# MIT-SPARK/Kimera-Semantics

Hardware: AMD Instinct MI355X
Metric: Mvoxel-updates/s + frames/s, 640×480 @5cm voxels, 1/2/4/8 MI355X (higher is better)
Workload: dtype f32; 1 GPU; bag-replay stand-in: 640x480 depth+label trajectory (room), 'fast' integrator, 5 cm voxels, 5 m rays, trunc 0.2 m, p=0.8; pipeline_frames=12, parallelism=frame-sharded x1, points_per_frame=305657, rays_per_frame=85307, updates_per_frame=502687

## Files before the change

### include/ks_hip.h

```cpp
#ifndef KS_HIP_H_
#define KS_HIP_H_

#include <stddef.h>
#include <stdint.h>

#ifdef __cplusplus
extern "C" {
#endif

#define KS_NUM_LABELS 21

enum {
  KS_OK = 0,
  KS_ERR_INVALID_ARG = -1,
  KS_ERR_LABEL_RANGE = -2,
  KS_ERR_PROBABILITY = -3,
  KS_ERR_HIP = -4,
  KS_ERR_POOL_FULL = -5,
  KS_ERR_INDEX_RANGE = -6,
  KS_ERR_NO_DEVICE = -7,
  KS_ERR_UNSUPPORTED = -8,
  KS_ERR_PEER_FAILED = -9
};

enum { KS_METHOD_FAST = 0, KS_METHOD_MERGED = 1 };
enum { KS_COLOR_MODE_COLOR = 0, KS_COLOR_MODE_SEMANTIC = 1, KS_COLOR_MODE_SEMANTIC_PROBABILITY = 2 };
enum { KS_ORDER_MIXED = 0, KS_ORDER_SORTED = 1, KS_ORDER_MIXED_1024_GROUPS = 2 };
enum { KS_BUNDLE_ORDER_REFERENCE = 0, KS_BUNDLE_ORDER_CANONICAL = 1 };
enum { KS_EARLY_OUT_EXACT = 1 };

typedef struct ks_config {
  float voxel_size;
  int32_t voxels_per_side;
  float truncation_distance;
  float max_weight;
  float min_ray_length_m;
  float max_ray_length_m;
  int32_t voxel_carving_enabled;
  int32_t use_const_weight;
  int32_t allow_clear;
  int32_t use_weight_dropoff;
  int32_t use_sparsity_compensation_factor;
  float sparsity_compensation_factor;
  int32_t enable_anti_grazing;
  float start_voxel_subsampling_factor;
  int32_t max_consecutive_ray_collisions;
  int32_t clear_checks_every_n_frames;
  int32_t integration_order_mode;
  int32_t integrator_threads;
  int32_t method;
  int32_t bundle_order;
  float semantic_measurement_probability;
  int32_t color_mode;
  int32_t n_dynamic_labels;
  uint8_t dynamic_labels[32];
  uint8_t label_rgba[256][4];
  int32_t early_out_phase_growth;
  int32_t device_id;
  uint32_t max_tiles;
  uint32_t max_points;
  int32_t pipeline_frames;
} ks_config;

typedef struct ks_frame_stats {
  uint64_t n_points;
  uint64_t n_valid_points;
  uint64_t n_rays_cast;
  uint64_t n_voxel_updates;
  uint64_t n_blocks_allocated;
} ks_frame_stats;

enum {
  KS_STAGE_POINTS = 0,
  KS_STAGE_SORT_POINTS,
  KS_STAGE_RAYS,
  KS_STAGE_MARCH,
  KS_STAGE_EMIT,
  KS_STAGE_SORT_PAIRS,
  KS_STAGE_APPLY,
  KS_STAGE_APPLY_LONG,
  KS_STAGE_COUNT
};
typedef struct ks_profile {
  double ms[KS_STAGE_COUNT];
  uint64_t launches[KS_STAGE_COUNT];
  uint64_t frames;
  uint64_t updates;
  uint64_t points;
  double apply_kernel_ms;
  uint64_t apply_kernel_launches;
  uint64_t apply_kernel_updates;
  double host_ms;
  double host_wait_ms;
} ks_profile;

typedef struct ks_ctx ks_ctx;

int ks_default_config(ks_config* cfg);
int ks_create(const ks_config* cfg, ks_ctx** out);
void ks_destroy(ks_ctx* ctx);
const char* ks_last_error(ks_ctx* ctx);

int ks_set_color_to_label(ks_ctx* ctx, const uint8_t* rgba_keys, const uint8_t* labels, size_t n);

int ks_integrate_points(ks_ctx* ctx, const float T_G_C[7], const float* xyz, const uint8_t* rgba,
                        const uint8_t* labels, size_t n, int freespace, ks_frame_stats* stats);
int ks_integrate_points_device(ks_ctx* ctx, const float T_G_C[7], const float* d_xyz, const uint8_t* d_rgba,
                               const uint8_t* d_labels, size_t n, int freespace, ks_frame_stats* stats);

int ks_integrate_depth(ks_ctx* ctx, const float T_G_C[7], const void* depth, int depth_fmt, const uint8_t* label_img,
                       const uint8_t* rgba_img, int width, int height, const float K[4], int freespace,
                       ks_frame_stats* stats);
int ks_integrate_depth_device(ks_ctx* ctx, const float T_G_C[7], const void* d_depth, int depth_fmt,
                              const uint8_t* d_label_img, const uint8_t* d_rgba_img, int width, int height,
                              const float K[4], int freespace, ks_frame_stats* stats);

int ks_num_blocks(ks_ctx* ctx, size_t* n);
int ks_get_block_indices(ks_ctx* ctx, int32_t* out_xyz, size_t cap, size_t* n);
int ks_get_updated_block_indices(ks_ctx* ctx, int32_t* out_xyz, size_t cap, size_t* n, int reset);
int ks_download_blocks(ks_ctx* ctx, const int32_t* idx_xyz, size_t n, void* tsdf_out, void* sem_out);
int ks_upload_blocks(ks_ctx* ctx, const int32_t* idx_xyz, size_t n, const void* tsdf_in, const void* sem_in);
#define KS_VOXEL_RECORD_BYTES 120
typedef struct ks_voxel_run {
  int32_t block[3];
  uint32_t first;
  uint32_t count;
} ks_voxel_run;
int ks_count_updated_voxels(ks_ctx* ctx, size_t* n_records, size_t* n_runs );
int ks_download_updated_voxels(ks_ctx* ctx, void* out, size_t cap_records, size_t* n_records, ks_voxel_run* runs,
                               size_t cap_runs, size_t* n_runs);
void* ks_host_alloc(size_t bytes);
void ks_host_free(void* p);

typedef struct ks_mesh_config { float min_weight; int32_t only_stale; } ks_mesh_config;
typedef struct ks_mesh_stats {
  uint64_t blocks_meshed, blocks_total, triangles_total, triangles_changed, degenerate_dropped;
} ks_mesh_stats;
typedef struct ks_mesh_block { int32_t block[3]; uint32_t first_vertex, n_vertices; } ks_mesh_block;
int ks_mesh_default_config(ks_mesh_config* cfg);
int ks_mesh_update(ks_ctx* ctx, const ks_mesh_config* cfg, ks_mesh_stats* stats );
int ks_mesh_size(ks_ctx* ctx, size_t* n_blocks, size_t* n_vertices);
int ks_mesh_download(ks_ctx* ctx, ks_mesh_block* blocks, size_t cap_blocks, float* xyz, float* normals, uint8_t* rgba,
                     uint8_t* labels, size_t cap_vertices);
int ks_mesh_changed_blocks(ks_ctx* ctx, int32_t* out_xyz, size_t cap, size_t* n);

typedef struct ks_esdf_config {
  float min_weight, min_distance_m, max_distance_m;
  int32_t use_region;
  int32_t region_min[3], region_max[3];
  uint64_t max_workspace_bytes;
} ks_esdf_config;
typedef struct ks_esdf_stats { uint64_t voxels_observed, voxels_fixed, voxels_clamped, box_voxels[3], workspace_bytes; } ks_esdf_stats;
#define KS_ESDF_RECORD_BYTES 8
int ks_esdf_default_config(ks_esdf_config* cfg);
int ks_esdf_update(ks_ctx* ctx, const ks_esdf_config* cfg, ks_esdf_stats* stats );
typedef struct ks_esdf_refresh_stats {
  uint64_t tiles_stale, tiles_recomputed, tiles_total;
  uint64_t voxels_observed, voxels_fixed, voxels_clamped;
  uint64_t workspace_bytes;
} ks_esdf_refresh_stats;
int ks_esdf_refresh(ks_ctx* ctx, uint64_t max_workspace_bytes , ks_esdf_refresh_stats* stats );
int ks_esdf_changed_blocks(ks_ctx* ctx, int32_t* out_xyz, size_t cap, size_t* n);
int ks_esdf_download_blocks(ks_ctx* ctx, const int32_t* idx_xyz, size_t n, void* out );
int ks_esdf_query(ks_ctx* ctx, const float* xyz , size_t n, float* distance, uint8_t* flags,
                  uint8_t* label );

typedef struct ks_render_config { float min_weight, min_range_m, max_range_m; } ks_render_config;
typedef struct ks_render_stats { uint64_t pixels_hit, pixels_missed, samples; } ks_render_stats;
int ks_render_default_config(ks_render_config* cfg);
int ks_render_view(ks_ctx* ctx, const float T_G_C[7], const float K[4] , int width, int height,
                   const ks_render_config* cfg, float* depth, uint8_t* labels, uint8_t* rgba ,
                   float* normals , ks_render_stats* stats );
int ks_render_view_device(ks_ctx* ctx, const float T_G_C[7], const float K[4], int width, int height, const ks_render_config* cfg,
                          float* d_depth, uint8_t* d_labels, uint8_t* d_rgba, float* d_normals, ks_render_stats* stats);

#define KS_TILE_BYTES 65536
int ks_get_tile_keys(ks_ctx* ctx, uint64_t* out, size_t cap, size_t* n);
int ks_export_tiles_device(ks_ctx* ctx, const uint32_t* slots, size_t n, void* d_payload);
int ks_merge_tiles_device(ks_ctx* ctx, const uint64_t* keys, size_t n, const void* d_payload);
int ks_clear(ks_ctx* ctx);
int ks_clear_voxels(ks_ctx* ctx);
int ks_reset_tiles(ks_ctx* ctx, const uint32_t* slots, size_t n);
int ks_tile_owner(uint64_t tile_key, int world);
typedef struct ks_reduce_stats {
  uint64_t tiles_sent, tiles_received, tiles_local, bytes_sent;
} ks_reduce_stats;
int ks_reduce(ks_ctx* ctx, void* rccl_comm, int rank, int world, ks_reduce_stats* stats);

typedef struct ks_round_stats {
  uint64_t updates_marched, updates_applied, bytes_sent, origin_voxel_touched, rays_cast;
} ks_round_stats;
int ks_integrate_round_exact(ks_ctx* marcher, ks_ctx* owner, void* rccl_comm, int rank, int world, uint64_t first_frame,
                             const float T_G_C[7], const float* xyz, const uint8_t* rgba, const uint8_t* labels, size_t n,
                             int freespace_points, ks_round_stats* stats);

int ks_debug_radix_sort(ks_ctx* ctx, void* keys, uint32_t* vals, size_t n, int key_bits, unsigned end_bit);

int ks_synchronize(ks_ctx* ctx);
void* ks_stream(ks_ctx* ctx);
int ks_flush(ks_ctx* ctx, ks_frame_stats* stats);
int ks_profile_enable(ks_ctx* ctx, int level);
int ks_early_out_iterations(ks_ctx* ctx, uint64_t* frames, uint64_t* iterations);
int ks_early_out_stats(ks_ctx* ctx, uint64_t out[5]);
int ks_profile_get(ks_ctx* ctx, ks_profile* out, int reset);
int ks_update_stats(ks_ctx* ctx, uint64_t out[4]);
int ks_pipeline_shape(ks_ctx* ctx, int32_t out[4]);
int ks_stream_plan(ks_ctx* ctx, int32_t out[8]);
int ks_seed_launch_shape(int32_t integration_order_mode, int32_t early_out_phase_growth, uint64_t cap_points, uint32_t* out, int32_t max_phases);

#ifdef __cplusplus
}
#endif
#endif
```

### kimera_semantics_amd/binding.py

```python
from __future__ import annotations

import ctypes as C
import os
import subprocess

import numpy as np

_HERE = os.path.dirname(os.path.abspath(__file__))
LIB_PATH = os.environ.get("KS_HIP_LIB") or os.path.join(_HERE, "libks_hip.so")
NUM_LABELS = 21

KS_METHOD_FAST, KS_METHOD_MERGED = 0, 1
KS_COLOR_MODE_COLOR, KS_COLOR_MODE_SEMANTIC, KS_COLOR_MODE_SEMANTIC_PROBABILITY = 0, 1, 2
KS_ORDER_MIXED, KS_ORDER_SORTED, KS_ORDER_MIXED_1024_GROUPS = 0, 1, 2
KS_BUNDLE_ORDER_REFERENCE, KS_BUNDLE_ORDER_CANONICAL = 0, 1
KS_EARLY_OUT_EXACT = 1
KS_ERR_LABEL_RANGE, KS_ERR_PROBABILITY, KS_ERR_POOL_FULL, KS_ERR_NO_DEVICE, KS_ERR_UNSUPPORTED = -2, -3, -5, -7, -8
KS_ERR_INVALID_ARG, KS_ERR_PEER_FAILED = -1, -9

STAGES = ["points", "sort_points", "rays", "march", "emit", "sort_pairs", "apply", "apply_long"]

TSDF_DTYPE = np.dtype([("distance", "<f4"), ("weight", "<f4"), ("color", "u1", (4,))])
SEM_DTYPE = np.dtype([("label", "u1"), ("pad", "u1", (3,)), ("priors", "<f4", (NUM_LABELS,)),
                      ("color", "u1", (4,))])

ABI_SYMBOLS = [
    "ks_default_config", "ks_create", "ks_destroy", "ks_last_error", "ks_set_color_to_label",
    "ks_integrate_points", "ks_integrate_points_device", "ks_integrate_depth", "ks_integrate_depth_device", "ks_num_blocks", "ks_get_block_indices",
    "ks_get_updated_block_indices", "ks_count_updated_voxels", "ks_download_updated_voxels", "ks_download_blocks", "ks_upload_blocks", "ks_host_alloc", "ks_host_free", "ks_get_tile_keys", "ks_export_tiles_device", "ks_merge_tiles_device", "ks_clear", "ks_clear_voxels", "ks_reset_tiles", "ks_tile_owner", "ks_reduce",
    "ks_debug_radix_sort", "ks_synchronize", "ks_flush", "ks_stream",
    "ks_profile_enable", "ks_profile_get", "ks_early_out_iterations", "ks_early_out_stats", "ks_pipeline_shape", "ks_stream_plan", "ks_seed_launch_shape", "ks_update_stats", "ks_integrate_round_exact",
    "ks_mesh_default_config", "ks_mesh_update", "ks_mesh_size", "ks_mesh_download", "ks_mesh_changed_blocks",
    "ks_esdf_default_config", "ks_esdf_update", "ks_esdf_download_blocks", "ks_esdf_query",
    "ks_esdf_refresh", "ks_esdf_changed_blocks",
    "ks_render_default_config", "ks_render_view", "ks_render_view_device",
]


class KsConfig(C.Structure):
    _fields_ = [
        ("voxel_size", C.c_float), ("voxels_per_side", C.c_int32),
        ("truncation_distance", C.c_float), ("max_weight", C.c_float),
        ("min_ray_length_m", C.c_float), ("max_ray_length_m", C.c_float),
        ("voxel_carving_enabled", C.c_int32), ("use_const_weight", C.c_int32),
        ("allow_clear", C.c_int32), ("use_weight_dropoff", C.c_int32),
        ("use_sparsity_compensation_factor", C.c_int32), ("sparsity_compensation_factor", C.c_float),
        ("enable_anti_grazing", C.c_int32), ("start_voxel_subsampling_factor", C.c_float),
        ("max_consecutive_ray_collisions", C.c_int32), ("clear_checks_every_n_frames", C.c_int32),
        ("integration_order_mode", C.c_int32), ("integrator_threads", C.c_int32),
        ("method", C.c_int32), ("bundle_order", C.c_int32),
        ("semantic_measurement_probability", C.c_float), ("color_mode", C.c_int32),
        ("n_dynamic_labels", C.c_int32), ("dynamic_labels", C.c_uint8 * 32),
        ("label_rgba", (C.c_uint8 * 4) * 256),
        ("early_out_phase_growth", C.c_int32),
        ("device_id", C.c_int32), ("max_tiles", C.c_uint32), ("max_points", C.c_uint32), ("pipeline_frames", C.c_int32),
    ]


class KsRoundStats(C.Structure):
    _fields_ = [("updates_marched", C.c_uint64), ("updates_applied", C.c_uint64), ("bytes_sent", C.c_uint64),
                ("origin_voxel_touched", C.c_uint64), ("rays_cast", C.c_uint64)]


class KsFrameStats(C.Structure):
    _fields_ = [("n_points", C.c_uint64), ("n_valid_points", C.c_uint64), ("n_rays_cast", C.c_uint64),
                ("n_voxel_updates", C.c_uint64), ("n_blocks_allocated", C.c_uint64)]


class KsReduceStats(C.Structure):
    _fields_ = [("tiles_sent", C.c_uint64), ("tiles_received", C.c_uint64), ("tiles_local", C.c_uint64),
                ("bytes_sent", C.c_uint64)]


class KsMeshConfig(C.Structure):
    _fields_ = [("min_weight", C.c_float), ("only_stale", C.c_int32)]


class KsMeshStats(C.Structure):
    _fields_ = [("blocks_meshed", C.c_uint64), ("blocks_total", C.c_uint64), ("triangles_total", C.c_uint64),
                ("triangles_changed", C.c_uint64), ("degenerate_dropped", C.c_uint64)]


MESH_BLOCK_DTYPE = np.dtype([("block", "<i4", (3,)), ("first_vertex", "<u4"), ("n_vertices", "<u4")])


class KsEsdfConfig(C.Structure):
    _fields_ = [("min_weight", C.c_float), ("min_distance_m", C.c_float), ("max_distance_m", C.c_float), ("use_region", C.c_int32),
                ("region_min", C.c_int32 * 3), ("region_max", C.c_int32 * 3), ("max_workspace_bytes", C.c_uint64)]


class KsEsdfStats(C.Structure):
    _fields_ = [("voxels_observed", C.c_uint64), ("voxels_fixed", C.c_uint64), ("voxels_clamped", C.c_uint64),
                ("box_voxels", C.c_uint64 * 3), ("workspace_bytes", C.c_uint64)]


class KsEsdfRefreshStats(C.Structure):
    _fields_ = [("tiles_stale", C.c_uint64), ("tiles_recomputed", C.c_uint64), ("tiles_total", C.c_uint64),
                ("voxels_observed", C.c_uint64), ("voxels_fixed", C.c_uint64), ("voxels_clamped", C.c_uint64),
                ("workspace_bytes", C.c_uint64)]


ESDF_DTYPE = np.dtype([("distance", "<f4"), ("flags", "u1"), ("label", "u1"), ("pad", "u1", (2,))])


class KsRenderConfig(C.Structure):
    _fields_ = [("min_weight", C.c_float), ("min_range_m", C.c_float), ("max_range_m", C.c_float)]


class KsRenderStats(C.Structure):
    _fields_ = [("pixels_hit", C.c_uint64), ("pixels_missed", C.c_uint64), ("samples", C.c_uint64)]


class KsProfile(C.Structure):
    _fields_ = [("ms", C.c_double * 8), ("launches", C.c_uint64 * 8), ("frames", C.c_uint64),
                ("updates", C.c_uint64), ("points", C.c_uint64), ("apply_kernel_ms", C.c_double),
                ("apply_kernel_launches", C.c_uint64), ("apply_kernel_updates", C.c_uint64),
                ("host_ms", C.c_double), ("host_wait_ms", C.c_double)]


def build(force: bool = False) -> str:
    src_dir = os.path.join(_HERE, "csrc")
    srcs = [os.path.join(src_dir, f) for f in ("ks_hip.hip", "ks_types.h", "ks_k_rays.h", "ks_k_bundle_order.h", "ks_k_march.h", "ks_k_exact.h", "ks_k_apply.h",
                                                "ks_k_apply_xl.h", "ks_k_shard.h", "ks_k_shard_merged.h", "ks_k_io.h", "ks_k_mesh.h", "ks_k_esdf.h", "ks_k_render.h", "ks_mc_tri_table.inc", "ks_device_math.h", "ks_radix_sort.h", "ks_owned.h")]
    srcs.append(os.path.join(_HERE, "..", "include", "ks_hip.h"))
    stale = (not os.path.exists(LIB_PATH)) or any(
        os.path.exists(s) and os.path.getmtime(s) > os.path.getmtime(LIB_PATH) for s in srcs)
    if force or stale:
        subprocess.check_call(["make", "-C", src_dir])
    return LIB_PATH


_lib = None


def lib():
    global _lib
    if _lib is None:
        if not os.path.exists(LIB_PATH):
            raise RuntimeError(f"{LIB_PATH} is missing: run `python -c 'import __graft_entry__ as g; g.build()'` "
                               "(the HIP path has no CPU fallback)")
        L = C.CDLL(LIB_PATH)
        vp = C.c_void_p
        L.ks_default_config.argtypes = [C.POINTER(KsConfig)]
        L.ks_create.argtypes = [C.POINTER(KsConfig), C.POINTER(vp)]
        L.ks_destroy.argtypes = [vp]
        L.ks_destroy.restype = None
        L.ks_last_error.argtypes = [vp]
        L.ks_last_error.restype = C.c_char_p
        L.ks_set_color_to_label.argtypes = [vp, vp, vp, C.c_size_t]
        L.ks_integrate_points.argtypes = [vp, vp, vp, vp, vp, C.c_size_t, C.c_int, C.POINTER(KsFrameStats)]
        L.ks_integrate_points_device.argtypes = [vp, vp, vp, vp, vp, C.c_size_t, C.c_int, C.POINTER(KsFrameStats)]
        L.ks_integrate_depth.argtypes = [vp, vp, vp, C.c_int, vp, vp, C.c_int, C.c_int, vp, C.c_int, C.POINTER(KsFrameStats)]
        L.ks_integrate_depth_device.argtypes = [vp, vp, vp, C.c_int, vp, vp, C.c_int, C.c_int, vp, C.c_int, C.POINTER(KsFrameStats)]
        L.ks_num_blocks.argtypes = [vp, C.POINTER(C.c_size_t)]
        L.ks_get_block_indices.argtypes = [vp, vp, C.c_size_t, C.POINTER(C.c_size_t)]
        L.ks_get_updated_block_indices.argtypes = [vp, vp, C.c_size_t, C.POINTER(C.c_size_t), C.c_int]
        L.ks_download_blocks.argtypes = [vp, vp, C.c_size_t, vp, vp]
        L.ks_count_updated_voxels.argtypes = [vp, C.POINTER(C.c_size_t), C.POINTER(C.c_size_t)]
        L.ks_download_updated_voxels.argtypes = [vp, vp, C.c_size_t, C.POINTER(C.c_size_t), vp, C.c_size_t, C.POINTER(C.c_size_t)]
        L.ks_upload_blocks.argtypes = [vp, vp, C.c_size_t, vp, vp]
        L.ks_host_alloc.argtypes = [C.c_size_t]
        L.ks_host_alloc.restype = C.c_void_p
        L.ks_host_free.argtypes = [vp]
        L.ks_host_free.restype = None
        L.ks_get_tile_keys.argtypes = [vp, vp, C.c_size_t, C.POINTER(C.c_size_t)]
        L.ks_export_tiles_device.argtypes = [vp, vp, C.c_size_t, vp]
        L.ks_merge_tiles_device.argtypes = [vp, vp, C.c_size_t, vp]
        L.ks_clear.argtypes = [vp]
        L.ks_clear_voxels.argtypes = [vp]
        L.ks_reset_tiles.argtypes = [vp, vp, C.c_size_t]
        L.ks_tile_owner.argtypes = [C.c_uint64, C.c_int]
        L.ks_reduce.argtypes = [vp, vp, C.c_int, C.c_int, C.POINTER(KsReduceStats)]
        L.ks_debug_radix_sort.argtypes = [vp, vp, vp, C.c_size_t, C.c_int, C.c_uint]
        L.ks_synchronize.argtypes = [vp]
        L.ks_flush.argtypes = [vp, C.POINTER(KsFrameStats)]
        L.ks_stream.argtypes = [vp]
        L.ks_stream.restype = vp
        L.ks_profile_enable.argtypes = [vp, C.c_int]
        L.ks_profile_get.argtypes = [vp, C.POINTER(KsProfile), C.c_int]
        L.ks_early_out_iterations.argtypes = [vp, C.POINTER(C.c_uint64), C.POINTER(C.c_uint64)]
        L.ks_early_out_stats.argtypes = [vp, C.POINTER(C.c_uint64)]
        L.ks_pipeline_shape.argtypes = [vp, C.POINTER(C.c_int32)]
        L.ks_stream_plan.argtypes = [vp, C.POINTER(C.c_int32)]
        L.ks_seed_launch_shape.argtypes = [C.c_int32, C.c_int32, C.c_uint64, C.POINTER(C.c_uint32), C.c_int32]
        L.ks_update_stats.argtypes = [vp, C.POINTER(C.c_uint64)]
        L.ks_integrate_round_exact.argtypes = [vp, vp, vp, C.c_int, C.c_int, C.c_uint64, vp, vp, vp, vp, C.c_size_t, C.c_int, C.POINTER(KsRoundStats)]
        L.ks_mesh_default_config.argtypes = [C.POINTER(KsMeshConfig)]
        L.ks_mesh_update.argtypes = [vp, C.POINTER(KsMeshConfig), C.POINTER(KsMeshStats)]
        L.ks_mesh_size.argtypes = [vp, C.POINTER(C.c_size_t), C.POINTER(C.c_size_t)]
        L.ks_mesh_download.argtypes = [vp, vp, C.c_size_t, vp, vp, vp, vp, C.c_size_t]
        L.ks_mesh_changed_blocks.argtypes = [vp, vp, C.c_size_t, C.POINTER(C.c_size_t)]
        L.ks_esdf_default_config.argtypes = [C.POINTER(KsEsdfConfig)]
        L.ks_esdf_update.argtypes = [vp, C.POINTER(KsEsdfConfig), C.POINTER(KsEsdfStats)]
        L.ks_esdf_download_blocks.argtypes = [vp, vp, C.c_size_t, vp]
        L.ks_esdf_query.argtypes = [vp, vp, C.c_size_t, vp, vp, vp]
        L.ks_esdf_refresh.argtypes = [vp, C.c_uint64, C.POINTER(KsEsdfRefreshStats)]
        L.ks_esdf_changed_blocks.argtypes = [vp, vp, C.c_size_t, C.POINTER(C.c_size_t)]
        L.ks_render_default_config.argtypes = [C.POINTER(KsRenderConfig)]
        L.ks_render_view.argtypes = [vp, vp, vp, C.c_int, C.c_int, C.POINTER(KsRenderConfig), vp, vp, vp, vp, C.POINTER(KsRenderStats)]
        L.ks_render_view_device.argtypes = [vp, vp, vp, C.c_int, C.c_int, C.POINTER(KsRenderConfig), vp, vp, vp, vp, C.POINTER(KsRenderStats)]
        _lib = L
    return _lib


def default_config(**overrides) -> KsConfig:
    cfg = KsConfig()
    lib().ks_default_config(C.byref(cfg))
    apply_overrides(cfg, **overrides)
    return cfg


def apply_overrides(cfg, **overrides):
    for k, v in overrides.items():
        if k == "dynamic_labels":
            cfg.n_dynamic_labels = len(v)
            for i, lab in enumerate(v):
                cfg.dynamic_labels[i] = int(lab)
        elif k == "label_rgba":
            arr = np.ascontiguousarray(np.asarray(v, dtype=np.uint8).reshape(256, 4))
            C.memmove(cfg.label_rgba, arr.ctypes.data, 1024)
        else:
            if not hasattr(cfg, k):
                raise AttributeError(k)
            setattr(cfg, k, v)
    return cfg


class KsError(RuntimeError):
    def __init__(self, code, msg):
        super().__init__(f"ks error {code}: {msg}")
        self.code = code


def _ptr(a):
    return None if a is None else a.ctypes.data


class HipIntegrator:

    def __init__(self, cfg: KsConfig):
        self.cfg = cfg
        self.vps = cfg.voxels_per_side
        self._h = C.c_void_p()
        rc = lib().ks_create(C.byref(cfg), C.byref(self._h))
        if rc != 0:
            raise KsError(rc, lib().ks_last_error(None).decode())

    def _chk(self, rc):
        if rc != 0:
            raise KsError(rc, lib().ks_last_error(self._h).decode())

    def close(self):
        if getattr(self, "_h", None):
            lib().ks_destroy(self._h)
            self._h = C.c_void_p()

    def __del__(self):
        try:
            self.close()
        except Exception:
            pass

    def set_color_to_label(self, rgba_keys, labels):
        k = np.ascontiguousarray(rgba_keys, dtype=np.uint8).reshape(-1, 4)
        l = np.ascontiguousarray(labels, dtype=np.uint8)
        self._chk(lib().ks_set_color_to_label(self._h, _ptr(k), _ptr(l), len(l)))

    def integrate(self, T_G_C, xyz, rgba, labels, freespace=False) -> KsFrameStats:
        T = np.ascontiguousarray(T_G_C, dtype=np.float32)
        xyz = np.ascontiguousarray(xyz, dtype=np.float32)
        labels = None if labels is None else np.ascontiguousarray(labels, dtype=np.uint8)
        rgba = None if rgba is None else np.ascontiguousarray(rgba, dtype=np.uint8)
        st = KsFrameStats()
        self._chk(lib().ks_integrate_points(self._h, _ptr(T), _ptr(xyz), _ptr(rgba), _ptr(labels), xyz.shape[0],
                                            int(freespace), C.byref(st)))
        return st

    def integrate_depth(self, T_G_C, depth, K, label_img=None, rgba_img=None, freespace=False) -> KsFrameStats:
        T = np.ascontiguousarray(T_G_C, dtype=np.float32)
        depth = np.ascontiguousarray(depth)
        fmt = 0 if depth.dtype == np.float32 else 1
        assert depth.dtype in (np.float32, np.uint16)
        Kc = np.ascontiguousarray(K, dtype=np.float32)
        lab = None if label_img is None else np.ascontiguousarray(label_img, dtype=np.uint8)
        col = None if rgba_img is None else np.ascontiguousarray(rgba_img, dtype=np.uint8)
        st = KsFrameStats()
        self._chk(lib().ks_integrate_depth(self._h, _ptr(T), _ptr(depth), fmt, _ptr(lab), _ptr(col), depth.shape[1],
                                           depth.shape[0], _ptr(Kc), int(freespace), C.byref(st)))
        return st

    def integrate_depth_device(self, T_G_C, d_depth: int, fmt: int, d_label_img: int, d_rgba_img: int, width: int,
                               height: int, K, freespace=False) -> KsFrameStats:
        T = np.ascontiguousarray(T_G_C, dtype=np.float32)
        Kc = np.ascontiguousarray(K, dtype=np.float32)
        st = KsFrameStats()
        self._chk(lib().ks_integrate_depth_device(self._h, _ptr(T), d_depth or None, fmt, d_label_img or None,
                                                  d_rgba_img or None, width, height, _ptr(Kc), int(freespace), C.byref(st)))
        return st

    def integrate_device(self, T_G_C, d_xyz: int, d_rgba: int, d_labels: int, n: int, freespace=False) -> KsFrameStats:
        T = np.ascontiguousarray(T_G_C, dtype=np.float32)
        st = KsFrameStats()
        self._chk(lib().ks_integrate_points_device(self._h, _ptr(T), d_xyz or None, d_rgba or None, d_labels or None, n,
                                                   int(freespace), C.byref(st)))
        return st

    def block_indices(self) -> np.ndarray:
        n = C.c_size_t()
        self._chk(lib().ks_get_block_indices(self._h, None, 0, C.byref(n)))
        out = np.zeros((n.value, 3), dtype=np.int32)
        if n.value:
            self._chk(lib().ks_get_block_indices(self._h, _ptr(out), n.value, C.byref(n)))
        return out

    def updated_block_indices(self, reset=True) -> np.ndarray:
        n = C.c_size_t()
        self._chk(lib().ks_get_updated_block_indices(self._h, None, 0, C.byref(n), 0))
        out = np.zeros((n.value, 3), dtype=np.int32)
        self._chk(lib().ks_get_updated_block_indices(self._h, _ptr(out), n.value, C.byref(n), int(reset)))
        return out

    def download(self, indices=None):
        if indices is None:
            indices = self.block_indices()
        indices = np.ascontiguousarray(indices, dtype=np.int32).reshape(-1, 3)
        nv = self.vps ** 3
        t = np.zeros((len(indices), nv), dtype=TSDF_DTYPE)
        s = np.zeros((len(indices), nv), dtype=SEM_DTYPE)
        if len(indices):
            self._chk(lib().ks_download_blocks(self._h, _ptr(indices), len(indices), _ptr(t), _ptr(s)))
        return indices, t, s

    def upload(self, indices, tsdf=None, sem=None):
        indices = np.ascontiguousarray(indices, dtype=np.int32).reshape(-1, 3)
        nv = self.vps ** 3
        tp = sp = None
        if tsdf is not None:
            tsdf = np.ascontiguousarray(tsdf, dtype=TSDF_DTYPE).reshape(len(indices), nv)
            tp = _ptr(tsdf)
        if sem is not None:
            sem = np.ascontiguousarray(sem, dtype=SEM_DTYPE).reshape(len(indices), nv)
            sp = _ptr(sem)
        self._chk(lib().ks_upload_blocks(self._h, _ptr(indices), len(indices), tp, sp))

    def mesh(self, only_stale=False, min_weight=1e-4):
        from .mesh import Mesh
        mc, st = KsMeshConfig(float(min_weight), int(bool(only_stale))), KsMeshStats()
        self._chk(lib().ks_mesh_update(self._h, C.byref(mc), C.byref(st)))
        nb, nv = C.c_size_t(), C.c_size_t()
        self._chk(lib().ks_mesh_size(self._h, C.byref(nb), C.byref(nv)))
        blocks = np.zeros(nb.value, dtype=MESH_BLOCK_DTYPE)
        xyz, normals = np.zeros((nv.value, 3), np.float32), np.zeros((nv.value, 3), np.float32)
        rgba, labels = np.zeros((nv.value, 4), np.uint8), np.zeros(nv.value, np.uint8)
        self._chk(lib().ks_mesh_download(self._h, _ptr(blocks), nb.value, _ptr(xyz), _ptr(normals), _ptr(rgba), _ptr(labels), nv.value))
        return Mesh(blocks, xyz, normals, rgba, labels, {k: int(getattr(st, k)) for k, _ in KsMeshStats._fields_})

    def mesh_changed_blocks(self) -> np.ndarray:
        n = C.c_size_t()
        self._chk(lib().ks_mesh_changed_blocks(self._h, None, 0, C.byref(n)))
        out = np.zeros((n.value, 3), dtype=np.int32)
        if n.value:
            self._chk(lib().ks_mesh_changed_blocks(self._h, _ptr(out), n.value, C.byref(n)))
        return out

    def esdf_update(self, region=None, **cfg) -> dict:
        ec, st = KsEsdfConfig(), KsEsdfStats()
        lib().ks_esdf_default_config(C.byref(ec))
        for k, v in cfg.items():
            if k not in ("min_weight", "min_distance_m", "max_distance_m", "max_workspace_bytes"):
                raise AttributeError(k)
            setattr(ec, k, v)
        if region is not None:
            ec.use_region = 1
            for a in range(3):
                ec.region_min[a], ec.region_max[a] = int(region[0][a]), int(region[1][a])
        rc = lib().ks_esdf_update(self._h, C.byref(ec), C.byref(st))
        stats = {k: ([int(v) for v in getattr(st, k)] if k == "box_voxels" else int(getattr(st, k))) for k, _ in KsEsdfStats._fields_}
        if rc != 0:
            err = KsError(rc, lib().ks_last_error(self._h).decode())
            err.stats = stats
            raise err
        return stats

    def esdf(self, region=None, **cfg):
        stats = self.esdf_update(region=region, **cfg)
        idx = self.block_indices()
        return idx, self.esdf_blocks(idx), stats

    def esdf_refresh(self, max_workspace_bytes=0) -> dict:
        st = KsEsdfRefreshStats()
        rc = lib().ks_esdf_refresh(self._h, int(max_workspace_bytes), C.byref(st))
        stats = {k: int(getattr(st, k)) for k, _ in KsEsdfRefreshStats._fields_}
        if rc != 0:
            err = KsError(rc, lib().ks_last_error(self._h).decode())
            err.stats = stats
            raise err
        return stats

    def esdf_changed_blocks(self) -> np.ndarray:
        n = C.c_size_t()
        self._chk(lib().ks_esdf_changed_blocks(self._h, None, 0, C.byref(n)))
        out = np.zeros((n.value, 3), dtype=np.int32)
        if n.value:
            self._chk(lib().ks_esdf_changed_blocks(self._h, _ptr(out), n.value, C.byref(n)))
        return out

    def esdf_blocks(self, indices) -> np.ndarray:
        indices = np.ascontiguousarray(indices, dtype=np.int32).reshape(-1, 3)
        out = np.zeros((len(indices), self.vps ** 3), dtype=ESDF_DTYPE)
        self._chk(lib().ks_esdf_download_blocks(self._h, _ptr(indices), len(indices), _ptr(out)))
        return out

    def esdf_query(self, xyz) -> np.ndarray:
        xyz = np.ascontiguousarray(xyz, dtype=np.float32).reshape(-1, 3)
        n = len(xyz)
        d, f, l = np.zeros(n, np.float32), np.zeros(n, np.uint8), np.zeros(n, np.uint8)
        self._chk(lib().ks_esdf_query(self._h, _ptr(xyz), n, _ptr(d), _ptr(f), _ptr(l)))
        out = np.zeros(n, dtype=ESDF_DTYPE)
        out["distance"], out["flags"], out["label"] = d, f, l
        return out

    def render_config(self, **cfg) -> KsRenderConfig:
        rc = KsRenderConfig()
        lib().ks_render_default_config(C.byref(rc))
        for k, v in cfg.items():
            if k not in ("min_weight", "min_range_m", "max_range_m"):
                raise AttributeError(k)
            if v is not None:
                setattr(rc, k, v)
        return rc

    def render(self, T_G_C, K, width, height, min_weight=None, min_range_m=None, max_range_m=None, normals=True):
        T = np.ascontiguousarray(T_G_C, dtype=np.float32)
        Kc = np.ascontiguousarray(K, dtype=np.float32)
        rc, st = self.render_config(min_weight=min_weight, min_range_m=min_range_m, max_range_m=max_range_m), KsRenderStats()
        w, h = int(width), int(height)
        shape = (max(h, 0), max(w, 0))
        depth, labels, rgba = np.zeros(shape, np.float32), np.zeros(shape, np.uint8), np.zeros(shape + (4,), np.uint8)
        nrm = np.zeros(shape + (3,), np.float32) if normals else None
        self._chk(lib().ks_render_view(self._h, _ptr(T), _ptr(Kc), w, h, C.byref(rc), _ptr(depth), _ptr(labels), _ptr(rgba), _ptr(nrm), C.byref(st)))
        return depth, labels, rgba, nrm, {k: int(getattr(st, k)) for k, _ in KsRenderStats._fields_}

    def render_device(self, T_G_C, K, width, height, d_depth: int, d_labels: int, d_rgba: int, d_normals: int, stats=True, **cfg):
        T = np.ascontiguousarray(T_G_C, dtype=np.float32)
        Kc = np.ascontiguousarray(K, dtype=np.float32)
        rc, st = self.render_config(**cfg), KsRenderStats()
        self._chk(lib().ks_render_view_device(self._h, _ptr(T), _ptr(Kc), int(width), int(height), C.byref(rc), d_depth or None, d_labels or None,
                                              d_rgba or None, d_normals or None, C.byref(st) if stats else None))
        return {k: int(getattr(st, k)) for k, _ in KsRenderStats._fields_} if stats else None

    TILE_BYTES = 65536

    def tile_keys(self) -> np.ndarray:
        n = C.c_size_t()
        self._chk(lib().ks_get_tile_keys(self._h, None, 0, C.byref(n)))
        out = np.zeros(n.value, dtype=np.uint64)
        if n.value:
            self._chk(lib().ks_get_tile_keys(self._h, _ptr(out), n.value, C.byref(n)))
        return out

    def export_tiles(self, slots: np.ndarray, d_payload: int):
        s = np.ascontiguousarray(slots, dtype=np.uint32)
        self._chk(lib().ks_export_tiles_device(self._h, _ptr(s), len(s), d_payload or None))

    def merge_tiles(self, keys: np.ndarray, d_payload: int):
        k = np.ascontiguousarray(keys, dtype=np.uint64)
        self._chk(lib().ks_merge_tiles_device(self._h, _ptr(k), len(k), d_payload or None))

    def download_updated_voxels(self):
        n, nr = C.c_size_t(), C.c_size_t()
        self._chk(lib().ks_count_updated_voxels(self._h, C.byref(n), C.byref(nr)))
        dt = np.dtype([("block", "<i4", (3,)), ("linear", "<u4"), ("tsdf", TSDF_DTYPE), ("sem", SEM_DTYPE)])
        rdt = np.dtype([("block", "<i4", (3,)), ("first", "<u4"), ("count", "<u4")])
        assert dt.itemsize == 120 and rdt.itemsize == 20
        out = np.zeros(n.value, dtype=dt)
        runs = np.zeros(nr.value, dtype=rdt)
        if n.value:
            m, mr = C.c_size_t(), C.c_size_t()
            self._chk(lib().ks_download_updated_voxels(self._h, _ptr(out), n.value, C.byref(m), _ptr(runs), nr.value, C.byref(mr)))
            assert m.value == n.value and mr.value == nr.value
            assert int(runs["count"].sum()) == n.value
            for r in runs[:: max(1, len(runs) // 16)]:
                if r["count"]:
                    assert (out["block"][r["first"]:r["first"] + r["count"]] == r["block"]).all()
        return out

    def clear(self):
        self._chk(lib().ks_clear(self._h))

    def clear_voxels(self):
        self._chk(lib().ks_clear_voxels(self._h))

    def reset_tiles(self, slots: np.ndarray):
        s = np.ascontiguousarray(slots, dtype=np.uint32)
        self._chk(lib().ks_reset_tiles(self._h, _ptr(s), len(s)))

    def reduce(self, rccl_comm, rank: int, world: int) -> dict:
        st = KsReduceStats()
        self._chk(lib().ks_reduce(self._h, C.c_void_p(rccl_comm) if rccl_comm else None, rank, world, C.byref(st)))
        return {"tiles_sent": st.tiles_sent, "tiles_received": st.tiles_received, "tiles_local": st.tiles_local,
                "bytes_sent": st.bytes_sent}

    def debug_radix_sort(self, keys: np.ndarray, vals=None, end_bit=None):
        keys = np.ascontiguousarray(keys).copy()
        bits = keys.dtype.itemsize * 8
        vals = None if vals is None else np.ascontiguousarray(vals, dtype=np.uint32).copy()
        self._chk(lib().ks_debug_radix_sort(self._h, _ptr(keys), _ptr(vals), keys.shape[0], bits,
                                            bits if end_bit is None else end_bit))
        return keys, vals

    def synchronize(self):
        self._chk(lib().ks_synchronize(self._h))

    @property
    def stream(self) -> int:
        return lib().ks_stream(self._h) or 0

    def profile_enable(self, level=1):
        self._chk(lib().ks_profile_enable(self._h, int(level)))

    def early_out_stats(self):
        out = (C.c_uint64 * 5)()
        self._chk(lib().ks_early_out_stats(self._h, out))
        return dict(frames=int(out[0]), rounds=int(out[1]), fallbacks=int(out[2]), event_driven=bool(out[3]), pipelined=bool(out[4]))

    def integrate_round_exact(self, marcher: "HipIntegrator", rccl_comm, rank: int, world: int, first_frame: int, T_G_C, xyz, rgba, labels,
                              freespace=False) -> dict:
        T = np.ascontiguousarray(T_G_C, dtype=np.float32)
        n = 0 if xyz is None else len(xyz)
        x = None if xyz is None else np.ascontiguousarray(xyz, dtype=np.float32)
        c = None if rgba is None else np.ascontiguousarray(rgba, dtype=np.uint8)
        l = None if labels is None else np.ascontiguousarray(labels, dtype=np.uint8)
        st = KsRoundStats()
        self._chk(lib().ks_integrate_round_exact(marcher._h, self._h, rccl_comm, int(rank), int(world), int(first_frame), _ptr(T),
                                                 _ptr(x) if x is not None else None, _ptr(c) if c is not None else None,
                                                 _ptr(l) if l is not None else None, n, int(bool(freespace)), C.byref(st)))
        return dict(updates_marched=int(st.updates_marched), updates_applied=int(st.updates_applied), bytes_sent=int(st.bytes_sent),
                    origin_voxel_touched=bool(st.origin_voxel_touched), rays_cast=int(st.rays_cast))

    def update_stats(self):
        out = (C.c_uint64 * 4)()
        self._chk(lib().ks_update_stats(self._h, out))
        return dict(walked=int(out[0]), serial=int(out[1]), chunks=int(out[2]), replayed=int(out[3]))

    def pipeline_shape(self):
        out = (C.c_int32 * 4)()
        self._chk(lib().ks_pipeline_shape(self._h, out))
        return dict(lag=int(out[0]), slots=int(out[1]), batch=int(out[2]), march_streams=int(out[3]))

    def stream_plan(self):
        out = (C.c_int32 * 8)()
        self._chk(lib().ks_stream_plan(self._h, out))
        side = {1: "own", 0: "tail", -1: "none"}
        return dict(budget=int(out[0]), streams=int(out[1]), march_streams=int(out[2]), long=side[int(out[3])], xlong=side[int(out[4])],
                    march="own" if out[5] else "A", tail="own" if out[6] else "A", streams_held=int(out[7]))

    def early_out_iterations(self):
        f, it = C.c_uint64(), C.c_uint64()
        self._chk(lib().ks_early_out_iterations(self._h, C.byref(f), C.byref(it)))
        return f.value, it.value

    def flush(self) -> KsFrameStats:
        st = KsFrameStats()
        self._chk(lib().ks_flush(self._h, C.byref(st)))
        return st

    def profile(self, reset=False) -> dict:
        p = KsProfile()
        self._chk(lib().ks_profile_get(self._h, C.byref(p), int(reset)))
        return {"ms": {STAGES[i]: p.ms[i] for i in range(8)}, "launches": {STAGES[i]: p.launches[i] for i in range(8)},
                "frames": p.frames, "updates": p.updates, "points": p.points,
                "apply_kernel_ms": p.apply_kernel_ms, "apply_kernel_launches": p.apply_kernel_launches,
                "apply_kernel_updates": p.apply_kernel_updates, "host_ms": p.host_ms, "host_wait_ms": p.host_wait_ms}
```

### kimera_semantics_amd/csrc/ks_hip.hip

```cpp

#include <atomic>
#include <chrono>
#include <condition_variable>
#include <mutex>
#include <thread>
#include <cstring>
#include <string.h>

#include <dlfcn.h>
#include <hip/hip_runtime.h>
#include <hip/hip_ext.h>
#include <rccl/rccl.h>

#include <algorithm>
#include <iterator>
#include <cmath>
#include <cstdio>
#include <cstring>
#include <string>
#include <unordered_map>
#include <vector>

#include "../../include/ks_hip.h"
#include "ks_device_math.h"
// ... 338 lines not shown
  DevBuf<float> mesh_xyz[2], mesh_nrm[2];
  DevBuf<uint32_t> mesh_rgba[2];
  DevBuf<uint8_t> mesh_label[2];
  size_t mesh_cap[2] = {0, 0};
  int mesh_cur = 0;
  bool mesh_valid = false;
  float mesh_min_weight = 0.f;
  std::vector<uint64_t> mesh_blocks;
  uint32_t mesh_tiles_seen = 0;
  std::vector<ks_mesh_block> mesh_dir;
  std::vector<int32_t> mesh_changed;
  DevBuf<uint8_t> d_mesh_buf[10];
  DevBuf<EsdfRecord> esdf_store;
  DevBuf<uint64_t> esdf_keys[2];
  DevBuf<uint32_t> esdf_slots;
  DevBuf<unsigned long long> esdf_counters;
  DevBuf<EsdfRecord> esdf_out;
  DevBuf<int32_t> esdf_idx;
  DevBuf<float> esdf_xyz;
  bool esdf_valid = false;
  uint32_t esdf_tiles = 0;
  ks_esdf_config esdf_cfg{};
  uint64_t esdf_totals[3] = {0, 0, 0};
  std::vector<int32_t> esdf_changed;
  DevBuf<uint64_t> esdf_bricks[2];
  DevBuf<uint64_t> esdf_lists;
  DevBuf<uint32_t> esdf_zslots;
  DevBuf<float> render_depth, render_normals;
  DevBuf<uint32_t> render_rgba;
  DevBuf<uint8_t> render_labels;
  DevBuf<unsigned long long> render_counters;
  ks_profile prof{};
  ProfSet pset[kProfSets];
  bool fatal = false;
};

#define HIPCHK(ctx, expr)                                                                         \
  do {                                                                                            \
    hipError_t e_ = (expr);                                                                       \
    if (e_ != hipSuccess) {                                                                       \
      (ctx)->err = std::string(#expr) + ": " + hipGetErrorString(e_);                             \
      return KS_ERR_HIP;                                                                          \
    }                                                                                             \
  } while (0)

int ks_hip_failed(ks_ctx* ctx, const char* what, hipError_t e) {
  ctx->err = std::string(what) + ": " + hipGetErrorString(e);
  return KS_ERR_HIP;
}

namespace {

inline hipStream_t march_stream(ks_ctx* c, uint64_t frame_no) { return c->stream_march_[frame_no % (uint64_t)c->n_march]; }
inline uint64_t* observed_table(ks_ctx* c, uint64_t frame_no) { return c->d_observed_[frame_no % (uint64_t)c->n_obs]; }
int sync_march(ks_ctx* c) {
  for (int i = 0; i < c->n_march; ++i)
    if (c->stream_march_[i] != c->stream) HIPCHK(c, hipStreamSynchronize(c->stream_march_[i]));
  return KS_OK;
}

void probe_rehash_schedule(size_t n_max, BoSchedule* out) {
  static std::mutex mu;
  static std::vector<uint32_t> t, b;
  static size_t probed = 0;
  std::lock_guard<std::mutex> lk(mu);
  if (probed < n_max) {
    t.clear();
    b.clear();
    std::unordered_map<uint32_t, char> m;
    size_t bc = m.bucket_count();
    for (uint32_t i = 0; i < n_max; ++i) {
      m.emplace(i, 0);
      if (m.bucket_count() != bc) {
        bc = m.bucket_count();
        t.push_back(i);
        b.push_back((uint32_t)bc);
      }
    }
    probed = n_max;
  }
  *out = BoSchedule{};
  uint32_t off = 0;
  int e = 0;
  for (; e < (int)t.size() && e < kBoMaxEpochs && t[e] < n_max; ++e) {
    out->t[e] = t[e];
    out->b[e] = b[e];
    out->head_off[e] = off;
    off += b[e];
  }
  out->n_epochs = (uint32_t)e;
  out->t[e] = UINT32_MAX;
}

int ensure_bundle_order(ks_ctx* c, size_t cap) {
  probe_rehash_schedule(cap, &c->bo_sched);
  const BoSchedule& S = c->bo_sched;
  {
    static const uint32_t kLibstdcxxBuckets[] = {13, 29, 59, 127, 257, 541, 1109, 2357, 5087, 10273, 20753, 42043, 85229, 172933};
    for (uint32_t e = 0; e < S.n_epochs && e < sizeof(kLibstdcxxBuckets) / sizeof(uint32_t); ++e)
      if (S.b[e] != kLibstdcxxBuckets[e] || (e > 0 && S.t[e] != kLibstdcxxBuckets[e - 1])) {
        c->err = "bundle_order = KS_BUNDLE_ORDER_REFERENCE needs libstdc++'s unordered_map rehash schedule (13, 29, 59, ...): this build's standard "
                 "library differs; use KS_BUNDLE_ORDER_CANONICAL";
        return KS_ERR_UNSUPPORTED;
      }
  }
  c->bo_epochs = (int)S.n_epochs;
  size_t heads = 0;
  for (uint32_t e = 0; e < S.n_epochs; ++e) heads += S.b[e];
  const size_t nbt = cap / kBoBlock + 2, nfbt = 2 * cap / kBoBlock + 2;
  auto al = [](size_t words) { return (words * 4 + 255) & ~(size_t)255; };
  const size_t per_map = 11 * al(cap) + al(nbt) + al(heads);
  const size_t total = 2 * per_map + al(2) + al((sizeof(BoSchedule) + 3) / 4) + 2 * al(2 * cap) + al(nfbt) + al(cap);
  if (int rc = c->d_bo_slab.alloc(c, total)) return rc;
  uint8_t* p = c->d_bo_slab;
  auto take = [&](size_t words) { uint32_t* r = (uint32_t*)p; p += al(words); return r; };
  for (int m = 0; m < 2; ++m) {
    BoMap& M = c->bo.m[m];
    M.H = take(cap); M.rank = take(cap);
    M.next[0] = take(cap); M.next[1] = take(cap);
    M.idj[0] = take(cap); M.idj[1] = take(cap);
    M.kj[0] = take(cap); M.kj[1] = take(cap);
    M.lp = take(cap); M.gm = take(cap); M.cj = take(cap);
    M.bt = take(nbt);
    M.head = take(heads);
    HIPCHK(c, hipMemsetAsync(M.head, 0xff, heads * 4, c->stream));
  }
  c->bo.B = take(2);
  BoSchedule* d_sched = (BoSchedule*)take((sizeof(BoSchedule) + 3) / 4);
  c->bo.sched = d_sched;
  c->bo.flag = take(2 * cap);
  c->bo.flag_lp = take(2 * cap);
  c->bo.flag_bt = take(nfbt);
  c->bo.t_of_head = take(cap);
  HIPCHK(c, hipMemcpyAsync(d_sched, &c->bo_sched, sizeof(BoSchedule), hipMemcpyHostToDevice, c->stream));
  HIPCHK(c, hipStreamSynchronize(c->stream));
  return KS_OK;
}

inline uint32_t order_chains(int order_mode, size_t n) {
  const size_t q = n / kOrderStep;
  return (order_mode == KS_ORDER_MIXED && q >= 1) ? (uint32_t)q : kOrderStep;
}
inline uint32_t order_chains_cap(int order_mode, size_t cap) { return std::max(order_chains(order_mode, cap), order_mode == KS_ORDER_MIXED ? kOrderStep : 0u); }
inline uint32_t order_generations_cap(int order_mode, size_t cap) {
  if (order_mode == KS_ORDER_MIXED) return cap >= kOrderStep ? 2u * kOrderStep - 1u : 1u;
  return (uint32_t)((cap + kOrderStep - 1) / kOrderStep);
}
std::vector<uint32_t> phase_bounds(uint32_t n_gen, int growth) {
  std::vector<uint32_t> b{0};
  for (;;) {
    const uint64_t inc = std::max<uint64_t>(1, (uint64_t)b.back() * (uint64_t)(growth - 16) / 16);
    if (b.back() + inc >= n_gen) break;
    b.push_back((uint32_t)(b.back() + inc));
  }
  return b;
}
inline uint64_t seed_items_of(int order_mode, size_t n, uint32_t g0, uint32_t g1) {
  if (n == 0) return 0;
  const uint64_t chains = order_chains(order_mode, n), full = n / chains, part = n % chains;
  auto subs = [&](uint64_t gens) -> uint64_t {
    const uint64_t hi = std::min<uint64_t>(g1, gens);
    return hi > g0 ? (hi - g0 + kSubRun - 1) / kSubRun : 0;
  };
  return (chains - part) * subs(full) + part * subs(full + 1);
}
std::vector<SeedPhase> seed_launch_shape(int order_mode, int growth, size_t cap) {
  const uint32_t n_gen = order_generations_cap(order_mode, cap);
  const std::vector<uint32_t> B = phase_bounds(n_gen, growth);
  std::vector<SeedPhase> out;
  uint64_t off = 0;
  for (size_t j = 0; j < B.size(); ++j) {
    const uint32_t g0 = B[j], g1 = (j + 1 < B.size()) ? B[j + 1] : n_gen;
    uint64_t m = 0;
    if (order_mode == KS_ORDER_MIXED) {
      m = seed_items_of(order_mode, std::min<size_t>(cap, kOrderStep - 1), g0, g1);
      for (size_t q = 1; q <= cap / kOrderStep; ++q) m = std::max(m, seed_items_of(order_mode, std::min<size_t>(cap, q * kOrderStep + kOrderStep - 1), g0, g1));
    } else {
      m = seed_items_of(order_mode, cap, g0, g1);
    }
    out.push_back(SeedPhase{g0, g1, (uint32_t)off, (uint32_t)m});
    off += m;
  }
  return out;
}

size_t steps_max_of(const ks_config& cfg, float voxel_size_inv) {
  const double max_len = (double)cfg.max_ray_length_m + 2.0 * (double)cfg.truncation_distance;
  return (size_t)std::ceil(1.7321 * max_len * (double)voxel_size_inv) + 8;
}
int ensure_exact_points(ks_ctx* c, size_t cap);
int ensure_points(ks_ctx* c, size_t n) {
  if (n <= c->cap_points) return KS_OK;
  const size_t cap = std::max<size_t>(c->cap_points ? n + n / 8 : n, 1024);
  c->cap_points = 0;
  int rc;
  if ((rc = c->d_xyz.alloc(c, cap * 3))) return rc;
  if ((rc = c->d_rgba.alloc(c, cap * 4))) return rc;
  if ((rc = c->d_labels.alloc(c, cap))) return rc;
  ++c->buffers_epoch;
  const size_t scan_cap = (c->cfg.method == KS_METHOD_MERGED ? 2 : 1) * cap;
  size_t seed_items = 0;
  if (c->uses_early_out) {
    c->seed_phases = seed_launch_shape(c->cfg.integration_order_mode, c->cfg.early_out_phase_growth, cap);
    uint32_t off = 0;
    for (SeedPhase& P : c->seed_phases) {
      if ((P.g1 - P.g0 + kSubRun - 1) / kSubRun > (1u << kSeedSubBits) || order_chains_cap(c->cfg.integration_order_mode, cap) > (1u << kSeedChainBits)) {
        c->err = "point cloud too large for the early-out's work list";
        return KS_ERR_INVALID_ARG;
      }
      if (c->seed_cap_items) P.item_cap = (uint32_t)std::min<size_t>(P.item_cap, c->seed_cap_items);
      P.item_off = off;
      off += P.item_cap;
    }
    seed_items = off;
    if ((rc = c->d_seed_phases.alloc(c, c->seed_phases.size()))) return rc;
    HIPCHK(c, hipMemcpyAsync(c->d_seed_phases, c->seed_phases.data(), c->seed_phases.size() * sizeof(SeedPhase), hipMemcpyHostToDevice, c->stream));
    HIPCHK(c, hipStreamSynchronize(c->stream));
  }
  for (int i = 0; i < (c->cfg.pipeline_frames ? c->n_slots : 1); ++i) {
    if (c->uses_early_out) {
      if ((rc = c->slot[i].d_seed_gen.alloc(c, cap + order_chains_cap(c->cfg.integration_order_mode, cap)))) return rc;
      if ((rc = c->slot[i].d_seed_items.alloc(c, seed_items))) return rc;
      if ((rc = c->slot[i].d_seed_n.alloc(c, c->seed_phases.size()))) return rc;
    }
    if ((rc = c->slot[i].d_rays.alloc(c, cap))) return rc;
    if ((rc = c->slot[i].d_ray_list.alloc(c, cap))) return rc;
    if ((rc = c->slot[i].d_cnt.alloc(c, scan_cap))) return rc;
    if ((rc = c->slot[i].d_lp.alloc(c, scan_cap))) return rc;
    if ((rc = c->slot[i].d_bt.alloc(c, scan_cap / kScanBlock + 2))) return rc;
    if (c->cfg.method == KS_METHOD_FAST && (rc = c->slot[i].d_live.alloc(c, cap))) return rc;
    if (c->cfg.enable_anti_grazing && c->cfg.method == KS_METHOD_MERGED) {
      if ((rc = c->slot[i].d_gkeys.alloc(c, cap))) return rc;
      if ((rc = c->slot[i].d_rkeys.alloc(c, cap))) return rc;
    }
    if (c->cfg.method == KS_METHOD_MERGED && (rc = c->slot[i].d_deltas.alloc(c, cap * kNumLabels))) return rc;
  }
  if ((rc = c->d_hash.alloc(c, cap))) return rc;
  if ((rc = c->d_skeys32.alloc(c, cap))) return rc;
  if ((rc = c->d_skeys32b.alloc(c, cap))) return rc;
  if ((rc = c->d_pkeys.alloc(c, cap))) return rc;
  if ((rc = c->d_pkeys2.alloc(c, cap))) return rc;
  if ((rc = c->d_pvals.alloc(c, cap))) return rc;
  if ((rc = c->d_pvals2.alloc(c, cap))) return rc;
  if ((rc = c->d_order.alloc(c, cap))) return rc;
  if ((rc = c->d_inv_order.alloc(c, cap))) return rc;
  if ((rc = c->d_okeys.alloc(c, cap))) return rc;
  if ((rc = c->d_okeys2.alloc(c, cap))) return rc;
  if ((rc = c->d_ovals.alloc(c, cap))) return rc;
  if (c->cfg.method == KS_METHOD_MERGED) {
    if ((rc = c->d_gpw.alloc(c, cap))) return rc;
    if ((rc = c->d_glc.alloc(c, cap))) return rc;
    if ((rc = c->d_ray_keys.alloc(c, cap))) return rc;
    if ((rc = c->d_blong.alloc(c, cap / kLongRun + 64))) return rc;
    if (c->key_bits) {
      size_t slots = 1024;
      while (slots < 2 * cap) slots <<= 1;
      if ((rc = c->d_key_overflow.alloc(c, slots))) return rc;
      HIPCHK(c, hipMemsetAsync(c->d_key_overflow, 0, slots * sizeof(uint64_t), c->stream));
      c->key_overflow_mask = (uint32_t)(slots - 1);
    }
  }
  if (c->use_bundle_rank && (rc = ensure_bundle_order(c, cap))) return rc;
  if (c->exact_early_out) {
    if ((rc = c->d_eo_lp.alloc(c, cap))) return rc;
    if ((rc = c->d_eo_bt.alloc(c, cap / kScanBlock + 2))) return rc;
    if ((rc = ensure_exact_points(c, cap))) return rc;
  }
  c->cap_points = cap;
  return KS_OK;
}

int ensure_pairs_in(ks_ctx* c, FrameSlot& S, size_t bound) {
  if (bound <= S.d_pairs.size()) return KS_OK;
  if (int rc = S.d_pairs.alloc(c, std::max<size_t>(bound, 1 << 20))) return rc;
  ++c->buffers_epoch;
  return KS_OK;
}
int ensure_pairs_out(ks_ctx* c, size_t n) {
  if (n <= c->cap_pairs) return KS_OK;
  const size_t cap = std::max<size_t>(n + n / 4, 1 << 20);
  c->cap_pairs = 0;
  int rc;
  HIPCHK(c, hipStreamSynchronize(c->stream_long));
  if (c->stream_xlong) HIPCHK(c, hipStreamSynchronize(c->stream_xlong));
  if (c->stream_tail) HIPCHK(c, hipStreamSynchronize(c->stream_tail));
  for (int b = 0; b < 2; ++b) {
    if ((rc = c->d_pairs2_[b].alloc(c, cap))) return rc;
    if ((rc = c->d_long_list_[b].alloc(c, cap / kLongRunLanes + 64 + cap / kXLongRun + 64))) return rc;
    if (c->long_lanes && (rc = c->d_long_sorted_[b].alloc(c, cap / kLongRunLanes + 64))) return rc;
  }
  if (c->d_xl_hdr && (rc = c->d_xl_fb.alloc(c, cap / kXLongRun + 64))) return rc;
  c->cap_pairs = cap;
  return KS_OK;
}

template <typename K>
int sort_keys(ks_ctx* c, K* a, K* b, size_t n, unsigned end_bit, K** result, unsigned begin_bit = 0, bool tail = false) {
  HIPCHK(c, (ksrs::sort<K, false>(tail ? c->sort_ws_tail : c->sort_ws, a, b, nullptr, nullptr, n, end_bit,
                                  tail ? c->stream_tail : c->stream, result, nullptr, begin_bit)));
  return KS_OK;
}
template <typename K>
int sort_pairs(ks_ctx* c, K* ka, K* kb, uint32_t* va, uint32_t* vb, size_t n, unsigned end_bit, K** kres,
               uint32_t** vres) {
  HIPCHK(c, (ksrs::sort<K, true>(c->sort_ws, ka, kb, va, vb, n, end_bit, c->stream, kres, vres)));
  return KS_OK;
}

inline unsigned bits_for(uint64_t n) {
  unsigned b = 1;
  while (b < 64 && (1ull << b) < n) ++b;
  return b;
}

int launch_batch(ks_ctx* c);
int quiesce(ks_ctx* c);
int reset_set(ks_ctx* c, uint64_t* d_set0, uint64_t* offset, bool observed) {
  const bool full = ++(*offset) >= kFullResetThreshold;
  const bool retag = observed && !full && c->obs_tag + (uint32_t)c->cfg.clear_checks_every_n_frames + 2u >= kObsMaxTag;
  if (full || retag) {
    if (int rc = launch_batch(c)) return rc;
    if (full && c->exact_early_out) {
      if (int rc = quiesce(c)) return rc;
    }
    if (int rc = sync_march(c)) return rc;
    if (full) *offset = 0;
    for (int t = 0; t < (observed ? c->n_obs : 1); ++t) {
      uint64_t* d_set = observed ? c->d_observed_[t] : d_set0;
      if (full) {
        HIPCHK(c, hipMemsetAsync(d_set, 0, (observed ? 2 : 1) * (sizeof(uint64_t) << kSetBits), c->stream));
        const uint64_t poison = observed ? kObsPoison : ~0ull;
        HIPCHK(c, hipMemcpyAsync(d_set, &poison, sizeof(poison), hipMemcpyHostToDevice, c->stream));
      } else {
        hipLaunchKernelGGL(k_obs_retag, dim3((2u << kSetBits) / 256), dim3(256), 0, c->stream, d_set);
      }
    }
    if (observed && full && c->d_eo_plain) {
      HIPCHK(c, hipMemsetAsync(c->d_eo_plain, 0, sizeof(uint64_t) << kSetBits, c->stream));
      const uint64_t poison = ~0ull;
      HIPCHK(c, hipMemcpyAsync(c->d_eo_plain, &poison, sizeof(poison), hipMemcpyHostToDevice, c->stream));
    }
    HIPCHK(c, hipStreamSynchronize(c->stream));
    if (observed) c->obs_tag = 0;
  }
  if (observed) c->obs_tag_lo = c->obs_tag + 1;
  return KS_OK;
}

inline void stage_mark(ks_ctx* c, int set, int ev) {
  if (set >= 0 && c->pset[set].stages)
    (void)hipEventRecord(c->pset[set].ev[ev], ev <= 3 ? c->stream : ev <= 5 ? c->prof_march_stream : c->stream_tail);
}

void resolve_prof(ks_ctx* c, int set) {
  ProfSet& P = c->pset[set];
  if (!P.used || !P.complete) return;
  (void)hipEventSynchronize(P.ev[kStageEvents - 1]);
  if (P.stages) {
    for (int s = 0; s < KS_STAGE_COUNT; ++s) {
      float ms = 0.f;
      const int a = s < 3 ? s : s == 3 ? 4 : s + 2;
      if (hipEventElapsedTime(&ms, P.ev[a], P.ev[a + 1]) == hipSuccess) {
        c->prof.ms[s] += ms;
        c->prof.launches[s] += 1;
      }
    }
  }
  if (P.applied) {
    float kms = 0.f;
    if (hipEventElapsedTime(&kms, P.k0, P.k1) == hipSuccess) {
      c->prof.apply_kernel_ms += kms;
      c->prof.apply_kernel_launches += 1;
      c->prof.apply_kernel_updates += P.n_pairs;
    }
  }
  c->prof.frames += 1;
  c->prof.updates += P.n_pairs;
  c->prof.points += P.n_points;
  P.used = P.complete = P.applied = false;
}

SlotView slot_view(const FrameSlot& S, Counters* counters = nullptr) {
  SlotView v{};
  v.F = S.d_F;
  v.rays = S.d_rays;
  v.cnt = S.d_cnt;
  v.lp = S.d_lp;
  v.bt = S.d_bt;
  v.ray_list = S.d_ray_list;
  v.pairs = S.d_pairs;
  v.pairs_cap = (unsigned long long)S.d_pairs.size();
  v.C = counters ? counters : S.d_counters;
  v.host_snap = (uint32_t*)S.h_snap.get();
  v.eo_stats = S.d_eo_ctl ? &S.d_eo_ctl->n_x : nullptr;
  v.seed_gen = S.d_seed_gen;
  v.seed_items = S.d_seed_items;
  v.seed_n = S.d_seed_n;
  return v;
}

void launch_emit(ks_ctx* c, const BatchView& V, uint32_t nb, bool wide, hipStream_t st) {
  const size_t n = c->cap_points;
  const size_t lds = ((2 * n + kScanBlock - 1) / kScanBlock) * sizeof(unsigned long long);
  if (!(c->cfg.method == KS_METHOD_MERGED && c->cfg.enable_anti_grazing)) {
    if (wide || c->cfg.method == KS_METHOD_MERGED || !c->uses_early_out) {
      hipLaunchKernelGGL(k_emit_lane<8>, dim3((uint32_t)((n + 31) / 32), nb), dim3(256), lds, st, V, c->table, c->pool);
    } else {
      hipLaunchKernelGGL(k_emit_lane<16>, dim3((uint32_t)((n + 63) / 64), nb), dim3(256), lds, st, V, c->table, c->pool);
    }
  } else if (wide) {
    hipLaunchKernelGGL(k_emit<64>, dim3((uint32_t)((n + 3) / 4), nb), dim3(256), lds, st, V, c->table, c->pool);
  } else {
    hipLaunchKernelGGL(k_emit<16>, dim3((uint32_t)((n + 15) / 16), nb), dim3(256), lds, st, V, c->table, c->pool);
  }
}

void enqueue_stage_b(ks_ctx* c, const BatchView& V, uint32_t nb, bool wide, hipStream_t sm, size_t steps_max, int part = 0) {
  const ks_config& cfg = c->cfg;
  const size_t n = c->cap_points;
  if (c->uses_early_out && part != 2) {
    for (size_t j = 0; j < c->seed_phases.size(); ++j) {
      const SeedPhase& P = c->seed_phases[j];
      if (P.item_cap == 0) continue;
      const uint32_t steps_cap = (uint32_t)((steps_max + 3) & ~(size_t)3);
      const size_t lds_wave = (size_t)test_lds_words64(steps_cap) * sizeof(unsigned long long);
      const uint32_t wpb = lds_wave * 4 <= 60 * 1024 ? 4u : lds_wave * 2 <= 60 * 1024 ? 2u : 1u;
      const dim3 grid((P.item_cap + wpb - 1) / wpb, nb), block(64 * wpb);
      if (c->test_overlap) hipLaunchKernelGGL(k_test<true>, grid, block, lds_wave * wpb, sm, V, P.g0, P.g1, (uint32_t)j, P.item_off, P.item_cap, steps_cap);
      else hipLaunchKernelGGL(k_test<false>, grid, block, lds_wave * wpb, sm, V, P.g0, P.g1, (uint32_t)j, P.item_off, P.item_cap, steps_cap);
    }
  }
  if (part == 1) return;
  if (cfg.method == KS_METHOD_MERGED && cfg.enable_anti_grazing)
    hipLaunchKernelGGL(k_count_grazing<16>, dim3((uint32_t)((n + 15) / 16), nb), dim3(256), 0, sm, V);
  hipLaunchKernelGGL(k_scan_local, dim3((uint32_t)(((cfg.method == KS_METHOD_MERGED ? 2 : 1) * n + kScanBlock - 1) / kScanBlock), nb),
                     dim3(1024), 0, sm, V);
  launch_emit(c, V, nb, wide, sm);
  hipLaunchKernelGGL(k_publish, dim3(nb), dim3(64), 0, sm, V, (const uint32_t*)c->table.n_tiles);
}

int ensure_marks(ks_ctx* c, size_t n) {
  if (n <= c->cap_marks) return KS_OK;
  const size_t cap = std::max<size_t>(n + n / 4, 1 << 20);
  c->cap_marks = 0;
  int rc;
  for (int b = 0; b < 2; ++b) {
    if ((rc = c->d_eo_keys[b].alloc(c, cap))) return rc;
    if ((rc = c->d_eo_vals[b].alloc(c, cap))) return rc;
  }
  c->cap_marks = cap;
  return KS_OK;
}
constexpr int kEoMaxIterations = 4096;
int exact_early_out(ks_ctx* c, FrameSlot& S, hipStream_t st, Counters* counters = nullptr) {
  const size_t n = S.n;
  Counters* const d_counters = counters ? counters : S.d_counters;
  const FrameParams* dF = S.d_F;
  EoState* hs = c->h_eo_state;
  HIPCHK(c, hipMemsetAsync(c->d_eo_state, 0, sizeof(EoState), st));
  hipLaunchKernelGGL(k_eo_total, dim3((uint32_t)std::min<size_t>((n + 255) / 256, 1024)), dim3(256), 0, st, dF,
                     (const uint32_t*)S.d_cnt, c->d_eo_state);
  HIPCHK(c, hipMemcpyAsync(hs, c->d_eo_state, sizeof(EoState), hipMemcpyDeviceToHost, st));
  HIPCHK(c, hipStreamSynchronize(st));
  const uint32_t nb4k = (uint32_t)((n + kScanBlock - 1) / kScanBlock);
  const size_t lds = (size_t)nb4k * sizeof(unsigned long long);
  uint64_t* kres = nullptr;
  uint32_t* vres = nullptr;
  unsigned long long n_marks = hs->n_marks_next;
  bool converged = n_marks == 0;
  int it = 0;
  for (; !converged && it < kEoMaxIterations; ++it) {
    int rc;
    if ((rc = ensure_marks(c, n_marks))) return rc;
    HIPCHK(c, hipMemsetAsync(c->d_eo_range, 0, sizeof(uint2) << kSetBits, st));
    hipLaunchKernelGGL(k_eo_scan, dim3(nb4k), dim3(1024), 0, st, dF, (const uint32_t*)S.d_cnt, c->d_eo_lp, c->d_eo_bt, c->d_eo_state);
    if (S.wide)
      hipLaunchKernelGGL(k_eo_emit<8>, dim3((uint32_t)((n + 31) / 32)), dim3(256), lds, st, dF, S.d_ray_list, S.d_rays, S.d_cnt,
                         c->d_eo_lp, c->d_eo_bt, c->d_eo_keys[0], c->d_eo_vals[0], (unsigned long long)c->cap_marks, d_counters,
                         c->d_eo_state);
    else
      hipLaunchKernelGGL(k_eo_emit<64>, dim3((uint32_t)((n + 255) / 256)), dim3(256), lds, st, dF, S.d_ray_list, S.d_rays, S.d_cnt,
                         c->d_eo_lp, c->d_eo_bt, c->d_eo_keys[0], c->d_eo_vals[0], (unsigned long long)c->cap_marks, d_counters,
                         c->d_eo_state);
    HIPCHK(c, (ksrs::sort<uint64_t, true>(counters ? c->sort_ws_tail : c->sort_ws, c->d_eo_keys[0], c->d_eo_keys[1], c->d_eo_vals[0], c->d_eo_vals[1],
                                          (size_t)n_marks, 64, st, &kres, &vres, 44)));
    hipLaunchKernelGGL(k_eo_index, dim3((uint32_t)((n_marks + 255) / 256)), dim3(256), 0, st, n_marks, (const uint64_t*)kres,
                       c->d_eo_range);
    EoBuf E{kres, vres, c->d_eo_range, c->d_eo_plain};
    if (S.wide)
      hipLaunchKernelGGL(k_eo_eval<8>, dim3((uint32_t)((n + 31) / 32)), dim3(256), 0, st, dF, S.d_ray_list, S.d_rays, S.d_cnt, E,
                         d_counters, c->d_eo_state);
    else
      hipLaunchKernelGGL(k_eo_eval<16>, dim3((uint32_t)((n + 63) / 64)), dim3(256), 0, st, dF, S.d_ray_list, S.d_rays, S.d_cnt, E,
                         d_counters, c->d_eo_state);
    HIPCHK(c, hipMemcpyAsync(hs, c->d_eo_state, sizeof(EoState), hipMemcpyDeviceToHost, st));
    HIPCHK(c, hipStreamSynchronize(st));
    if (hs->n_marks != n_marks) {
      c->err = "exact early-out: mark count mismatch";
      return KS_ERR_HIP;
    }
    if (hs->changed == 0) converged = true;
    else n_marks = hs->n_marks_next;
  }
  if (!converged) {
    c->err = "exact early-out: no fixed point within the iteration limit";
    return KS_ERR_UNSUPPORTED;
  }
  c->eo_iterations += (uint64_t)it;
  if (!counters) c->eo_frames += 1;
  if (n_marks)
    hipLaunchKernelGGL(k_eo_commit, dim3((uint32_t)((n_marks + 255) / 256)), dim3(256), 0, st, n_marks, (const uint64_t*)kres,
                       (const uint32_t*)vres, c->d_eo_plain);
  return KS_OK;
}

int ensure_exact_slots(ks_ctx* c, size_t cap_marks, size_t cap_x) {
  if (!c->eo_device) return KS_OK;
  int rc;
  const int n_slots = c->cfg.pipeline_frames ? c->n_slots : 1;
  for (int i = 0; i < n_slots; ++i) {
    FrameSlot& S = c->slot[i];
    if (!S.d_eo_ctl) {
      if ((rc = S.d_eo_ctl.alloc(c, 1))) return rc;
      if ((rc = S.d_eo_tab.alloc(c, (size_t)1 << kSetBits))) return rc;
      HIPCHK(c, hipMemsetAsync(S.d_eo_tab, 0, sizeof(uint4) << kSetBits, c->stream));
      if ((rc = S.eo_committed.create(c, hipEventDisableTiming))) return rc;
    }
    if (S.eo_cap_marks < cap_marks) {
      S.eo_cap_marks = 0;
      for (int b = 0; b < 2; ++b) {
        if ((rc = S.d_eo_keys[b].alloc(c, cap_marks))) return rc;
        if ((rc = S.d_eo_vals[b].alloc(c, cap_marks))) return rc;
      }
      if ((rc = S.d_eo_sort_ws.alloc(c, ksrs::ws_words_dev(cap_marks, 3)))) return rc;
      if ((rc = S.d_eo_hitb.alloc(c, cap_marks))) return rc;
      if ((rc = S.d_eo_hseq.alloc(c, cap_marks))) return rc;
      if ((rc = S.d_eo_where.alloc(c, cap_marks))) return rc;
      if ((rc = S.d_eo_bits_a.alloc(c, cap_marks / 64 + 2))) return rc;
      if ((rc = S.d_eo_bits_b.alloc(c, cap_marks / 64 + 2))) return rc;
      S.eo_cap_marks = cap_marks;
    }
    if ((rc = S.d_eo_xnode.reserve(c, 2 * cap_x, 2 * cap_x))) return rc;
  }
  c->eo_cap_marks = cap_marks;
  c->eo_cap_x = cap_x;
  ++c->buffers_epoch;
  HIPCHK(c, hipStreamSynchronize(c->stream));
  return KS_OK;
}
int ensure_exact_points(ks_ctx* c, size_t cap) {
  if (!c->eo_device) return KS_OK;
  int rc;
  for (int i = 0; i < (c->cfg.pipeline_frames ? c->n_slots : 1); ++i) {
    FrameSlot& S = c->slot[i];
    for (DevBuf<uint32_t>* p : {&S.d_eo_cnt_b, &S.d_eo_ux, &S.d_eo_dirty, &S.d_eo_list[0], &S.d_eo_list[1], &S.d_eo_chg, &S.d_eo_consulted, &S.d_eo_lp})
      if ((rc = p->alloc(c, cap))) return rc;
    if ((rc = S.d_eo_bt.alloc(c, cap / kScanBlock + 2))) return rc;
    if ((rc = S.d_eo_btp.alloc(c, cap / kScanBlock + 2))) return rc;
    if ((rc = S.d_eo_rinfo.alloc(c, cap))) return rc;
    if ((rc = S.d_eo_ckpt.alloc(c, 3 * cap))) return rc;
  }
  return KS_OK;
}
EoView eo_view(ks_ctx* c, const FrameSlot& S) {
  EoView E{};
  E.F = S.d_F;
  E.ray_list = S.d_ray_list;
  E.rays = S.d_rays;
  E.C = S.d_counters;
  E.cnt_a = S.d_cnt;
  E.cnt_b = S.d_eo_cnt_b;
  E.ux = S.d_eo_ux;
  E.dirty = S.d_eo_dirty;
  E.keys = S.d_eo_keys[1];
  E.vals = S.d_eo_vals[1];
  E.bits_a = S.d_eo_bits_a;
  E.bits_b = S.d_eo_bits_b;
  E.lp = S.d_eo_lp;
  E.bt = S.d_eo_bt;
  E.btp = S.d_eo_btp;
  E.keys0 = S.d_eo_keys[0];
  E.vals0 = S.d_eo_vals[0];
  E.cap_marks = (unsigned long long)S.eo_cap_marks;
  E.hitb = S.d_eo_hitb;
  E.hseq_w = S.d_eo_hseq;
  E.wide = S.wide ? 1u : 0u;
  E.live = S.d_live;
  E.hseq = S.d_eo_hseq;
  E.where = S.d_eo_where;
  E.rinfo = S.d_eo_rinfo;
  E.ckpt = S.d_eo_ckpt;
  E.tab = S.d_eo_tab;
  E.xnode = S.d_eo_xnode;
  E.cap_x = (uint32_t)(S.d_eo_xnode.size() / 2);
  E.list[0] = S.d_eo_list[0];
  E.list[1] = S.d_eo_list[1];
  E.chg = S.d_eo_chg;
  E.consulted = S.d_eo_consulted;
  E.plain = c->d_eo_plain;
  E.committed = c->d_eo_committed;
  E.ctl = S.d_eo_ctl;
  return E;
}
void enqueue_sweeps(ks_ctx* c, const EoBatch& Bt, uint32_t nb, int count, hipStream_t st) {
  const size_t n = c->cap_points;
  const size_t waves = (size_t)order_chains_cap(c->cfg.integration_order_mode, n) *
                       ((order_generations_cap(c->cfg.integration_order_mode, n) + kEoSweepSegment - 1) / kEoSweepSegment);
  const uint32_t grid = (uint32_t)std::min<size_t>((waves + 3) / 4, 1 << 16);
  for (int i = 0; i < count; ++i) {
    hipLaunchKernelGGL(k_eo2_sweep, dim3(grid, nb), dim3(256), 0, st, Bt);
    hipLaunchKernelGGL(k_eo2_sweep_next, dim3(nb), dim3(64), 0, st, Bt);
  }
}
int enqueue_exact_rounds(ks_ctx* c, FrameSlot* const* slots, uint32_t nb, hipStream_t st) {
  const size_t n = c->cap_points;
  const uint32_t nb4k = (uint32_t)((n + kScanBlock - 1) / kScanBlock);
  const size_t lds = (size_t)nb4k * sizeof(unsigned long long);
  EoBatch Bt{};
  ksrs::DevBatch<uint64_t> Rs{};
  const FrameSlot& S0 = *slots[0];
  for (uint32_t k = 0; k < nb; ++k) {
    const FrameSlot& S = *slots[k];
    Bt.v[k] = eo_view(c, S);
    Rs.keys_a[k] = S.d_eo_keys[0];
    Rs.keys_b[k] = S.d_eo_keys[1];
    Rs.vals_a[k] = S.d_eo_vals[0];
    Rs.vals_b[k] = S.d_eo_vals[1];
    Rs.n_dev[k] = (const unsigned long long*)&S.d_eo_ctl->st.n_marks;
    Rs.ws[k] = S.d_eo_sort_ws;
  }
  hipLaunchKernelGGL(k_eo2_begin, dim3(nb), dim3(64), 0, st, Bt);
  const uint32_t gm = (uint32_t)std::min<size_t>((S0.eo_cap_marks + 255) / 256, 2048);
  const uint32_t gn = (uint32_t)std::min<size_t>((n + 255) / 256, 2048);
  if (S0.wide) {
    hipLaunchKernelGGL(k_eo2_full, dim3(gn, nb), dim3(256), 0, st, Bt);
    hipLaunchKernelGGL(k_eo2_scan, dim3(nb4k, nb), dim3(1024), 0, st, Bt);
    hipLaunchKernelGGL(k_eo2_emit<8>, dim3((uint32_t)((n + 31) / 32), nb), dim3(256), lds, st, Bt);
    HIPCHK(c, ksrs::sort_dev_batch<uint64_t>(Rs, (int)nb, S0.d_eo_sort_ws.size(), S0.eo_cap_marks, 44, 64, st));
    hipLaunchKernelGGL(k_eo2_bits, dim3(gm, nb), dim3(256), 0, st, Bt, 0u);
    hipLaunchKernelGGL(k_eo2_where, dim3(gm, nb), dim3(256), 0, st, Bt);
    enqueue_sweeps(c, Bt, nb, c->eo_sweeps, st);
    return KS_OK;
  } else {
    hipLaunchKernelGGL(k_eo2_scan, dim3(nb4k, nb), dim3(1024), 0, st, Bt);
    hipLaunchKernelGGL(k_eo2_emit<64>, dim3((uint32_t)((n + 255) / 256), nb), dim3(256), lds, st, Bt);
    HIPCHK(c, ksrs::sort_dev_batch<uint64_t>(Rs, (int)nb, S0.d_eo_sort_ws.size(), S0.eo_cap_marks, 44, 64, st));
    hipLaunchKernelGGL(k_eo2_hits, dim3(gm, nb), dim3(256), 0, st, Bt);
    hipLaunchKernelGGL(k_eo2_stop0, dim3(gn, nb), dim3(256), 0, st, Bt);
    hipLaunchKernelGGL(k_eo2_bits, dim3(gm, nb), dim3(256), 0, st, Bt, 1u);
  }
  const uint32_t gr = (uint32_t)std::min<size_t>((n + 3) / 4, 2048);
  for (int r = 1; r <= c->eo_bulk_rounds; ++r) {
    const uint32_t g = S0.wide ? gr : std::min(gr, r == 1 ? 2048u : r == 2 ? 1024u : r <= 4 ? 512u : 256u);
    hipLaunchKernelGGL(k_eo2_eval, dim3(g, nb), dim3(256), 0, st, Bt, (uint32_t)r);
    hipLaunchKernelGGL(k_eo2_propagate, dim3(g, nb), dim3(256), 0, st, Bt, (uint32_t)r);
  }
  return KS_OK;
}
void enqueue_exact_finish(ks_ctx* c, FrameSlot& S, hipStream_t st) {
  const EoView E = eo_view(c, S);
  hipLaunchKernelGGL(k_eo2_finish, dim3(1), dim3(kEoFinishThreads), 0, st, E, (uint32_t)c->eo_bulk_rounds + 1u, 1u);
  hipLaunchKernelGGL(k_eo2_commit, dim3(1024), dim3(256), 0, st, E);
}

template <typename Enqueue> hipGraphExec_t capture_graph(hipStream_t sm, Enqueue enqueue) {
  hipGraph_t g = nullptr;
  hipGraphExec_t out = nullptr;
  bool ok = hipStreamBeginCapture(sm, hipStreamCaptureModeRelaxed) == hipSuccess;
  if (ok) {
    const int rc = enqueue();
    ok = hipStreamEndCapture(sm, &g) == hipSuccess && g != nullptr && rc == KS_OK;
  }
  if (ok) ok = hipGraphInstantiate(&out, g, nullptr, nullptr, 0) == hipSuccess;
  if (g) (void)hipGraphDestroy(g);
  return ok ? out : nullptr;
}
struct BatchLaunch {
  ks_ctx* c;
  FrameSlot* const* slots;
  uint32_t nb;
  FrameSlot& S0;
  hipStream_t sm;
  const BatchView& V;
  size_t steps_max;
  uint64_t key;
  FrameSlot::GraphSet& G;
  int sweeps_host_driven() const {
    EoBatch Bt{};
    for (uint32_t k = 0; k < nb; ++k) Bt.v[k] = eo_view(c, *slots[k]);
    for (int chunk = 1;; ++chunk) {
      bool going = false;
      for (uint32_t k = 0; k < nb; ++k) {
        uint32_t w[2] = {0u, 0u};
        HIPCHK(c, hipMemcpyAsync(&w[0], &slots[k]->d_eo_ctl->sw_prev, sizeof(uint32_t), hipMemcpyDeviceToHost, sm));
        HIPCHK(c, hipMemcpyAsync(&w[1], &slots[k]->d_eo_ctl->fail, sizeof(uint32_t), hipMemcpyDeviceToHost, sm));
        HIPCHK(c, hipStreamSynchronize(sm));
        going = going || (w[0] != 0u && w[1] == 0u);
      }
      if (!going || chunk >= c->eo_sweep_chunks) break;
      enqueue_sweeps(c, Bt, nb, c->eo_sweeps, sm);
    }
    hipLaunchKernelGGL(k_eo2_sweep_done, dim3(nb), dim3(64), 0, sm, Bt);
    return KS_OK;
  }
  int exact_device() const {
    int rc;
    auto seed_and_rounds = [&] {
      enqueue_stage_b(c, V, nb, S0.wide, sm, steps_max, 1);
      return enqueue_exact_rounds(c, slots, nb, sm);
    };
    auto finish = [&] {
      for (uint32_t k = 0; k < nb; ++k) enqueue_exact_finish(c, *slots[k], sm);
      return KS_OK;
    };
    auto emission = [&] { return enqueue_stage_b(c, V, nb, S0.wide, sm, steps_max, 2), KS_OK; };
    bool graphs = c->use_graphs && !S0.wide;
    if (graphs && (G.key != key || !G.g1 || !G.g2 || !G.g3)) {
      std::lock_guard<std::mutex> cap(c->capture_mu);
      G.reset();
      if ((G.g1 = capture_graph(sm, seed_and_rounds)) && (G.g2 = capture_graph(sm, finish)) && (G.g3 = capture_graph(sm, emission))) {
        G.key = key;
      } else {
        (void)hipGetLastError();
        G.reset();
        c->use_graphs = graphs = false;
      }
    }
    if (graphs) HIPCHK(c, hipGraphLaunch(G.g1, sm));
    else if ((rc = seed_and_rounds()) || (S0.wide && (rc = sweeps_host_driven()))) return rc;
    if (c->eo_last_commit && c->eo_last_commit != S0.eo_committed) HIPCHK(c, hipStreamWaitEvent(sm, c->eo_last_commit, 0));
    if (graphs) HIPCHK(c, hipGraphLaunch(G.g2, sm));
    else finish();
    HIPCHK(c, hipEventRecord(S0.eo_committed, sm));
    c->eo_last_commit = S0.eo_committed;
    if (graphs) HIPCHK(c, hipGraphLaunch(G.g3, sm));
    else emission();
    return KS_OK;
  }
  int exact_host() const {
    enqueue_stage_b(c, V, nb, S0.wide, sm, steps_max, 1);
    if (int rc = exact_early_out(c, S0, sm)) return rc;
    enqueue_stage_b(c, V, nb, S0.wide, sm, steps_max, 2);
    return KS_OK;
  }
  int plain_or_replayed() const {
    if (c->use_graphs && (G.key != key || !G.g1)) {
      std::lock_guard<std::mutex> cap(c->capture_mu);
      G.reset();
      if ((G.g1 = capture_graph(sm, [&] { return enqueue_stage_b(c, V, nb, S0.wide, sm, steps_max), KS_OK; }))) {
        G.key = key;
      } else {
        (void)hipGetLastError();
        c->use_graphs = false;
      }
    }
    if (c->use_graphs && G.g1) HIPCHK(c, hipGraphLaunch(G.g1, sm));
    else enqueue_stage_b(c, V, nb, S0.wide, sm, steps_max);
    return KS_OK;
  }
};

int launch_batch(ks_ctx* c) {
  if (c->batch_slots.empty()) return KS_OK;
  std::vector<FrameSlot*> slots;
  slots.swap(c->batch_slots);
  const uint32_t nb = (uint32_t)slots.size();
  FrameSlot& S0 = *slots[0];
  hipStream_t sm = c->batch > 1 ? c->stream_march_[(S0.frame_no / (uint64_t)c->batch) % (uint64_t)c->n_march] : march_stream(c, S0.frame_no);
  c->prof_march_stream = sm;
  if (sm != c->stream) HIPCHK(c, hipStreamWaitEvent(sm, slots[nb - 1]->a_done, 0));
  const bool stage_events = nb == 1 && S0.prof_set >= 0 && c->pset[S0.prof_set].stages;
  if (stage_events) (void)hipEventRecord(c->pset[S0.prof_set].ev[4], sm);
  BatchView V{};
  size_t steps_max = 0;
  ParamsBatch PB{};
  for (uint32_t k = 0; k < nb; ++k) {
    FrameSlot& S = *slots[k];
    S.F.observed = observed_table(c, S.frame_no);
    if (c->exact_early_out) S.F.eo_frame = c->eo_frame_no++;
    PB.F[k] = S.F;
    PB.out[k] = S.d_F;
    V.s[k] = slot_view(S);
    steps_max = std::max(steps_max, S.steps_max);
  }
  if (nb == 1) hipLaunchKernelGGL(k_set_params, dim3(1), dim3(64), 0, sm, slots[0]->F, slots[0]->d_F);
  else hipLaunchKernelGGL(k_set_params_batch, dim3(nb), dim3(64), 0, sm, PB);
  const uint64_t key = ((uint64_t)c->cap_points << 24) ^ (c->buffers_epoch.load() << 4) ^ (S0.wide ? 1u : 0u) ^ ((uint64_t)nb << 1);
  const BatchLaunch B{c, slots.data(), nb, S0, sm, V, steps_max, key, S0.b_graphs[nb == (uint32_t)c->batch ? 0 : 1]};
  if (int rc = !c->exact_early_out ? B.plain_or_replayed() : c->eo_device && !c->eo_device_off ? B.exact_device() : B.exact_host()) return rc;
  for (uint32_t k = 0; k < nb; ++k) {
    HIPCHK(c, hipEventRecord(slots[k]->ready, sm));
    slots[k]->b_launched = true;
  }
  if (stage_events) (void)hipEventRecord(c->pset[S0.prof_set].ev[5], sm);
  return KS_OK;
}

void fill_frame_params(ks_ctx* c, FrameParams& F, const float Tq[7], size_t n, int freespace) {
  const ks_config& cfg = c->cfg;
  F = FrameParams{};
  F.T.w = Tq[0];
  F.T.v = {Tq[1], Tq[2], Tq[3]};
  F.T.t = {Tq[4], Tq[5], Tq[6]};
  F.voxel_size_inv = c->voxel_size_inv;
  F.min_ray = cfg.min_ray_length_m;
  F.max_ray = cfg.max_ray_length_m;
  F.trunc = cfg.truncation_distance;
  F.start_inv = cfg.start_voxel_subsampling_factor * c->voxel_size_inv;
  F.log_match = c->log_match;
  F.log_non_match = c->log_non_match;
  F.tsdf.voxel_size = cfg.voxel_size;
  F.tsdf.trunc = cfg.truncation_distance;
  F.tsdf.max_weight = cfg.max_weight;
  F.tsdf.dropoff_denominator = cfg.truncation_distance - cfg.voxel_size;
  F.tsdf.sparsity_factor = cfg.sparsity_compensation_factor;
  F.tsdf.use_dropoff = cfg.use_weight_dropoff;
  F.tsdf.use_sparsity = cfg.use_sparsity_compensation_factor;
  F.start_offset = c->start_offset;
  F.observed_offset = c->observed_offset;
  F.obs_tag = c->obs_tag;
  F.obs_tag_lo = c->obs_tag_lo;
  F.max_collisions = cfg.max_consecutive_ray_collisions;
  F.n = (uint32_t)n;
  const uint32_t q = (uint32_t)(n / kOrderStep);
  const bool by_1024 = cfg.integration_order_mode == KS_ORDER_MIXED_1024_GROUPS;
  F.order_groups = q == 0 ? 1u : by_1024 ? kOrderStep : q;
  F.order_per = q == 0 ? 0u : by_1024 ? q : kOrderStep;
  F.chains = order_chains(cfg.integration_order_mode, n);
  F.carving = cfg.voxel_carving_enabled;
  F.allow_clear = cfg.allow_clear;
  F.freespace = freespace;
  F.use_const_weight = cfg.use_const_weight;
  F.method = cfg.method;
  F.color_mode = cfg.color_mode;
  F.sorted_order = cfg.integration_order_mode == KS_ORDER_SORTED;
  F.n_dynamic = cfg.n_dynamic_labels;
  const unsigned pb = bits_for(n);
  F.point_mask = (1u << pb) - 1u;
  F.clear_bit = (cfg.method == KS_METHOD_MERGED) ? (1u << pb) : 0u;
  F.seq_bits = pb + (cfg.method == KS_METHOD_MERGED ? 1u : 0u);
  F.inv_order = F.sorted_order ? c->d_inv_order : nullptr;
  std::memcpy(F.dynamic_labels, cfg.dynamic_labels, 32);
  F.early_out = c->uses_early_out;
}
void begin_prof_set(ks_ctx* c, FrameSlot& S, size_t n) {
  const int set = (int)(c->frame_no % kProfSets);
  resolve_prof(c, set);
  ProfSet& P = c->pset[set];
  P.used = true;
  P.complete = P.applied = false;
  P.stages = c->profiling == 1;
  P.apply = c->profiling == 1 || (c->frame_no % 4) == 0;
  P.n_points = n;
  P.n_pairs = 0;
  S.prof_set = set;
}
int stage_a_fast(ks_ctx* c, FrameSlot& S, const float* d_xyz, const uint8_t* d_rgba, const uint8_t* d_labels, size_t n) {
  const FrameParams& F = S.F;
  hipStream_t st = c->stream;
  const uint32_t nb1k = (uint32_t)((n + 1023) / 1024);
  hipLaunchKernelGGL(k_points_fast, dim3(nb1k), dim3(1024), 0, st, F, d_xyz, d_rgba, d_labels, c->d_color_lut,
                     S.d_rays, c->d_hash, c->d_skeys32, c->d_pvals, S.d_cnt, S.d_live, S.d_counters);
  stage_mark(c, S.prof_set, 1);
  uint32_t *sk = nullptr, *sv = nullptr;
  if (int rc = sort_pairs(c, c->d_skeys32.get(), c->d_skeys32b.get(), c->d_pvals.get(), c->d_pvals2.get(), n, kSetBits + 1, &sk, &sv)) return rc;
  stage_mark(c, S.prof_set, 2);
  hipLaunchKernelGGL(k_dedup, dim3(nb1k), dim3(1024), 0, st, F, sk, sv, c->d_hash, c->d_start_set, S.d_ray_list, S.d_rays, S.d_cnt, S.d_live, S.d_counters);
  if (c->uses_early_out && n > 0) {
    const uint32_t n_gen = (uint32_t)((n + F.chains - 1) / F.chains);
    uint32_t n_ph = 0;
    while (n_ph < c->seed_phases.size() && c->seed_phases[n_ph].g0 < n_gen) ++n_ph;
    HIPCHK(c, hipMemsetAsync(S.d_seed_n, 0, c->seed_phases.size() * sizeof(uint32_t), st));
    hipLaunchKernelGGL(k_seed_list, dim3((F.chains + 63u) / 64u, n_ph), dim3(64 * kSeedSegs), 0, st, F, (const SeedPhase*)c->d_seed_phases,
                       (const uint8_t*)S.d_live, S.d_seed_gen, S.d_seed_items, S.d_seed_n, S.d_counters);
  }
  hipLaunchKernelGGL(k_dedup_commit, dim3(nb1k), dim3(1024), 0, st, F, sk, sv, c->d_hash, c->d_start_set, S.d_counters);
  return KS_OK;
}
void enqueue_bundle_order(ks_ctx* c, hipStream_t st, size_t n, const uint64_t* sk, const uint32_t* sv) {
  const uint32_t capb = (uint32_t)((c->cap_points + kBoBlock - 1) / kBoBlock);
  const size_t lds_f = (2 * c->cap_points / kBoBlock + 3) * sizeof(uint32_t), lds_e = ((size_t)capb + 2) * sizeof(uint32_t);
  hipLaunchKernelGGL(k_bo_scan_flags, dim3((uint32_t)((2 * n + kBoBlock - 1) / kBoBlock)), dim3(kBoBlock), 0, st, (uint32_t)n, c->bo);
  hipLaunchKernelGGL(k_bo_init, dim3((uint32_t)((n + kBoBlock - 1) / kBoBlock)), dim3(kBoBlock), lds_f, st, (uint32_t)n, sk, sv, c->bo);
  const uint32_t nbb = (uint32_t)((n + kBoBlock - 1) / kBoBlock);
  int e_small = 0;
  while (e_small < c->bo_epochs && c->bo_sched.b[e_small] <= kBoSmallBuckets) ++e_small;
  if (e_small > 0) hipLaunchKernelGGL(k_bo_small, dim3(2), dim3(kBoBlock), 0, st, c->bo, e_small);
  const size_t nh_floor = c->bo_hint_fixed ? (e_small > 0 ? (size_t)c->bo_sched.t[e_small - 1] + 1 : 1) : 2 * (size_t)kBoSmallBuckets;
  const size_t nh = std::min<size_t>(n, std::max<size_t>(c->bo_hint.load(std::memory_order_relaxed), nh_floor));
  int e_last = -1;
  for (int e = e_small; e <= c->bo_epochs; ++e) {
    if (e > 0 && c->bo_sched.t[e - 1] >= nh) break;
    hipLaunchKernelGGL(k_bo_link, dim3(nbb, 2), dim3(kBoBlock), lds_e, st, c->bo, e, (e == e_small && e_small > 0) ? 1 : 0);
    if (e < c->bo_epochs && c->bo_sched.t[e] < nh)
      hipLaunchKernelGGL(k_bo_walk, dim3(nbb, 2), dim3(kBoBlock), 0, st, c->bo, e);
    else
      e_last = e;
  }
  if (nh < n && e_last >= 0 && e_last < c->bo_epochs) hipLaunchKernelGGL(k_bo_rest, dim3(2), dim3(kBoBlock), lds_e, st, c->bo, e_last);
}
int stage_a_merged(ks_ctx* c, FrameSlot& S, const float* d_xyz, const uint8_t* d_rgba, const uint8_t* d_labels, size_t n, const uint32_t* order_ptr) {
  const ks_config& cfg = c->cfg;
  FrameParams& F = S.F;
  hipStream_t st = c->stream;
  const uint32_t nb = (uint32_t)((n + 255) / 256);
  const uint32_t nb1k = (uint32_t)((n + 1023) / 1024);
  if (c->key_bits) {
    const float reach = cfg.max_ray_length_m + 2.0f * cfg.voxel_size;
    const float tq[3] = {F.T.t.x, F.T.t.y, F.T.t.z};
    for (int a = 0; a < 3; ++a) {
      const float lo = std::floor((tq[a] - reach) * c->voxel_size_inv) - 2.0f;
      F.key_base[a] = (int32_t)std::min(std::max(lo, -2.0e9f), 2.0e9f);
    }
    F.key_bits = c->key_bits;
  }
  hipLaunchKernelGGL(k_points_merged, dim3(nb1k), dim3(1024), 0, st, F, d_xyz, d_rgba, d_labels, c->d_color_lut, c->d_pkeys, c->d_skeys32, c->d_pvals,
                     S.d_cnt, c->use_bundle_rank ? c->bo.flag : nullptr, c->d_key_overflow, c->key_overflow_mask, S.d_counters);
  stage_mark(c, S.prof_set, 1);
  uint64_t* sk = nullptr;
  uint32_t *sk32 = nullptr, *sv = nullptr;
  if (c->key_bits) {
    if (int rc = sort_pairs(c, c->d_skeys32.get(), c->d_skeys32b.get(), c->d_pvals.get(), c->d_pvals2.get(), n, 32, &sk32, &sv)) return rc;
    sk = c->d_pkeys;
  } else {
    if (int rc = sort_pairs(c, c->d_pkeys.get(), c->d_pkeys2.get(), c->d_pvals.get(), c->d_pvals2.get(), n, 64, &sk, &sv)) return rc;
  }
  stage_mark(c, S.prof_set, 2);
  hipLaunchKernelGGL(k_gather_sorted, dim3(nb), dim3(256), 0, st, F, d_xyz, d_rgba, d_labels, c->d_color_lut,
                     order_ptr, (const uint64_t*)sk, (const uint32_t*)sk32, sk, sv, c->d_gpw, c->d_glc, c->use_bundle_rank ? c->bo.flag : nullptr, c->d_blong,
                     c->d_key_overflow, S.d_counters);
  if (c->use_bundle_rank) enqueue_bundle_order(c, st, n, sk, sv);
  uint64_t* ray_keys = cfg.enable_anti_grazing ? S.d_rkeys : nullptr;
  if (cfg.enable_anti_grazing) HIPCHK(c, hipMemcpyAsync(S.d_gkeys, sk, n * sizeof(uint64_t), hipMemcpyDeviceToDevice, st));
  const uint32_t n_long_blocks = (uint32_t)std::min<size_t>(n / kLongRun + 1, 512);
  hipLaunchKernelGGL(k_bundles_all, dim3(n_long_blocks + (uint32_t)((n + 127) / 128)), dim3(128), 0, st, F, sk, sv, c->d_gpw, c->d_glc, c->d_blong,
                     S.d_rays, S.d_deltas, S.d_ray_list, ray_keys, S.d_cnt, c->bo, c->use_bundle_rank, S.d_counters, n_long_blocks);
  if (cfg.enable_anti_grazing) {
    F.grazing_keys = S.d_gkeys;
    F.ray_keys = S.d_rkeys;
  }
  return KS_OK;
}
int frame_front(ks_ctx* c, FrameSlot& S, const float Tq[7], const float* d_xyz, const uint8_t* d_rgba, const uint8_t* d_labels, size_t n, int freespace) {
  int rc;
  FrameParams& F = S.F;
  fill_frame_params(c, F, Tq, n, freespace);
  const size_t steps_max = steps_max_of(c->cfg, c->voxel_size_inv);
  S.wide = steps_max > 400;
  const size_t hint = c->pairs_hint.load(std::memory_order_relaxed);
// ... 1654 lines not shown
    c->esdf_changed.clear();
    return KS_OK;
  }
  if (workspace > max_workspace_bytes) {
    c->err = "ks_esdf_refresh: " + std::to_string(nz) + " tiles to recompute need " + std::to_string(workspace) +
             " bytes of work space, more than max_workspace_bytes = " + std::to_string(max_workspace_bytes);
    return KS_ERR_UNSUPPORTED;
  }
  if (nx >= (1ull << 31) || ny >= (1ull << 31)) {
    c->err = "ks_esdf_refresh: too many tiles for one call";
    return KS_ERR_UNSUPPORTED;
  }
  DevBuf<EsdfRecord> grown;
  if ((size_t)nt * kTileVoxels > c->esdf_store.size())
    if ((rc = grown.alloc(c, ((size_t)nt + nt / 2 + 64) * kTileVoxels))) return rc;
  if ((rc = c->esdf_bricks[0].reserve(c, nx * kEsdfBrickKeys, (nx + nx / 2) * kEsdfBrickKeys)) ||
      (rc = c->esdf_bricks[1].reserve(c, ny * kEsdfBrickKeys, (ny + ny / 2) * kEsdfBrickKeys)) ||
      (rc = c->esdf_lists.reserve(c, nx + ny + nz, (nx + ny + nz) * 3 / 2)) || (rc = c->esdf_zslots.reserve(c, nz, nz * 3 / 2)) ||
      (rc = c->esdf_counters.reserve(c, 3, 3)))
    return rc;
  c->esdf_valid = false;
  if (grown.get()) {
    if (nt_old) HIPCHK(c, hipMemcpyAsync(grown.get(), c->esdf_store.get(), (size_t)nt_old * kTileVoxels * sizeof(EsdfRecord), hipMemcpyDeviceToDevice, st));
    HIPCHK(c, hipStreamSynchronize(st));
    c->esdf_store = std::move(grown);
  }
  if (nt > nt_old)
    hipLaunchKernelGGL(k_esdf_fill, dim3((uint32_t)(((size_t)(nt - nt_old) * kTileVoxels + 255) / 256)), dim3(256), 0, st,
                       c->esdf_store.get() + (size_t)nt_old * kTileVoxels, (size_t)(nt - nt_old) * kTileVoxels);
  unsigned long long counts[3] = {c->esdf_totals[0], c->esdf_totals[1], c->esdf_totals[2]};
  if (nz) {
    uint64_t* d_x = c->esdf_lists.get();
    uint64_t *d_y = d_x + nx, *d_z = d_y + ny;
    if (nx) HIPCHK(c, hipMemcpyAsync(d_x, L.X.data(), nx * 8, hipMemcpyHostToDevice, st));
    if (ny) HIPCHK(c, hipMemcpyAsync(d_y, L.Y.data(), ny * 8, hipMemcpyHostToDevice, st));
    HIPCHK(c, hipMemcpyAsync(d_z, L.Z.data(), nz * 8, hipMemcpyHostToDevice, st));
    HIPCHK(c, hipMemcpyAsync(c->esdf_zslots, L.z_slots.data(), nz * 4, hipMemcpyHostToDevice, st));
    HIPCHK(c, hipMemsetAsync(c->esdf_counters, 0, 3 * sizeof(unsigned long long), st));
    EsdfRefresh E{R, c->cfg.voxel_size, e.min_weight, e.min_distance_m, e.max_distance_m};
    if (nx)
      hipLaunchKernelGGL(k_esdf_brick<0>, dim3((uint32_t)nx), dim3(256), 0, st, E, c->table, c->pool, nt, (const uint64_t*)d_x,
                         (const uint64_t*)nullptr, 0u, (const uint64_t*)nullptr, c->esdf_bricks[0].get(), (const uint32_t*)nullptr,
                         (EsdfRecord*)nullptr);
    if (ny)
      hipLaunchKernelGGL(k_esdf_brick<1>, dim3((uint32_t)ny), dim3(256), 0, st, E, c->table, c->pool, nt, (const uint64_t*)d_y,
                         (const uint64_t*)d_x, (uint32_t)nx, (const uint64_t*)c->esdf_bricks[0].get(), c->esdf_bricks[1].get(),
                         (const uint32_t*)nullptr, (EsdfRecord*)nullptr);
    hipLaunchKernelGGL(k_esdf_brick<2>, dim3((uint32_t)nz), dim3(256), 0, st, E, c->table, c->pool, nt, (const uint64_t*)d_z,
                       (const uint64_t*)d_y, (uint32_t)ny, (const uint64_t*)c->esdf_bricks[1].get(), (uint64_t*)nullptr,
                       (const uint32_t*)c->esdf_zslots.get(), c->esdf_store.get());
    const size_t nrec = (size_t)nt * kTileVoxels;
    hipLaunchKernelGGL(k_esdf_count, dim3((uint32_t)((nrec + 1023) / 1024)), dim3(256), 0, st, (const EsdfRecord*)c->esdf_store.get(), nrec,
                       e.max_distance_m, c->esdf_counters.get());
    HIPCHK(c, hipMemcpyAsync(counts, c->esdf_counters, sizeof(counts), hipMemcpyDeviceToHost, st));
  }
  hipLaunchKernelGGL(k_stale_clear, dim3((nt + 255) / 256), dim3(256), 0, st, c->pool.mesh_stale(), nt, kStaleEsdf);
  HIPCHK(c, hipStreamSynchronize(st));
  HIPCHK(c, hipGetLastError());
  c->esdf_valid = true;
  c->esdf_tiles = nt;
  for (int k = 0; k < 3; ++k) c->esdf_totals[k] = counts[k];
  words_to_triples(blocks_of_tiles(L.Z, c->vps_shift), &c->esdf_changed);
  if (stats) {
    stats->voxels_observed = counts[0];
    stats->voxels_fixed = counts[1];
    stats->voxels_clamped = counts[2];
  }
  return KS_OK;
}

int ks_esdf_changed_blocks(ks_ctx* c, int32_t* out_xyz, size_t cap, size_t* n) {
  return c ? copy_block_list(c, "ks_esdf_changed_blocks", c->esdf_changed, out_xyz, cap, n) : KS_ERR_INVALID_ARG;
}

int ks_esdf_download_blocks(ks_ctx* c, const int32_t* idx, size_t n, void* out) {
  if (!c || (n && (!idx || !out))) return KS_ERR_INVALID_ARG;
  if (int rc = esdf_ready(c, "ks_esdf_download_blocks")) return rc;
  if (n == 0) return KS_OK;
  if (int rc = quiesce(c)) return rc;
  const int vps = c->cfg.voxels_per_side;
  const size_t nv = (size_t)vps * vps * vps;
  const size_t chunk = std::min<size_t>(std::max<size_t>(1, (size_t(64) << 20) / (nv * sizeof(EsdfRecord))), 65535);
  const size_t m_max = std::min(chunk, n);
  int rc;
  if ((rc = c->esdf_out.reserve(c, m_max * nv, m_max * nv))) return rc;
  if ((rc = c->esdf_idx.reserve(c, m_max * 3, m_max * 3))) return rc;
  for (size_t off = 0; off < n; off += m_max) {
    const size_t m = std::min(m_max, n - off);
    HIPCHK(c, hipMemcpyAsync(c->esdf_idx, idx + 3 * off, m * 3 * sizeof(int32_t), hipMemcpyHostToDevice, c->stream));
    hipLaunchKernelGGL(k_esdf_download, dim3((uint32_t)((nv + 255) / 256), (uint32_t)m), dim3(256), 0, c->stream, c->table,
                       (const EsdfRecord*)c->esdf_store.get(), c->esdf_tiles, (const int32_t*)c->esdf_idx.get(), vps, c->esdf_out.get());
    HIPCHK(c, hipMemcpyAsync((uint8_t*)out + off * nv * sizeof(EsdfRecord), c->esdf_out, m * nv * sizeof(EsdfRecord), hipMemcpyDeviceToHost, c->stream));
    HIPCHK(c, hipStreamSynchronize(c->stream));
  }
  HIPCHK(c, hipGetLastError());
  return KS_OK;
}

int ks_esdf_query(ks_ctx* c, const float* xyz, size_t n, float* distance, uint8_t* flags, uint8_t* label) {
  if (!c || (n && !xyz)) return KS_ERR_INVALID_ARG;
  if (int rc = esdf_ready(c, "ks_esdf_query")) return rc;
  if (n == 0) return KS_OK;
  if (int rc = quiesce(c)) return rc;
  const size_t chunk = size_t(1) << 22;
  const size_t m_max = std::min(chunk, n);
  int rc;
  if ((rc = c->esdf_out.reserve(c, m_max, m_max))) return rc;
  if ((rc = c->esdf_xyz.reserve(c, m_max * 3, m_max * 3))) return rc;
  std::vector<EsdfRecord> rec(m_max);
  for (size_t off = 0; off < n; off += m_max) {
    const size_t m = std::min(m_max, n - off);
    HIPCHK(c, hipMemcpyAsync(c->esdf_xyz, xyz + 3 * off, m * 3 * sizeof(float), hipMemcpyHostToDevice, c->stream));
    hipLaunchKernelGGL(k_esdf_query, dim3((uint32_t)((m + 255) / 256)), dim3(256), 0, c->stream, c->table, (const EsdfRecord*)c->esdf_store.get(),
                       c->esdf_tiles, (const float*)c->esdf_xyz.get(), m, c->voxel_size_inv, c->esdf_out.get());
    HIPCHK(c, hipMemcpyAsync(rec.data(), c->esdf_out, m * sizeof(EsdfRecord), hipMemcpyDeviceToHost, c->stream));
    HIPCHK(c, hipStreamSynchronize(c->stream));
    for (size_t i = 0; i < m; ++i) {
      if (distance) distance[off + i] = rec[i].distance;
      if (flags) flags[off + i] = (uint8_t)(rec[i].tail & 0xffu);
      if (label) label[off + i] = (uint8_t)((rec[i].tail >> 8) & 0xffu);
    }
  }
  HIPCHK(c, hipGetLastError());
  return KS_OK;
}

int ks_render_default_config(ks_render_config* r) {
  if (!r) return KS_ERR_INVALID_ARG;
  r->min_weight = 1e-4f;
  r->min_range_m = 0.1f;
  r->max_range_m = 10.0f;
  return KS_OK;
}

static int render_enqueue(ks_ctx* c, const char* who, const float T[7], const float K[4], int width, int height, const ks_render_config* r,
                          float* d_depth, uint8_t* d_labels, uint8_t* d_rgba, float* d_normals) {
  auto refuse = [&](const char* why) {
    c->err = std::string(who) + ": " + why;
    return KS_ERR_INVALID_ARG;
  };
  if (width < 1 || width > 8192 || height < 1 || height > 8192) return refuse("width and height must lie in 1..8192");
  for (int k = 0; k < 4; ++k)
    if (!std::isfinite(K[k])) return refuse("K must be finite");
  if (!(K[0] > 0.0f) || !(K[1] > 0.0f)) return refuse("fx and fy must be positive");
  const float par[3] = {r->min_weight, r->min_range_m, r->max_range_m};
  for (float v : par)
    if (!std::isfinite(v) || !(v > 0.0f)) return refuse("min_weight, min_range_m and max_range_m must be finite positive numbers");
  if (r->min_range_m >= r->max_range_m) return refuse("min_range_m must be below max_range_m");
  if (r->max_range_m / c->cfg.voxel_size > 4096.0f) return refuse("max_range_m is more than 4096 voxels");
  if (!d_depth && !d_labels && !d_rgba && !d_normals) return refuse("all four outputs are NULL");
  if (int rc = holds_voxels(c, who)) return rc;
  if (int rc = quiesce(c)) return rc;
  if (int rc = c->render_counters.reserve(c, 3, 3)) return rc;
  RenderView V{};
  V.T.w = T[0];
  V.T.v = {T[1], T[2], T[3]};
  V.T.t = {T[4], T[5], T[6]};
  V.cx = K[2];
  V.cy = K[3];
  V.constant_x = (float)(1.0 / (double)K[0]);
  V.constant_y = (float)(1.0 / (double)K[1]);
  V.width = width;
  V.height = height;
  V.voxel_size = c->cfg.voxel_size;
  V.voxel_size_inv = c->voxel_size_inv;
  V.min_weight = r->min_weight;
  V.min_range = r->min_range_m;
  V.max_range = r->max_range_m;
  V.n_tiles = c->tiles_initialised;
  V.depth = d_depth;
  V.labels = d_labels;
  V.rgba = (uint32_t*)d_rgba;
  V.normals = d_normals;
  V.counters = c->render_counters;
  HIPCHK(c, hipMemsetAsync(c->render_counters, 0, 3 * sizeof(unsigned long long), c->stream));
  hipLaunchKernelGGL(k_render_view, dim3((uint32_t)((width + 15) / 16), (uint32_t)((height + 15) / 16)), dim3(256), 0, c->stream, c->table, c->pool, V);
  HIPCHK(c, hipGetLastError());
  return KS_OK;
}

static int render_stats(ks_ctx* c, ks_render_stats* stats) {
  unsigned long long counts[3] = {0, 0, 0};
  HIPCHK(c, hipMemcpyAsync(counts, c->render_counters, sizeof(counts), hipMemcpyDeviceToHost, c->stream));
  HIPCHK(c, hipStreamSynchronize(c->stream));
  stats->pixels_hit = counts[0];
  stats->pixels_missed = counts[1];
  stats->samples = counts[2];
  return KS_OK;
}

int ks_render_view_device(ks_ctx* c, const float T[7], const float K[4], int width, int height, const ks_render_config* r, float* d_depth,
                          uint8_t* d_labels, uint8_t* d_rgba, float* d_normals, ks_render_stats* stats) {
  if (!c || !T || !K || !r) return KS_ERR_INVALID_ARG;
  if (stats) std::memset(stats, 0, sizeof(*stats));
  if (int rc = render_enqueue(c, "ks_render_view_device", T, K, width, height, r, d_depth, d_labels, d_rgba, d_normals)) return rc;
  return stats ? render_stats(c, stats) : KS_OK;
}

int ks_render_view(ks_ctx* c, const float T[7], const float K[4], int width, int height, const ks_render_config* r, float* depth,
                   uint8_t* labels, uint8_t* rgba, float* normals, ks_render_stats* stats) {
  if (!c || !T || !K || !r) return KS_ERR_INVALID_ARG;
  if (stats) std::memset(stats, 0, sizeof(*stats));
  const size_t n = width > 0 && height > 0 && width <= 8192 && height <= 8192 ? (size_t)width * (size_t)height : 0;
  int rc;
  if (n && depth && (rc = c->render_depth.reserve(c, n, n))) return rc;
  if (n && labels && (rc = c->render_labels.reserve(c, n, n))) return rc;
  if (n && rgba && (rc = c->render_rgba.reserve(c, n, n))) return rc;
  if (n && normals && (rc = c->render_normals.reserve(c, 3 * n, 3 * n))) return rc;
  if ((rc = render_enqueue(c, "ks_render_view", T, K, width, height, r, depth ? c->render_depth.get() : nullptr,
                           labels ? c->render_labels.get() : nullptr, rgba ? (uint8_t*)c->render_rgba.get() : nullptr,
                           normals ? c->render_normals.get() : nullptr)))
    return rc;
  hipStream_t st = c->stream;
  if (depth) HIPCHK(c, hipMemcpyAsync(depth, c->render_depth, n * sizeof(float), hipMemcpyDeviceToHost, st));
  if (labels) HIPCHK(c, hipMemcpyAsync(labels, c->render_labels, n, hipMemcpyDeviceToHost, st));
  if (rgba) HIPCHK(c, hipMemcpyAsync(rgba, c->render_rgba, n * 4, hipMemcpyDeviceToHost, st));
  if (normals) HIPCHK(c, hipMemcpyAsync(normals, c->render_normals, 3 * n * sizeof(float), hipMemcpyDeviceToHost, st));
  if (stats) return render_stats(c, stats);
  HIPCHK(c, hipStreamSynchronize(st));
  return KS_OK;
}

static void* device_view_of_pinned(void* p) {
  hipPointerAttribute_t a;
  if (hipPointerGetAttributes(&a, p) != hipSuccess) {
    (void)hipGetLastError();
    return nullptr;
  }
  return a.type == hipMemoryTypeHost ? a.devicePointer : nullptr;
}

static int updated_voxels_impl(ks_ctx* c, void* out, size_t cap, size_t* n, bool count_only, ks_voxel_run* runs, size_t cap_runs,
                               size_t* n_runs) {
  if (!c || !n) return KS_ERR_INVALID_ARG;
  *n = 0;
  if (n_runs) *n_runs = 0;
  if (int rc = quiesce(c)) return rc;
  const uint32_t nt = c->tiles_initialised;
  if (nt == 0) return KS_OK;
  int rc;
  if ((rc = ensure_exchange(c, (size_t)nt + 8))) return rc;
  uint32_t* d_cnt = c->d_xchg_u32;
  uint32_t* d_list = c->d_xchg_u32 + 8;
  hipStream_t st = c->stream;
  HIPCHK(c, hipMemsetAsync(d_cnt, 0, 8 * sizeof(uint32_t), st));
  hipLaunchKernelGGL(k_list_updated_tiles, dim3((nt + 255) / 256), dim3(256), 0, st, c->pool, nt, d_list, d_cnt);
  uint32_t h_cnt[2] = {0, 0};
  HIPCHK(c, hipMemcpyAsync(h_cnt, d_cnt, sizeof(uint32_t), hipMemcpyDeviceToHost, st));
  HIPCHK(c, hipStreamSynchronize(st));
  const uint32_t n_list = h_cnt[0];
  if (n_list == 0) return KS_OK;
  if (n_runs) *n_runs = n_list;
  hipLaunchKernelGGL(k_export_dirty, dim3(n_list), dim3(512), 0, st, c->table, c->pool, (const uint32_t*)d_list,
                     (const uint32_t*)c->d_label_lut, c->vps_shift, 1, d_cnt, (uint8_t*)nullptr, (uint32_t*)nullptr);
  HIPCHK(c, hipMemcpyAsync(h_cnt, d_cnt, 2 * sizeof(uint32_t), hipMemcpyDeviceToHost, st));
  HIPCHK(c, hipStreamSynchronize(st));
  *n = h_cnt[1];
  if (count_only || h_cnt[1] == 0) return KS_OK;
  if ((size_t)h_cnt[1] > cap) {
    c->err = "ks_download_updated_voxels: output buffer too small (call ks_count_updated_voxels first)";
    return KS_ERR_INVALID_ARG;
  }
  if (runs && (size_t)n_list > cap_runs) {
    c->err = "ks_download_updated_voxels: run buffer too small";
    return KS_ERR_INVALID_ARG;
  }
  uint8_t* rec_direct = (uint8_t*)device_view_of_pinned(out);
  uint32_t* run_direct = runs ? (uint32_t*)device_view_of_pinned(runs) : nullptr;
  const size_t bytes = (size_t)h_cnt[1] * kVoxRecBytes;
  const size_t run_bytes = (size_t)n_list * sizeof(ks_voxel_run);
  const size_t need = (rec_direct ? 0 : bytes + bytes / 4) + (run_direct ? 0 : 2 * run_bytes) + 64;
  if ((!rec_direct || (runs && !run_direct)) && (rc = c->d_vox_out.reserve(c, need, need))) return rc;
  uint8_t* d_rec = rec_direct ? rec_direct : c->d_vox_out;
  uint32_t* d_runs = run_direct ? run_direct : (uint32_t*)(c->d_vox_out.get() + (rec_direct ? 0 : ((bytes + 15) & ~(size_t)15)));
  HIPCHK(c, hipMemsetAsync(d_cnt + 1, 0, sizeof(uint32_t), st));
  hipLaunchKernelGGL(k_export_dirty, dim3(n_list), dim3(512), 0, st, c->table, c->pool, (const uint32_t*)d_list,
                     (const uint32_t*)c->d_label_lut, c->vps_shift, 0, d_cnt, d_rec, runs ? d_runs : (uint32_t*)nullptr);
  if (!rec_direct) HIPCHK(c, hipMemcpyAsync(out, c->d_vox_out, bytes, hipMemcpyDeviceToHost, st));
  if (runs && !run_direct) HIPCHK(c, hipMemcpyAsync(runs, d_runs, run_bytes, hipMemcpyDeviceToHost, st));
  HIPCHK(c, hipStreamSynchronize(st));
  HIPCHK(c, hipGetLastError());
  return KS_OK;
}

int ks_count_updated_voxels(ks_ctx* c, size_t* n, size_t* n_runs) {
  return updated_voxels_impl(c, nullptr, 0, n, true, nullptr, 0, n_runs);
}
int ks_download_updated_voxels(ks_ctx* c, void* out, size_t cap, size_t* n, ks_voxel_run* runs, size_t cap_runs, size_t* n_runs) {
  if (!out && cap) return KS_ERR_INVALID_ARG;
  static_assert(sizeof(ks_voxel_run) == 20, "run record layout");
  return updated_voxels_impl(c, out, cap, n, false, runs, cap_runs, n_runs);
}

void* ks_host_alloc(size_t bytes) {
  void* p = nullptr;
  if (hipHostMalloc(&p, std::max<size_t>(bytes, 1), hipHostMallocDefault) != hipSuccess) return nullptr;
  return p;
}

void ks_host_free(void* p) {
  if (p) (void)hipHostFree(p);
}

int ks_debug_radix_sort(ks_ctx* c, void* keys, uint32_t* vals, size_t n, int key_bits, unsigned end_bit) {
  if (!c || (n && !keys) || (key_bits != 32 && key_bits != 64)) return KS_ERR_INVALID_ARG;
  if (n == 0) return KS_OK;
  const size_t kb = key_bits / 8;
  DevBuf<uint8_t> ka, kbuf;
  DevBuf<uint32_t> va, vb;
  int rc;
  if ((rc = ka.alloc(c, n * kb)) || (rc = kbuf.alloc(c, n * kb))) return rc;
  HIPCHK(c, hipMemcpy(ka, keys, n * kb, hipMemcpyHostToDevice));
  if (vals) {
    if ((rc = va.alloc(c, n)) || (rc = vb.alloc(c, n))) return rc;
    HIPCHK(c, hipMemcpy(va, vals, n * 4, hipMemcpyHostToDevice));
  }
  void* kres = nullptr;
  uint32_t* vres = nullptr;
  if (key_bits == 32) {
    uint32_t* r = nullptr;
    rc = vals ? sort_pairs(c, (uint32_t*)ka.get(), (uint32_t*)kbuf.get(), va.get(), vb.get(), n, end_bit, &r, &vres)
              : sort_keys(c, (uint32_t*)ka.get(), (uint32_t*)kbuf.get(), n, end_bit, &r);
    kres = r;
  } else {
    uint64_t* r = nullptr;
    rc = vals ? sort_pairs(c, (uint64_t*)ka.get(), (uint64_t*)kbuf.get(), va.get(), vb.get(), n, end_bit, &r, &vres)
              : sort_keys(c, (uint64_t*)ka.get(), (uint64_t*)kbuf.get(), n, end_bit, &r);
    kres = r;
  }
  if (rc) return rc;
  HIPCHK(c, hipStreamSynchronize(c->stream));
  HIPCHK(c, hipMemcpy(keys, kres, n * kb, hipMemcpyDeviceToHost));
  if (vals) HIPCHK(c, hipMemcpy(vals, vres, n * 4, hipMemcpyDeviceToHost));
  return KS_OK;
}

int ks_get_tile_keys(ks_ctx* c, uint64_t* out, size_t cap, size_t* n) {
  if (!c || !n) return KS_ERR_INVALID_ARG;
  if (int rc = quiesce(c)) return rc;
  HIPCHK(c, hipStreamSynchronize(c->stream));
  *n = c->tiles_initialised;
  const size_t m = std::min<size_t>(cap, *n);
  if (out && m) HIPCHK(c, hipMemcpy(out, c->table.slot_keys, m * sizeof(uint64_t), hipMemcpyDeviceToHost));
  return KS_OK;
}

int ks_export_tiles_device(ks_ctx* c, const uint32_t* slots, size_t n, void* d_payload) {
  if (!c || (n && (!slots || !d_payload))) return KS_ERR_INVALID_ARG;
  if (n == 0) return KS_OK;
  if (int rc = quiesce(c)) return rc;
  for (size_t i = 0; i < n; ++i)
    if (slots[i] >= c->tiles_initialised) return KS_ERR_INVALID_ARG;
  if (int rc = ensure_exchange(c, n)) return rc;
  HIPCHK(c, hipMemcpyAsync(c->d_xchg_u32, slots, n * sizeof(uint32_t), hipMemcpyHostToDevice, c->stream));
  hipLaunchKernelGGL(k_export_tiles, dim3((uint32_t)n), dim3(512), 0, c->stream, c->pool, c->d_xchg_u32, (uint4*)d_payload);
  HIPCHK(c, hipStreamSynchronize(c->stream));
  return KS_OK;
}

int ks_merge_tiles_device(ks_ctx* c, const uint64_t* keys, size_t n, const void* d_payload) {
  if (!c || (n && (!keys || !d_payload))) return KS_ERR_INVALID_ARG;
  if (n == 0) return KS_OK;
  if (c->fatal) return KS_ERR_INVALID_ARG;
  std::vector<uint32_t> order(n);
  for (size_t i = 0; i < n; ++i) order[i] = (uint32_t)i;
  std::stable_sort(order.begin(), order.end(), [&](uint32_t a, uint32_t b) { return keys[a] < keys[b]; });
  std::vector<uint64_t> ukeys;
  std::vector<uint32_t> offs;
  for (size_t i = 0; i < n; ++i) {
    if (i == 0 || keys[order[i]] != keys[order[i - 1]]) {
      ukeys.push_back(keys[order[i]]);
      offs.push_back((uint32_t)i);
    }
  }
  offs.push_back((uint32_t)n);
  const size_t nu = ukeys.size();
  int rc;
  if ((rc = quiesce(c))) return rc;
  if ((rc = ensure_exchange(c, n + 1))) return rc;
  uint32_t* d_offs = c->d_xchg_u32;
  uint32_t* d_idx = c->d_xchg_u32 + (nu + 1);
  HIPCHK(c, hipMemcpyAsync(c->d_xchg_u64, ukeys.data(), nu * sizeof(uint64_t), hipMemcpyHostToDevice, c->stream));
  HIPCHK(c, hipMemcpyAsync(d_offs, offs.data(), (nu + 1) * sizeof(uint32_t), hipMemcpyHostToDevice, c->stream));
  HIPCHK(c, hipMemcpyAsync(d_idx, order.data(), n * sizeof(uint32_t), hipMemcpyHostToDevice, c->stream));
  if ((rc = insert_tiles(c, c->d_xchg_u64, nu))) return rc;
  switch (c->cfg.color_mode) {
    case KS_COLOR_MODE_COLOR:
      hipLaunchKernelGGL(k_merge_tiles<KS_COLOR_MODE_COLOR>, dim3((uint32_t)nu), dim3(512), 0, c->stream, c->table, c->pool,
                         c->d_xchg_u64, d_offs, d_idx, (const uint4*)d_payload, c->cfg.max_weight, c->d_label_lut);
      break;
    case KS_COLOR_MODE_SEMANTIC:
      hipLaunchKernelGGL(k_merge_tiles<KS_COLOR_MODE_SEMANTIC>, dim3((uint32_t)nu), dim3(512), 0, c->stream, c->table,
                         c->pool, c->d_xchg_u64, d_offs, d_idx, (const uint4*)d_payload, c->cfg.max_weight, c->d_label_lut);
      break;
    default:
      hipLaunchKernelGGL(k_merge_tiles<KS_COLOR_MODE_SEMANTIC_PROBABILITY>, dim3((uint32_t)nu), dim3(512), 0, c->stream,
                         c->table, c->pool, c->d_xchg_u64, d_offs, d_idx, (const uint4*)d_payload, c->cfg.max_weight,
                         c->d_label_lut);
      break;
  }
  HIPCHK(c, hipStreamSynchronize(c->stream));
  HIPCHK(c, hipGetLastError());
  return KS_OK;
}

int ks_reset_tiles(ks_ctx* c, const uint32_t* slots, size_t n) {
  if (!c || (n && !slots)) return KS_ERR_INVALID_ARG;
  if (n == 0) return KS_OK;
  if (int rc = quiesce(c)) return rc;
  for (size_t i = 0; i < n; ++i)
    if (slots[i] >= c->tiles_initialised) return KS_ERR_INVALID_ARG;
  if (int rc = ensure_exchange(c, n)) return rc;
  HIPCHK(c, hipMemcpyAsync(c->d_xchg_u32, slots, n * sizeof(uint32_t), hipMemcpyHostToDevice, c->stream));
  hipLaunchKernelGGL(k_reset_tiles, dim3((uint32_t)n), dim3(512), 0, c->stream, c->pool, c->d_xchg_u32);
  HIPCHK(c, hipStreamSynchronize(c->stream));
  return KS_OK;
}

namespace {
struct RcclApi {
  void* h = nullptr;
  decltype(&ncclAllGather) all_gather = nullptr;
  decltype(&ncclSend) send = nullptr;
  decltype(&ncclRecv) recv = nullptr;
  decltype(&ncclGroupStart) group_start = nullptr;
  decltype(&ncclGroupEnd) group_end = nullptr;
  decltype(&ncclGetErrorString) err_string = nullptr;
  bool load(std::string* why) {
    if (h) return true;
    const char* env = getenv("KS_RCCL_LIB");
    const char* names[] = {env, "librccl.so.1", "librccl.so", "/opt/rocm/lib/librccl.so.1"};
    for (const char* nm : names) {
      if (!nm) continue;
      h = dlopen(nm, RTLD_NOW | RTLD_LOCAL);
      if (h) break;
    }
    if (!h) { *why = "librccl not found (set KS_RCCL_LIB)"; return false; }
    all_gather = (decltype(all_gather))dlsym(h, "ncclAllGather");
    send = (decltype(send))dlsym(h, "ncclSend");
    recv = (decltype(recv))dlsym(h, "ncclRecv");
    group_start = (decltype(group_start))dlsym(h, "ncclGroupStart");
    group_end = (decltype(group_end))dlsym(h, "ncclGroupEnd");
    err_string = (decltype(err_string))dlsym(h, "ncclGetErrorString");
    if (!all_gather || !send || !recv || !group_start || !group_end) { *why = "librccl lacks a required symbol"; h = nullptr; return false; }
    return true;
  }
};
RcclApi g_rccl;

inline uint64_t splitmix64(uint64_t x) {
  x += 0x9E3779B97F4A7C15ull;
  x = (x ^ (x >> 30)) * 0xBF58476D1CE4E5B9ull;
  x = (x ^ (x >> 27)) * 0x94D049BB133111EBull;
  return x ^ (x >> 31);
}
}

#define NCCLCHK(ctx, expr)                                                                                    \
  do {                                                                                                        \
    ncclResult_t r_ = (expr);                                                                                 \
    if (r_ != ncclSuccess) {                                                                                  \
      (ctx)->err = std::string(#expr) + ": " + (g_rccl.err_string ? g_rccl.err_string(r_) : "rccl error");    \
      return KS_ERR_HIP;                                                                                      \
    }                                                                                                         \
  } while (0)

int ks_tile_owner(uint64_t tile_key, int world) { return world > 0 ? (int)(splitmix64(tile_key) % (uint64_t)world) : 0; }

static int ensure_reduce_scratch(ks_ctx* c, size_t n_send, size_t n_recv, int world) {
  int rc;
  if ((rc = c->d_rx_counts.reserve(c, (size_t)(world + 3) * world, (size_t)(world + 3) * world))) return rc;
  if (n_send > c->cap_tx) {
    const size_t cap = std::max<size_t>(n_send + n_send / 2, 64);
    c->cap_tx = 0;
    if ((rc = c->d_tx_keys.alloc(c, cap))) return rc;
    if ((rc = c->d_tx_slots.alloc(c, cap))) return rc;
    if ((rc = c->d_tx_payload.alloc(c, cap * (size_t)KS_TILE_BYTES))) return rc;
    c->cap_tx = cap;
  }
  if (n_recv > c->cap_rx) {
    const size_t cap = std::max<size_t>(n_recv + n_recv / 2, 64);
    c->cap_rx = 0;
    if ((rc = c->d_rx_keys.alloc(c, cap))) return rc;
    if ((rc = c->d_rx_payload.alloc(c, cap * (size_t)KS_TILE_BYTES))) return rc;
    c->cap_rx = cap;
  }
  return KS_OK;
}

int ks_reduce(ks_ctx* c, void* rccl_comm, int rank, int world, ks_reduce_stats* stats) {
  if (!c || world < 1 || rank < 0 || rank >= world || (world > 1 && !rccl_comm)) return KS_ERR_INVALID_ARG;
  if (stats) std::memset(stats, 0, sizeof(*stats));
  if (c->fatal) return KS_ERR_INVALID_ARG;
  int rc;
  if ((rc = quiesce(c))) return rc;
  const uint32_t nt = c->tiles_initialised;
  if (stats) stats->tiles_local = nt;
  hipStream_t st = c->stream;
  if (world == 1) {
    if (nt) HIPCHK(c, hipMemsetAsync(c->pool.dirty, 0, nt, st));
    HIPCHK(c, hipStreamSynchronize(st));
    return KS_OK;
  }
  std::string why;
  if (!g_rccl.load(&why)) {
    c->err = why;
    return KS_ERR_UNSUPPORTED;
  }
  ncclComm_t comm = (ncclComm_t)rccl_comm;
  if ((rc = ensure_reduce_scratch(c, 0, 0, world))) return rc;
  int32_t* d_own = c->d_rx_counts;
  int32_t* d_all = d_own + world;
  uint32_t* d_offs = (uint32_t*)(d_all + (size_t)world * world);
  uint32_t* d_cursor = d_offs + world;
  HIPCHK(c, hipMemsetAsync(d_own, 0, (size_t)(world + 3) * world * sizeof(int32_t), st));
  const uint32_t nb = (nt + 255) / 256;
  if (nt)
    hipLaunchKernelGGL(k_dirty_by_owner, dim3(nb), dim3(256), 0, st, c->pool, (const uint64_t*)c->table.slot_keys, nt, (uint32_t)rank,
                       (uint32_t)world, 0, d_own, (const uint32_t*)nullptr, (uint32_t*)nullptr, (uint32_t*)nullptr, (uint64_t*)nullptr);
  NCCLCHK(c, g_rccl.all_gather(d_own, d_all, (size_t)world, ncclInt32, comm, st));
  std::vector<int32_t> all_counts((size_t)world * world);
  HIPCHK(c, hipMemcpyAsync(all_counts.data(), d_all, all_counts.size() * sizeof(int32_t), hipMemcpyDeviceToHost, st));
  HIPCHK(c, hipStreamSynchronize(st));
  std::vector<size_t> send_counts(world), recv_counts(world), recv_off(world + 1, 0), send_off(world + 1, 0);
  for (int p = 0; p < world; ++p) {
    send_counts[p] = (size_t)all_counts[(size_t)rank * world + p];
    recv_counts[p] = (size_t)all_counts[(size_t)p * world + rank];
    send_off[p + 1] = send_off[p] + send_counts[p];
    recv_off[p + 1] = recv_off[p] + recv_counts[p];
  }
  const size_t n_send = send_off[world], n_recv = recv_off[world];
  if ((rc = ensure_reduce_scratch(c, n_send, n_recv, world))) return rc;
  if (n_send) {
    std::vector<uint32_t> offs32(world);
    for (int p = 0; p < world; ++p) offs32[p] = (uint32_t)send_off[p];
    HIPCHK(c, hipMemcpyAsync(d_offs, offs32.data(), world * sizeof(uint32_t), hipMemcpyHostToDevice, st));
    hipLaunchKernelGGL(k_dirty_by_owner, dim3(nb), dim3(256), 0, st, c->pool, (const uint64_t*)c->table.slot_keys, nt, (uint32_t)rank,
                       (uint32_t)world, 1, d_own, (const uint32_t*)d_offs, d_cursor, c->d_tx_slots, c->d_tx_keys);
    hipLaunchKernelGGL(k_export_tiles, dim3((uint32_t)n_send), dim3(512), 0, st, c->pool, (const uint32_t*)c->d_tx_slots,
                       (uint4*)c->d_tx_payload.get());
    HIPCHK(c, hipStreamSynchronize(st));
  }
  NCCLCHK(c, g_rccl.group_start());
  for (int peer = 0; peer < world; ++peer) {
    if (peer == rank) continue;
    if (send_counts[peer]) {
      NCCLCHK(c, g_rccl.send(c->d_tx_keys + send_off[peer], send_counts[peer], ncclUint64, peer, comm, st));
      NCCLCHK(c, g_rccl.send(c->d_tx_payload + send_off[peer] * (size_t)KS_TILE_BYTES, send_counts[peer] * (size_t)KS_TILE_BYTES,
                             ncclUint8, peer, comm, st));
    }
    if (recv_counts[peer]) {
      NCCLCHK(c, g_rccl.recv(c->d_rx_keys + recv_off[peer], recv_counts[peer], ncclUint64, peer, comm, st));
      NCCLCHK(c, g_rccl.recv(c->d_rx_payload + recv_off[peer] * (size_t)KS_TILE_BYTES, recv_counts[peer] * (size_t)KS_TILE_BYTES,
                             ncclUint8, peer, comm, st));
    }
  }
  NCCLCHK(c, g_rccl.group_end());
  std::vector<uint64_t> k_host(n_recv);
  if (n_recv) HIPCHK(c, hipMemcpyAsync(k_host.data(), c->d_rx_keys, n_recv * 8, hipMemcpyDeviceToHost, st));
  HIPCHK(c, hipStreamSynchronize(st));
  if (n_recv && (rc = ks_merge_tiles_device(c, k_host.data(), n_recv, c->d_rx_payload))) return rc;
  if (n_send) hipLaunchKernelGGL(k_reset_tiles, dim3((uint32_t)n_send), dim3(512), 0, st, c->pool, (const uint32_t*)c->d_tx_slots);
  HIPCHK(c, hipMemsetAsync(c->pool.dirty, 0, c->tiles_initialised, st));
  HIPCHK(c, hipStreamSynchronize(st));
  if (stats) {
    stats->tiles_sent = n_send;
    stats->tiles_received = n_recv;
    stats->bytes_sent = n_send * (uint64_t)(KS_TILE_BYTES + 8);
  }
  return KS_OK;
}

struct ShardTables {
  const float2* btab;
  uint32_t n_bundles;
  const float* mixed;
  uint32_t n_mixed;
};
static int shard_apply_segment(ks_ctx* o, const uint64_t* d_gkey, const uint32_t* d_seq, const float* d_sdf, const float* d_uw, size_t n,
                               size_t tiles_at_most, const ShardTables* mt = nullptr) {
  if (n == 0) return KS_OK;
  if (n >= (size_t)1 << 31) { o->err = "ks_integrate_round_exact: more than 2^31 updates of one frame for one owner"; return KS_ERR_INVALID_ARG; }
  int rc;
  if (n > o->cap_sh_rx) {
    const size_t cap = std::max<size_t>(n + n / 4, 1 << 18);
    o->cap_sh_rx = 0;
    if ((rc = o->d_sh_tk.alloc(o, cap))) return rc;
    for (int b = 0; b < 2; ++b) {
      if ((rc = o->d_sh_pairs[b].alloc(o, cap))) return rc;
      if ((rc = o->d_sh_vals[b].alloc(o, cap))) return rc;
    }
    o->cap_sh_rx = cap;
  }
  if (mt && n > o->cap_shm_ops) {
    const size_t cap = std::max<size_t>(n + n / 4, 1 << 18);
    o->cap_shm_ops = 0;
    if ((rc = o->d_shm_ops.alloc(o, cap))) return rc;
    if ((rc = o->d_shm_long.alloc(o, cap / (kLongRun + 1) + 2))) return rc;
    o->cap_shm_ops = cap;
  }
  hipStream_t st = o->stream;
  const uint32_t nb = (uint32_t)((n + 255) / 256);
  hipLaunchKernelGGL(k_shard_tile_keys, dim3(nb), dim3(256), 0, st, (uint32_t)n, d_gkey, o->d_sh_tk);
  if ((rc = insert_tiles(o, o->d_sh_tk, n, tiles_at_most))) return rc;
  hipLaunchKernelGGL(k_shard_import, dim3(nb), dim3(256), 0, st, (uint32_t)n, o->table, o->pool, d_gkey, d_seq, o->d_sh_pairs[0], o->d_sh_vals[0]);
  const unsigned end_bit = kShardSeqBits + 9 + bits_for(o->tiles_initialised);
  uint64_t* kres = nullptr;
  uint32_t* vres = nullptr;
  HIPCHK(o, (ksrs::sort<uint64_t, true>(o->sort_ws, o->d_sh_pairs[0], o->d_sh_pairs[1], o->d_sh_vals[0], o->d_sh_vals[1], n, std::min(56u, end_bit), st,
                                        &kres, &vres, kShardSeqBits)));
  FrameParams F{};
  const ks_config& cfg = o->cfg;
  F.log_match = o->log_match;
  F.log_non_match = o->log_non_match;
  F.tsdf.voxel_size = cfg.voxel_size;
  F.tsdf.trunc = cfg.truncation_distance;
  F.tsdf.max_weight = cfg.max_weight;
  F.tsdf.dropoff_denominator = cfg.truncation_distance - cfg.voxel_size;
  F.tsdf.sparsity_factor = cfg.sparsity_compensation_factor;
  F.tsdf.use_dropoff = cfg.use_weight_dropoff;
  F.tsdf.use_sparsity = cfg.use_sparsity_compensation_factor;
  if (mt) {
    uint32_t* const d_n_long = o->d_shm_long + (o->cap_shm_ops / (kLongRun + 1) + 1);
    HIPCHK(o, hipMemsetAsync(d_n_long, 0, sizeof(uint32_t), st));
    hipLaunchKernelGGL(k_shard_stage_merged, dim3(nb), dim3(256), 0, st, (uint32_t)n, mt->n_bundles, (const uint64_t*)kres, (const uint32_t*)vres, d_sdf,
                       d_uw, mt->btab, o->d_shm_ops, o->d_shm_long, d_n_long);
    const uint32_t lb = (uint32_t)std::min<size_t>(2 * (n / (kLongRun + 1) + 1), 4096);
#define KS_LAUNCH_SHARD_MERGED(MODE)                                                                                                         \
  hipLaunchKernelGGL(k_shard_apply_merged<MODE>, dim3(nb), dim3(256), 0, st, F.tsdf, (uint32_t)n, mt->n_mixed, (const uint64_t*)kres,         \
                     (const float4*)o->d_shm_ops, mt->mixed, o->pool, (const uint32_t*)o->d_label_lut);                                      \
  hipLaunchKernelGGL(k_shard_apply_merged_long<MODE>, dim3(lb), dim3(64), 0, st, F.tsdf, (uint32_t)n, mt->n_mixed, (const uint64_t*)kres,     \
                     (const float4*)o->d_shm_ops, mt->mixed, o->pool, (const uint32_t*)o->d_label_lut, (const uint32_t*)o->d_shm_long,       \
                     (const uint32_t*)d_n_long)
    if (cfg.color_mode == KS_COLOR_MODE_SEMANTIC) {
      KS_LAUNCH_SHARD_MERGED(KS_COLOR_MODE_SEMANTIC);
    } else {
// ... 404 lines not shown
```

### kimera_semantics_amd/csrc/ks_radix_sort.h

```cpp
#pragma once
#include <hip/hip_runtime.h>
#include <stdint.h>
#include <algorithm>
#include <stdlib.h>

#include "ks_owned.h"

namespace ksrs {

constexpr int kMaxPasses = 8;
constexpr int kMaxBins = 2048;
constexpr size_t kHistBlocks = 2048;
constexpr uint32_t kFlagLocal = 1u << 30, kFlagPrefix = 2u << 30, kCountMask = (1u << 30) - 1u;

template <int RB, typename K>
__device__ __forceinline__ uint32_t digit_of(K key, int shift) {
  return (uint32_t)(key >> shift) & (uint32_t)((1 << RB) - 1);
}

template <int RB>
__device__ __forceinline__ unsigned long long match_digit(uint32_t d, unsigned long long active) {
  unsigned long long peers = active;
#pragma unroll
  for (int b = 0; b < RB; ++b) {
    const bool bit = (d >> b) & 1u;
    const unsigned long long bal = __ballot(bit);
    peers &= bit ? bal : ~bal;
  }
  return peers;
}

template <typename K, int RB>
__device__ __forceinline__ void rs_hist_body(const K* __restrict__ keys, uint32_t n, int passes, int begin_bit,
                                             uint32_t* __restrict__ hist, uint32_t* __restrict__ zero_ptr,
                                             uint32_t zero_words, const unsigned long long* __restrict__ n_dev, uint32_t* s_hist) {
  constexpr int kBins = 1 << RB;
  const uint32_t tid = threadIdx.x, lane = tid & 63u;
  if (n_dev) n = (uint32_t)(*n_dev < (unsigned long long)n ? *n_dev : (unsigned long long)n);
  for (uint32_t i = blockIdx.x * 256u + tid; i < zero_words / 4u; i += gridDim.x * 256u)
    ((uint4*)zero_ptr)[i] = make_uint4(0u, 0u, 0u, 0u);
  for (int i = tid; i < passes * kBins; i += 256) s_hist[i] = 0;
  __syncthreads();
  const uint32_t n_slices = (n + 2047u) / 2048u;
  for (uint32_t slice = blockIdx.x; slice < n_slices; slice += gridDim.x) {
    const uint32_t base = slice * 2048u;
#pragma unroll
    for (int i = 0; i < 8; ++i) {
      const uint32_t idx = base + i * 256 + tid;
      const bool valid = idx < n;
      const K key = valid ? keys[idx] : (K)0;
      const unsigned long long active = __ballot(valid);
      for (int p = 0; p < passes; ++p) {
        const uint32_t d = digit_of<RB>(key, begin_bit + p * RB);
        const uint32_t d0 = (uint32_t)__builtin_amdgcn_readfirstlane((int)d);
        if (__ballot(valid && d != d0) == 0ull) {
          if (active && lane == (uint32_t)(__ffsll((long long)active) - 1))
            atomicAdd(&s_hist[p * kBins + d0], (uint32_t)__popcll(active));
        } else {
          const uint32_t dp = __shfl_up(d, 1);
          const unsigned long long lead = __ballot(valid && (lane == 0u || d != dp));
          if (valid && ((lead >> lane) & 1ull)) {
            const unsigned long long rest = (lane < 63u) ? (lead >> (lane + 1u)) : 0ull;
            const uint32_t stop = rest ? lane + (uint32_t)__ffsll((long long)rest) : 64u;
            const unsigned long long in_run = (stop < 64u ? ((1ull << stop) - 1ull) : ~0ull) & ~((1ull << lane) - 1ull);
            atomicAdd(&s_hist[p * kBins + d], (uint32_t)__popcll(in_run & active));
          }
        }
      }
    }
  }
  __syncthreads();
  for (int i = tid; i < passes * kBins; i += 256) {
    const uint32_t c = s_hist[i];
    if (c) atomicAdd(&hist[(i / kBins) * kMaxBins + (i % kBins)], c);
  }
}
template <typename K, int RB>
__global__ void __launch_bounds__(256) k_rs_hist(const K* __restrict__ keys, uint32_t n, int passes, int begin_bit,
                                                 uint32_t* __restrict__ hist, uint32_t* __restrict__ zero_ptr,
                                                 uint32_t zero_words, const unsigned long long* __restrict__ n_dev = nullptr) {
  extern __shared__ uint32_t s_hist[];
  rs_hist_body<K, RB>(keys, n, passes, begin_bit, hist, zero_ptr, zero_words, n_dev, s_hist);
}
constexpr int kRsBatch = 8;
template <typename K>
struct DevBatch {
  K* keys_a[kRsBatch];
  K* keys_b[kRsBatch];
  uint32_t* vals_a[kRsBatch];
  uint32_t* vals_b[kRsBatch];
  const unsigned long long* n_dev[kRsBatch];
  uint32_t* ws[kRsBatch];
};
template <typename K, int RB>
__global__ void __launch_bounds__(256) k_rs_hist_b(DevBatch<K> B, uint32_t cap, int passes, int begin_bit) {
  extern __shared__ uint32_t s_hist[];
  rs_hist_body<K, RB>(B.keys_a[blockIdx.y], cap, passes, begin_bit, B.ws[blockIdx.y], nullptr, 0u, B.n_dev[blockIdx.y], s_hist);
}

template <typename K, bool HAS_VALUES, int THREADS, int ITEMS, int RB, bool REORDER = false>
__device__ __forceinline__ void rs_pass_body(const K* __restrict__ keys_in, K* __restrict__ keys_out,
                                             const uint32_t* __restrict__ vals_in,
                                             uint32_t* __restrict__ vals_out, uint32_t n, int shift,
                                             const uint32_t* __restrict__ bin_hist,
                                             uint32_t* __restrict__ status, uint32_t* __restrict__ ticket,
                                             const unsigned long long* __restrict__ n_dev) {
  constexpr int kBins = 1 << RB;
  constexpr int kChunks = kBins / 64;
  constexpr int kWaves = THREADS / 64;
  constexpr int kTile = THREADS * ITEMS;
  if (n_dev) n = (uint32_t)(*n_dev < (unsigned long long)n ? *n_dev : (unsigned long long)n);
  __shared__ uint32_t s_cnt[kWaves][kBins];
  __shared__ uint32_t s_off[kBins];
  __shared__ uint32_t s_chunk[kChunks];
  __shared__ uint32_t s_tile;
  __shared__ K s_keys[REORDER ? kTile : 1];
  __shared__ uint32_t s_loc[REORDER ? kBins : 1];
  static_assert(!REORDER || (!HAS_VALUES && kBins <= THREADS), "reorder variant: keys only");
  const uint32_t tid = threadIdx.x, lane = tid & 63u, wave = tid >> 6;
  if (tid == 0) s_tile = ticket ? atomicAdd(ticket, 1u) : blockIdx.x;
  for (int i = tid; i < kWaves * kBins; i += THREADS) (&s_cnt[0][0])[i] = 0;
  __syncthreads();
  const uint32_t tile = s_tile;
  if (n_dev && (unsigned long long)tile * kTile >= (unsigned long long)n) return;
  const uint32_t wbase = tile * kTile + wave * (ITEMS * 64);

  K key[ITEMS];
  uint32_t rd[ITEMS];
#pragma unroll
  for (int i = 0; i < ITEMS; ++i) {
    const uint32_t idx = wbase + i * 64 + lane;
    key[i] = (idx < n) ? keys_in[idx] : (K)0;
  }
#pragma unroll
  for (int i = 0; i < ITEMS; ++i) {
    const uint32_t idx = wbase + i * 64 + lane;
    const bool valid = idx < n;
    const uint32_t d = digit_of<RB>(key[i], shift);
    const unsigned long long peers = match_digit<RB>(d, __ballot(valid));
    const uint32_t prev = s_cnt[wave][d];
    rd[i] = (prev + (uint32_t)__popcll(peers & ((1ull << lane) - 1ull))) | (d << 20);
    __builtin_amdgcn_wave_barrier();
    if (valid && (peers & ((1ull << lane) - 1ull)) == 0ull) s_cnt[wave][d] = prev + (uint32_t)__popcll(peers);
    __builtin_amdgcn_wave_barrier();
  }
  __syncthreads();

  for (int d = tid; d < kBins; d += THREADS) {
    uint32_t total = 0;
#pragma unroll
    for (int w = 0; w < kWaves; ++w) {
      const uint32_t c = s_cnt[w][d];
      s_cnt[w][d] = total;
      total += c;
    }
    if (REORDER) s_loc[d] = total;
    uint32_t* st = status + d;
    uint32_t prefix = 0;
    __hip_atomic_store(st + (size_t)tile * kBins, total | kFlagLocal, __ATOMIC_RELAXED, __HIP_MEMORY_SCOPE_AGENT);
    constexpr int kWindow = 8;
    int t = (int)tile - 1;
    bool done = false;
    while (!done) {
      uint32_t s[kWindow];
#pragma unroll
      for (int j = 0; j < kWindow; ++j)
        s[j] = (t - j >= 0) ? __hip_atomic_load(st + (size_t)(t - j) * kBins, __ATOMIC_RELAXED, __HIP_MEMORY_SCOPE_AGENT)
                            : kFlagPrefix;
      int consumed = 0;
#pragma unroll
      for (int j = 0; j < kWindow; ++j) {
        if (done || consumed != j) continue;
        const uint32_t flag = s[j] >> 30;
        if (flag == 0u) continue;
        prefix += s[j] & kCountMask;
        ++consumed;
        if (flag == 2u) done = true;
      }
      t -= consumed;
    }
    __hip_atomic_store(st + (size_t)tile * kBins, (prefix + total) | kFlagPrefix, __ATOMIC_RELAXED,
                       __HIP_MEMORY_SCOPE_AGENT);
    s_off[d] = prefix;
  }
  __syncthreads();
  for (int c = wave; c < kChunks; c += kWaves) {
    const uint32_t hv = bin_hist[c * 64 + lane];
    uint32_t x = hv;
#pragma unroll
    for (int o = 1; o < 64; o <<= 1) {
      const uint32_t y = __shfl_up(x, o);
      if (lane >= (uint32_t)o) x += y;
    }
    if (lane == 63) s_chunk[c] = x;
    s_off[c * 64 + lane] += x - hv;
  }
  __syncthreads();
  for (int d = tid; d < kBins; d += THREADS) {
    uint32_t add = 0;
    for (int cc = 0; cc < d / 64; ++cc) add += s_chunk[cc];
    s_off[d] += add;
  }
  __syncthreads();

  if (REORDER) {
    __shared__ uint32_t s_lchunk[kChunks];
    for (int c = wave; c < kChunks; c += kWaves) {
      const uint32_t tv = s_loc[c * 64 + lane];
      uint32_t x = tv;
#pragma unroll
      for (int o = 1; o < 64; o <<= 1) {
        const uint32_t y = __shfl_up(x, o);
        if (lane >= (uint32_t)o) x += y;
      }
      if (lane == 63) s_lchunk[c] = x;
      s_loc[c * 64 + lane] = x - tv;
    }
    __syncthreads();
    for (int d = tid; d < kBins; d += THREADS) {
      uint32_t add = 0;
      for (int cc = 0; cc < d / 64; ++cc) add += s_lchunk[cc];
      s_loc[d] += add;
    }
    __syncthreads();
#pragma unroll
    for (int i = 0; i < ITEMS; ++i) {
      const uint32_t idx = wbase + i * 64 + lane;
      if (idx < n) {
        const uint32_t d = rd[i] >> 20;
        s_keys[s_loc[d] + s_cnt[wave][d] + (rd[i] & 0xfffffu)] = key[i];
      }
    }
    __syncthreads();
    const uint32_t t0 = tile * (uint32_t)kTile;
    const uint32_t count = (n - t0 < (uint32_t)kTile) ? n - t0 : (uint32_t)kTile;
    for (uint32_t j = tid; j < count; j += THREADS) {
      const K k = s_keys[j];
      const uint32_t d = digit_of<RB>(k, shift);
      keys_out[s_off[d] + (j - s_loc[d])] = k;
    }
    return;
  }
#pragma unroll
  for (int i = 0; i < ITEMS; ++i) {
    const uint32_t idx = wbase + i * 64 + lane;
    if (idx < n) {
      const uint32_t d = rd[i] >> 20;
      const uint32_t pos = s_off[d] + s_cnt[wave][d] + (rd[i] & 0xfffffu);
      keys_out[pos] = key[i];
      if (HAS_VALUES) vals_out[pos] = vals_in[idx];
    }
  }
}

template <typename K, bool HAS_VALUES, int THREADS, int ITEMS, int RB, bool REORDER = false>
__global__ void __launch_bounds__(THREADS) k_rs_pass(const K* __restrict__ keys_in, K* __restrict__ keys_out,
                                                     const uint32_t* __restrict__ vals_in,
                                                     uint32_t* __restrict__ vals_out, uint32_t n, int shift,
                                                     const uint32_t* __restrict__ bin_hist,
                                                     uint32_t* __restrict__ status, uint32_t* __restrict__ ticket,
                                                     const unsigned long long* __restrict__ n_dev = nullptr) {
  rs_pass_body<K, HAS_VALUES, THREADS, ITEMS, RB, REORDER>(keys_in, keys_out, vals_in, vals_out, n, shift, bin_hist, status, ticket, n_dev);
}
template <typename K, int THREADS, int ITEMS, int RB>
__global__ void __launch_bounds__(THREADS) k_rs_pass_b(DevBatch<K> B, uint32_t cap, int begin_bit, int p, uint32_t tiles) {
  const uint32_t y = blockIdx.y;
  uint32_t* ws = B.ws[y];
  const bool odd = (p & 1) != 0;
  rs_pass_body<K, true, THREADS, ITEMS, RB, false>(odd ? B.keys_b[y] : B.keys_a[y], odd ? B.keys_a[y] : B.keys_b[y], odd ? B.vals_b[y] : B.vals_a[y],
                                                   odd ? B.vals_a[y] : B.vals_b[y], cap, begin_bit + p * RB, ws + (size_t)p * kMaxBins,
                                                   ws + ((size_t)kMaxPasses * kMaxBins + kMaxPasses) + (size_t)p * tiles * (1 << RB),
                                                   ws + (size_t)kMaxPasses * kMaxBins + p, B.n_dev[y]);
}

struct Workspace {
  DevBuf<uint32_t> d_ws;
  size_t words = 0;
  int cur = 0;
  size_t dirty[2] = {0, 0};
};
constexpr size_t kHeadWords = (size_t)kMaxPasses * kMaxBins + kMaxPasses;

inline hipError_t ensure(Workspace& w, size_t words, hipStream_t stream) {
  if (words <= w.words) return hipSuccess;
  w.words = 0;
  const size_t cap = ((words + words / 4) + 3) & ~(size_t)3;
  hipError_t e = w.d_ws.try_alloc(2 * cap);
  if (e != hipSuccess) return e;
  e = hipMemsetAsync(w.d_ws, 0, 2 * cap * sizeof(uint32_t), stream);
  if (e != hipSuccess) return e;
  w.words = cap;
  w.cur = 0;
  w.dirty[0] = w.dirty[1] = 0;
  return hipSuccess;
}

template <typename K, bool HAS_VALUES, int THREADS, int ITEMS, int RB, bool REORDER = false>
inline void launch_passes(Workspace& w, K*& kin, K*& kout, uint32_t*& vin, uint32_t*& vout, size_t n, int passes,
                          uint32_t tiles, unsigned begin_bit, hipStream_t stream) {
  constexpr int kBins = 1 << RB;
  uint32_t* base = w.d_ws + (size_t)w.cur * w.words;
  uint32_t* hist = base;
  uint32_t* tickets = base + (size_t)kMaxPasses * kMaxBins;
  uint32_t* status = base + kHeadWords;
  for (int p = 0; p < passes; ++p) {
    hipLaunchKernelGGL((k_rs_pass<K, HAS_VALUES, THREADS, ITEMS, RB, REORDER>), dim3(tiles), dim3(THREADS), 0, stream, kin, kout,
                       vin, vout, (uint32_t)n, (int)begin_bit + p * RB, hist + (size_t)p * kMaxBins,
                       status + (size_t)p * tiles * kBins, tickets + p);
    K* tk = kin; kin = kout; kout = tk;
    uint32_t* tv = vin; vin = vout; vout = tv;
  }
}

template <typename K, bool HAS_VALUES, int RB>
inline hipError_t sort_rb(Workspace& w, K* keys_a, K* keys_b, uint32_t* vals_a, uint32_t* vals_b, size_t n,
                          unsigned begin_bit, unsigned end_bit, hipStream_t stream, K** keys_result,
                          uint32_t** vals_result) {
  constexpr int kBins = 1 << RB;
  const int passes = (int)((end_bit - begin_bit + RB - 1) / RB);
  const bool reorder = !HAS_VALUES && n > (1u << 20);
  const int tile = (n <= (1u << 20)) ? 2048 : (reorder || n <= (1u << 24)) ? 8192 : 16384;
  const uint32_t tiles = (uint32_t)((n + tile - 1) / tile);
  const size_t words = kHeadWords + (size_t)passes * tiles * kBins;
  hipError_t e = ensure(w, words, stream);
  if (e != hipSuccess) return e;
  const int h = w.cur ^ 1;
  hipLaunchKernelGGL((k_rs_hist<K, RB>), dim3((uint32_t)std::min<size_t>((n + 2047) / 2048, kHistBlocks)), dim3(256),
                     (size_t)passes * kBins * sizeof(uint32_t), stream, keys_a, (uint32_t)n, passes, (int)begin_bit,
                     w.d_ws + (size_t)h * w.words, w.d_ws + (size_t)(h ^ 1) * w.words,
                     (uint32_t)((w.dirty[h ^ 1] + 3) & ~(size_t)3));
  w.dirty[h ^ 1] = 0;
  w.dirty[h] = words;
  w.cur = h;
  K* kin = keys_a;
  K* kout = keys_b;
  uint32_t* vin = vals_a;
  uint32_t* vout = vals_b;
  if (tile == 2048) launch_passes<K, HAS_VALUES, 256, 8, RB>(w, kin, kout, vin, vout, n, passes, tiles, begin_bit, stream);
  else if (tile == 8192 && reorder) {
    if constexpr (!HAS_VALUES) launch_passes<K, false, 512, 16, RB, true>(w, kin, kout, vin, vout, n, passes, tiles, begin_bit, stream);
  } else if (tile == 8192) launch_passes<K, HAS_VALUES, 512, 16, RB>(w, kin, kout, vin, vout, n, passes, tiles, begin_bit, stream);
  else launch_passes<K, HAS_VALUES, 512, 32, RB>(w, kin, kout, vin, vout, n, passes, tiles, begin_bit, stream);
  *keys_result = kin;
  if (vals_result) *vals_result = vin;
  return hipGetLastError();
}

inline size_t dev_tile(size_t cap) { return cap <= (1u << 20) ? 2048 : cap <= (1u << 24) ? 8192 : 16384; }
inline size_t ws_words_dev(size_t cap, int passes) { return kHeadWords + (size_t)passes * ((cap + dev_tile(cap) - 1) / dev_tile(cap)) * 256; }
template <typename K>
inline hipError_t sort_dev(uint32_t* ws, size_t ws_words, K* keys_a, K* keys_b, uint32_t* vals_a, uint32_t* vals_b,
                           const unsigned long long* n_dev, size_t cap, unsigned begin_bit, unsigned end_bit, hipStream_t stream,
                           K** keys_result, uint32_t** vals_result) {
  constexpr int RB = 8;
  constexpr int kBins = 1 << RB;
  const int passes = (int)((end_bit - begin_bit + RB - 1) / RB);
  const size_t tile = dev_tile(cap);
  const uint32_t tiles = (uint32_t)((cap + tile - 1) / tile);
  if (kHeadWords + (size_t)passes * tiles * kBins > ws_words) return hipErrorInvalidValue;
  hipError_t e = hipMemsetAsync(ws, 0, (kHeadWords + (size_t)passes * tiles * kBins) * sizeof(uint32_t), stream);
  if (e != hipSuccess) return e;
  uint32_t* hist = ws;
  uint32_t* tickets = ws + (size_t)kMaxPasses * kMaxBins;
  uint32_t* status = ws + kHeadWords;
  hipLaunchKernelGGL((k_rs_hist<K, RB>), dim3((uint32_t)std::min<size_t>((cap + 2047) / 2048, kHistBlocks)), dim3(256),
                     (size_t)passes * kBins * sizeof(uint32_t), stream, (const K*)keys_a, (uint32_t)cap, passes, (int)begin_bit, hist,
                     (uint32_t*)nullptr, 0u, n_dev);
  K* kin = keys_a;
  K* kout = keys_b;
  uint32_t* vin = vals_a;
  uint32_t* vout = vals_b;
  for (int p = 0; p < passes; ++p) {
#define KS_RS_DEV_PASS(THREADS, ITEMS)                                                                                                 \
  hipLaunchKernelGGL((k_rs_pass<K, true, THREADS, ITEMS, RB>), dim3(tiles), dim3(THREADS), 0, stream, (const K*)kin, kout,             \
                     (const uint32_t*)vin, vout, (uint32_t)cap, (int)begin_bit + p * RB, (const uint32_t*)(hist + (size_t)p * kMaxBins), \
                     status + (size_t)p * tiles * kBins, tickets + p, n_dev)
    if (tile == 2048) KS_RS_DEV_PASS(256, 8);
    else if (tile == 8192) KS_RS_DEV_PASS(512, 16);
    else KS_RS_DEV_PASS(512, 32);
#undef KS_RS_DEV_PASS
    K* tk = kin; kin = kout; kout = tk;
    uint32_t* tv = vin; vin = vout; vout = tv;
  }
  *keys_result = kin;
  *vals_result = vin;
  return hipGetLastError();
}

template <typename K>
inline hipError_t sort_dev_batch(const DevBatch<K>& B, int nb, size_t ws_words, size_t cap, unsigned begin_bit, unsigned end_bit, hipStream_t stream) {
  constexpr int RB = 8;
  constexpr int kBins = 1 << RB;
  const int passes = (int)((end_bit - begin_bit + RB - 1) / RB);
  const size_t tile = dev_tile(cap);
  const uint32_t tiles = (uint32_t)((cap + tile - 1) / tile);
  if (kHeadWords + (size_t)passes * tiles * kBins > ws_words || nb < 1 || nb > kRsBatch) return hipErrorInvalidValue;
  for (int y = 0; y < nb; ++y) {
    hipError_t e = hipMemsetAsync(B.ws[y], 0, (kHeadWords + (size_t)passes * tiles * kBins) * sizeof(uint32_t), stream);
    if (e != hipSuccess) return e;
  }
  hipLaunchKernelGGL((k_rs_hist_b<K, RB>), dim3((uint32_t)std::min<size_t>((cap + 2047) / 2048, kHistBlocks), (uint32_t)nb), dim3(256),
                     (size_t)passes * kBins * sizeof(uint32_t), stream, B, (uint32_t)cap, passes, (int)begin_bit);
  for (int p = 0; p < passes; ++p) {
    if (tile == 2048) hipLaunchKernelGGL((k_rs_pass_b<K, 256, 8, RB>), dim3(tiles, (uint32_t)nb), dim3(256), 0, stream, B, (uint32_t)cap, (int)begin_bit, p, tiles);
    else if (tile == 8192) hipLaunchKernelGGL((k_rs_pass_b<K, 512, 16, RB>), dim3(tiles, (uint32_t)nb), dim3(512), 0, stream, B, (uint32_t)cap, (int)begin_bit, p, tiles);
    else hipLaunchKernelGGL((k_rs_pass_b<K, 512, 32, RB>), dim3(tiles, (uint32_t)nb), dim3(512), 0, stream, B, (uint32_t)cap, (int)begin_bit, p, tiles);
  }
  return hipGetLastError();
}

template <typename K, bool HAS_VALUES>
inline hipError_t sort(Workspace& w, K* keys_a, K* keys_b, uint32_t* vals_a, uint32_t* vals_b, size_t n,
                       unsigned end_bit, hipStream_t stream, K** keys_result, uint32_t** vals_result,
                       unsigned begin_bit = 0) {
  *keys_result = keys_a;
  if (vals_result) *vals_result = vals_a;
  if (end_bit > sizeof(K) * 8) end_bit = (unsigned)(sizeof(K) * 8);
  if (n == 0 || end_bit <= begin_bit) return hipSuccess;
  return sort_rb<K, HAS_VALUES, 8>(w, keys_a, keys_b, vals_a, vals_b, n, begin_bit, end_bit, stream, keys_result, vals_result);
}

}
```

Baseline: 1012 Mvoxel-updates/s.

## Plan radix sort digit width and tile shape per key range

Replaces the fixed 8-bit-digit radix sort with a planner that chooses the digit width (8 or 10 bits), tile shape and pass count from the element count and key bit range. Digits are masked at end_bit so partial final digits are handled correctly. Device and batch sort paths are unified, and callers now ask where the result landed after an odd or even number of passes. The aim is fewer passes over the early-out and pair keys. The cost is wider histograms per pass and more template instantiations, plus new debug entry points for testing.

```diff
diff --git a/include/ks_hip.h b/include/ks_hip.h
--- a/include/ks_hip.h
+++ b/include/ks_hip.h
@@ -195,6 +195,10 @@
                              int freespace_points, ks_round_stats* stats);
 
 int ks_debug_radix_sort(ks_ctx* ctx, void* keys, uint32_t* vals, size_t n, int key_bits, unsigned end_bit);
+int ks_debug_radix_sort_bits(ks_ctx* ctx, void* keys, uint32_t* vals, size_t n, int key_bits, unsigned begin_bit, unsigned end_bit);
+int ks_debug_radix_sort_plan(size_t n, int key_bits, int has_values, unsigned begin_bit, unsigned end_bit, int out[4]);
+int ks_debug_radix_sort_batch(ks_ctx* ctx, uint64_t* const* keys, uint32_t* const* vals, const unsigned long long* n, int nb, size_t cap,
+                              unsigned begin_bit, unsigned end_bit);
 
 int ks_synchronize(ks_ctx* ctx);
 void* ks_stream(ks_ctx* ctx);
diff --git a/kimera_semantics_amd/binding.py b/kimera_semantics_amd/binding.py
--- a/kimera_semantics_amd/binding.py
+++ b/kimera_semantics_amd/binding.py
@@ -28,7 +28,7 @@
     "ks_default_config", "ks_create", "ks_destroy", "ks_last_error", "ks_set_color_to_label",
     "ks_integrate_points", "ks_integrate_points_device", "ks_integrate_depth", "ks_integrate_depth_device", "ks_num_blocks", "ks_get_block_indices",
     "ks_get_updated_block_indices", "ks_count_updated_voxels", "ks_download_updated_voxels", "ks_download_blocks", "ks_upload_blocks", "ks_host_alloc", "ks_host_free", "ks_get_tile_keys", "ks_export_tiles_device", "ks_merge_tiles_device", "ks_clear", "ks_clear_voxels", "ks_reset_tiles", "ks_tile_owner", "ks_reduce",
-    "ks_debug_radix_sort", "ks_synchronize", "ks_flush", "ks_stream",
+    "ks_debug_radix_sort", "ks_debug_radix_sort_bits", "ks_debug_radix_sort_plan", "ks_debug_radix_sort_batch", "ks_synchronize", "ks_flush", "ks_stream",
     "ks_profile_enable", "ks_profile_get", "ks_early_out_iterations", "ks_early_out_stats", "ks_pipeline_shape", "ks_stream_plan", "ks_seed_launch_shape", "ks_update_stats", "ks_integrate_round_exact",
     "ks_mesh_default_config", "ks_mesh_update", "ks_mesh_size", "ks_mesh_download", "ks_mesh_changed_blocks",
     "ks_esdf_default_config", "ks_esdf_update", "ks_esdf_download_blocks", "ks_esdf_query",
@@ -131,6 +131,14 @@
 
 
 _lib = None
+
+
+def radix_sort_plan(n: int, key_bits: int, has_values: bool, begin_bit: int, end_bit: int) -> dict:
+    out = (C.c_int * 4)()
+    rc = lib().ks_debug_radix_sort_plan(n, key_bits, int(has_values), begin_bit, end_bit, out)
+    if rc != 0:
+        raise KsError(rc, "ks_debug_radix_sort_plan")
+    return dict(tile=out[0], window=out[1], digit_bits=out[2], passes=out[3])
 
 
 def lib():
@@ -172,6 +180,9 @@
         L.ks_tile_owner.argtypes = [C.c_uint64, C.c_int]
         L.ks_reduce.argtypes = [vp, vp, C.c_int, C.c_int, C.POINTER(KsReduceStats)]
         L.ks_debug_radix_sort.argtypes = [vp, vp, vp, C.c_size_t, C.c_int, C.c_uint]
+        L.ks_debug_radix_sort_bits.argtypes = [vp, vp, vp, C.c_size_t, C.c_int, C.c_uint, C.c_uint]
+        L.ks_debug_radix_sort_plan.argtypes = [C.c_size_t, C.c_int, C.c_int, C.c_uint, C.c_uint, C.POINTER(C.c_int)]
+        L.ks_debug_radix_sort_batch.argtypes = [vp, C.POINTER(vp), C.POINTER(vp), C.POINTER(C.c_ulonglong), C.c_int, C.c_size_t, C.c_uint, C.c_uint]
         L.ks_synchronize.argtypes = [vp]
         L.ks_flush.argtypes = [vp, C.POINTER(KsFrameStats)]
         L.ks_stream.argtypes = [vp]
@@ -509,6 +520,23 @@
                                             bits if end_bit is None else end_bit))
         return keys, vals
 
+    def debug_radix_sort_bits(self, keys: np.ndarray, vals, begin_bit: int, end_bit: int):
+        keys = np.ascontiguousarray(keys).copy()
+        vals = None if vals is None else np.ascontiguousarray(vals, dtype=np.uint32).copy()
+        self._chk(lib().ks_debug_radix_sort_bits(self._h, _ptr(keys), _ptr(vals), keys.shape[0], keys.dtype.itemsize * 8, begin_bit, end_bit))
+        return keys, vals
+
+    def debug_radix_sort_batch(self, keys, vals, counts, begin_bit: int, end_bit: int):
+        keys = [np.ascontiguousarray(k, dtype=np.uint64).copy() for k in keys]
+        vals = [np.ascontiguousarray(v, dtype=np.uint32).copy() for v in vals]
+        nb, cap = len(keys), keys[0].shape[0]
+        assert all(k.shape == (cap,) for k in keys) and all(v.shape == (cap,) for v in vals) and len(vals) == nb == len(counts)
+        kp = (C.c_void_p * nb)(*[k.ctypes.data for k in keys])
+        vp_ = (C.c_void_p * nb)(*[v.ctypes.data for v in vals])
+        n = (C.c_ulonglong * nb)(*[int(x) for x in counts])
+        self._chk(lib().ks_debug_radix_sort_batch(self._h, kp, vp_, n, nb, cap, begin_bit, end_bit))
+        return keys, vals
+
     def synchronize(self):
         self._chk(lib().ks_synchronize(self._h))
 
diff --git a/kimera_semantics_amd/csrc/ks_hip.hip b/kimera_semantics_amd/csrc/ks_hip.hip
--- a/kimera_semantics_amd/csrc/ks_hip.hip
+++ b/kimera_semantics_amd/csrc/ks_hip.hip
@@ -664,8 +664,8 @@
 }
 template <typename K>
 int sort_pairs(ks_ctx* c, K* ka, K* kb, uint32_t* va, uint32_t* vb, size_t n, unsigned end_bit, K** kres,
-               uint32_t** vres) {
-  HIPCHK(c, (ksrs::sort<K, true>(c->sort_ws, ka, kb, va, vb, n, end_bit, c->stream, kres, vres)));
+               uint32_t** vres, unsigned begin_bit = 0) {
+  HIPCHK(c, (ksrs::sort<K, true>(c->sort_ws, ka, kb, va, vb, n, end_bit, c->stream, kres, vres, begin_bit)));
   return KS_OK;
 }
 
@@ -814,6 +814,7 @@
   return KS_OK;
 }
 constexpr int kEoMaxIterations = 4096;
+constexpr unsigned kEoSlotBit = 44;
 int exact_early_out(ks_ctx* c, FrameSlot& S, hipStream_t st, Counters* counters = nullptr) {
   const size_t n = S.n;
   Counters* const d_counters = counters ? counters : S.d_counters;
@@ -845,7 +846,7 @@
                          c->d_eo_lp, c->d_eo_bt, c->d_eo_keys[0], c->d_eo_vals[0], (unsigned long long)c->cap_marks, d_counters,
                          c->d_eo_state);
     HIPCHK(c, (ksrs::sort<uint64_t, true>(counters ? c->sort_ws_tail : c->sort_ws, c->d_eo_keys[0], c->d_eo_keys[1], c->d_eo_vals[0], c->d_eo_vals[1],
-                                          (size_t)n_marks, 64, st, &kres, &vres, 44)));
+                                          (size_t)n_marks, 64, st, &kres, &vres, kEoSlotBit)));
     hipLaunchKernelGGL(k_eo_index, dim3((uint32_t)((n_marks + 255) / 256)), dim3(256), 0, st, n_marks, (const uint64_t*)kres,
                        c->d_eo_range);
     EoBuf E{kres, vres, c->d_eo_range, c->d_eo_plain};
@@ -894,7 +895,7 @@
         if ((rc = S.d_eo_keys[b].alloc(c, cap_marks))) return rc;
         if ((rc = S.d_eo_vals[b].alloc(c, cap_marks))) return rc;
       }
-      if ((rc = S.d_eo_sort_ws.alloc(c, ksrs::ws_words_dev(cap_marks, 3)))) return rc;
+      if ((rc = S.d_eo_sort_ws.alloc(c, ksrs::ws_words_dev(cap_marks, kEoSlotBit, 64)))) return rc;
       if ((rc = S.d_eo_hitb.alloc(c, cap_marks))) return rc;
       if ((rc = S.d_eo_hseq.alloc(c, cap_marks))) return rc;
       if ((rc = S.d_eo_where.alloc(c, cap_marks))) return rc;
@@ -934,8 +935,9 @@
   E.cnt_b = S.d_eo_cnt_b;
   E.ux = S.d_eo_ux;
   E.dirty = S.d_eo_dirty;
-  E.keys = S.d_eo_keys[1];
-  E.vals = S.d_eo_vals[1];
+  const int sorted = ksrs::dev_result_in_b(S.eo_cap_marks, kEoSlotBit, 64) ? 1 : 0;
+  E.keys = S.d_eo_keys[sorted];
+  E.vals = S.d_eo_vals[sorted];
   E.bits_a = S.d_eo_bits_a;
   E.bits_b = S.d_eo_bits_b;
   E.lp = S.d_eo_lp;
@@ -998,7 +1000,7 @@
     hipLaunchKernelGGL(k_eo2_full, dim3(gn, nb), dim3(256), 0, st, Bt);
     hipLaunchKernelGGL(k_eo2_scan, dim3(nb4k, nb), dim3(1024), 0, st, Bt);
     hipLaunchKernelGGL(k_eo2_emit<8>, dim3((uint32_t)((n + 31) / 32), nb), dim3(256), lds, st, Bt);
-    HIPCHK(c, ksrs::sort_dev_batch<uint64_t>(Rs, (int)nb, S0.d_eo_sort_ws.size(), S0.eo_cap_marks, 44, 64, st));
+    HIPCHK(c, ksrs::sort_dev_batch<uint64_t>(Rs, (int)nb, S0.d_eo_sort_ws.size(), S0.eo_cap_marks, kEoSlotBit, 64, st));
     hipLaunchKernelGGL(k_eo2_bits, dim3(gm, nb), dim3(256), 0, st, Bt, 0u);
     hipLaunchKernelGGL(k_eo2_where, dim3(gm, nb), dim3(256), 0, st, Bt);
     enqueue_sweeps(c, Bt, nb, c->eo_sweeps, st);
@@ -1006,7 +1008,7 @@
   } else {
     hipLaunchKernelGGL(k_eo2_scan, dim3(nb4k, nb), dim3(1024), 0, st, Bt);
     hipLaunchKernelGGL(k_eo2_emit<64>, dim3((uint32_t)((n + 255) / 256), nb), dim3(256), lds, st, Bt);
-    HIPCHK(c, ksrs::sort_dev_batch<uint64_t>(Rs, (int)nb, S0.d_eo_sort_ws.size(), S0.eo_cap_marks, 44, 64, st));
+    HIPCHK(c, ksrs::sort_dev_batch<uint64_t>(Rs, (int)nb, S0.d_eo_sort_ws.size(), S0.eo_cap_marks, kEoSlotBit, 64, st));
     hipLaunchKernelGGL(k_eo2_hits, dim3(gm, nb), dim3(256), 0, st, Bt);
     hipLaunchKernelGGL(k_eo2_stop0, dim3(gn, nb), dim3(256), 0, st, Bt);
     hipLaunchKernelGGL(k_eo2_bits, dim3(gm, nb), dim3(256), 0, st, Bt, 1u);
@@ -3267,7 +3269,7 @@
   if (p) (void)hipHostFree(p);
 }
 
-int ks_debug_radix_sort(ks_ctx* c, void* keys, uint32_t* vals, size_t n, int key_bits, unsigned end_bit) {
+int ks_debug_radix_sort_bits(ks_ctx* c, void* keys, uint32_t* vals, size_t n, int key_bits, unsigned begin_bit, unsigned end_bit) {
   if (!c || (n && !keys) || (key_bits != 32 && key_bits != 64)) return KS_ERR_INVALID_ARG;
   if (n == 0) return KS_OK;
   const size_t kb = key_bits / 8;
@@ -3284,19 +3286,67 @@
   uint32_t* vres = nullptr;
   if (key_bits == 32) {
     uint32_t* r = nullptr;
-    rc = vals ? sort_pairs(c, (uint32_t*)ka.get(), (uint32_t*)kbuf.get(), va.get(), vb.get(), n, end_bit, &r, &vres)
-              : sort_keys(c, (uint32_t*)ka.get(), (uint32_t*)kbuf.get(), n, end_bit, &r);
+    rc = vals ? sort_pairs(c, (uint32_t*)ka.get(), (uint32_t*)kbuf.get(), va.get(), vb.get(), n, end_bit, &r, &vres, begin_bit)
+              : sort_keys(c, (uint32_t*)ka.get(), (uint32_t*)kbuf.get(), n, end_bit, &r, begin_bit);
     kres = r;
   } else {
     uint64_t* r = nullptr;
-    rc = vals ? sort_pairs(c, (uint64_t*)ka.get(), (uint64_t*)kbuf.get(), va.get(), vb.get(), n, end_bit, &r, &vres)
-              : sort_keys(c, (uint64_t*)ka.get(), (uint64_t*)kbuf.get(), n, end_bit, &r);
+    rc = vals ? sort_pairs(c, (uint64_t*)ka.get(), (uint64_t*)kbuf.get(), va.get(), vb.get(), n, end_bit, &r, &vres, begin_bit)
+              : sort_keys(c, (uint64_t*)ka.get(), (uint64_t*)kbuf.get(), n, end_bit, &r, begin_bit);
     kres = r;
   }
   if (rc) return rc;
   HIPCHK(c, hipStreamSynchronize(c->stream));
   HIPCHK(c, hipMemcpy(keys, kres, n * kb, hipMemcpyDeviceToHost));
   if (vals) HIPCHK(c, hipMemcpy(vals, vres, n * 4, hipMemcpyDeviceToHost));
+  return KS_OK;
+}
+
+int ks_debug_radix_sort(ks_ctx* c, void* keys, uint32_t* vals, size_t n, int key_bits, unsigned end_bit) {
+  return ks_debug_radix_sort_bits(c, keys, vals, n, key_bits, 0u, end_bit);
+}
+
+int ks_debug_radix_sort_plan(size_t n, int key_bits, int has_values, unsigned begin_bit, unsigned end_bit, int out[4]) {
+  if (!out || (key_bits != 32 && key_bits != 64) || end_bit <= begin_bit || end_bit > (unsigned)key_bits) return KS_ERR_INVALID_ARG;
+  const ksrs::Plan P = ksrs::plan(n, end_bit - begin_bit, has_values != 0);
+  out[0] = P.tile;
+  out[1] = ksrs::window_of(P);
+  out[2] = P.rb;
+  out[3] = P.passes;
+  return KS_OK;
+}
+
+int ks_debug_radix_sort_batch(ks_ctx* c, uint64_t* const* keys, uint32_t* const* vals, const unsigned long long* n, int nb, size_t cap,
+                              unsigned begin_bit, unsigned end_bit) {
+  if (!c || !keys || !vals || !n || nb < 1 || nb > ksrs::kRsBatch || cap == 0 || end_bit <= begin_bit || end_bit > 64) return KS_ERR_INVALID_ARG;
+  for (int i = 0; i < nb; ++i)
+    if (!keys[i] || !vals[i] || n[i] > cap) return KS_ERR_INVALID_ARG;
+  DevBuf<uint64_t> k[ksrs::kRsBatch][2];
+  DevBuf<uint32_t> v[ksrs::kRsBatch][2], ws[ksrs::kRsBatch];
+  DevBuf<unsigned long long> d_n;
+  const size_t ws_words = ksrs::ws_words_dev(cap, begin_bit, end_bit);
+  ksrs::DevBatch<uint64_t> Rs{};
+  int rc;
+  if ((rc = d_n.alloc(c, (size_t)nb))) return rc;
+  HIPCHK(c, hipMemcpy(d_n, n, (size_t)nb * sizeof(unsigned long long), hipMemcpyHostToDevice));
+  for (int i = 0; i < nb; ++i) {
+    for (int b = 0; b < 2; ++b) {
+      if ((rc = k[i][b].alloc(c, cap)) || (rc = v[i][b].alloc(c, cap))) return rc;
+      HIPCHK(c, hipMemcpy(k[i][b], keys[i], cap * sizeof(uint64_t), hipMemcpyHostToDevice));
+      HIPCHK(c, hipMemcpy(v[i][b], vals[i], cap * sizeof(uint32_t), hipMemcpyHostToDevice));
+    }
+    if ((rc = ws[i].alloc(c, ws_words))) return rc;
+    Rs.keys_a[i] = k[i][0], Rs.keys_b[i] = k[i][1], Rs.vals_a[i] = v[i][0], Rs.vals_b[i] = v[i][1];
+    Rs.n_dev[i] = d_n.get() + i;
+    Rs.ws[i] = ws[i];
+  }
+  HIPCHK(c, ksrs::sort_dev_batch<uint64_t>(Rs, nb, ws_words, cap, begin_bit, end_bit, c->stream));
+  HIPCHK(c, hipStreamSynchronize(c->stream));
+  const int r = ksrs::dev_result_in_b(cap, begin_bit, end_bit) ? 1 : 0;
+  for (int i = 0; i < nb; ++i) {
+    HIPCHK(c, hipMemcpy(keys[i], k[i][r], cap * sizeof(uint64_t), hipMemcpyDeviceToHost));
+    HIPCHK(c, hipMemcpy(vals[i], v[i][r], cap * sizeof(uint32_t), hipMemcpyDeviceToHost));
+  }
   return KS_OK;
 }
 
diff --git a/kimera_semantics_amd/csrc/ks_radix_sort.h b/kimera_semantics_amd/csrc/ks_radix_sort.h
--- a/kimera_semantics_amd/csrc/ks_radix_sort.h
+++ b/kimera_semantics_amd/csrc/ks_radix_sort.h
@@ -13,9 +13,13 @@
 constexpr size_t kHistBlocks = 2048;
 constexpr uint32_t kFlagLocal = 1u << 30, kFlagPrefix = 2u << 30, kCountMask = (1u << 30) - 1u;
 
-template <int RB, typename K>
-__device__ __forceinline__ uint32_t digit_of(K key, int shift) {
-  return (uint32_t)(key >> shift) & (uint32_t)((1 << RB) - 1);
+template <typename K>
+__device__ __forceinline__ uint32_t digit_of(K key, int shift, uint32_t mask) {
+  return (uint32_t)(key >> shift) & mask;
+}
+__host__ __device__ __forceinline__ uint32_t digit_mask(int rb, int shift, int end_bit) {
+  const int nb = end_bit - shift < rb ? end_bit - shift : rb;
+  return nb <= 0 ? 0u : (1u << nb) - 1u;
 }
 
 template <int RB>
@@ -31,7 +35,7 @@
 }
 
 template <typename K, int RB>
-__device__ __forceinline__ void rs_hist_body(const K* __restrict__ keys, uint32_t n, int passes, int begin_bit,
+__device__ __forceinline__ void rs_hist_body(const K* __restrict__ keys, uint32_t n, int passes, int begin_bit, int end_bit,
                                              uint32_t* __restrict__ hist, uint32_t* __restrict__ zero_ptr,
                                              uint32_t zero_words, const unsigned long long* __restrict__ n_dev, uint32_t* s_hist) {
   constexpr int kBins = 1 << RB;
@@ -51,7 +55,7 @@
       const K key = valid ? keys[idx] : (K)0;
       const unsigned long long active = __ballot(valid);
       for (int p = 0; p < passes; ++p) {
-        const uint32_t d = digit_of<RB>(key, begin_bit + p * RB);
+        const uint32_t d = digit_of(key, begin_bit + p * RB, digit_mask(RB, begin_bit + p * RB, end_bit));
         const uint32_t d0 = (uint32_t)__builtin_amdgcn_readfirstlane((int)d);
         if (__ballot(valid && d != d0) == 0ull) {
           if (active && lane == (uint32_t)(__ffsll((long long)active) - 1))
@@ -76,11 +80,11 @@
   }
 }
 template <typename K, int RB>
-__global__ void __launch_bounds__(256) k_rs_hist(const K* __restrict__ keys, uint32_t n, int passes, int begin_bit,
+__global__ void __launch_bounds__(256) k_rs_hist(const K* __restrict__ keys, uint32_t n, int passes, int begin_bit, int end_bit,
                                                  uint32_t* __restrict__ hist, uint32_t* __restrict__ zero_ptr,
                                                  uint32_t zero_words, const unsigned long long* __restrict__ n_dev = nullptr) {
   extern __shared__ uint32_t s_hist[];
-  rs_hist_body<K, RB>(keys, n, passes, begin_bit, hist, zero_ptr, zero_words, n_dev, s_hist);
+  rs_hist_body<K, RB>(keys, n, passes, begin_bit, end_bit, hist, zero_ptr, zero_words, n_dev, s_hist);
 }
 constexpr int kRsBatch = 8;
 template <typename K>
@@ -93,15 +97,21 @@
   uint32_t* ws[kRsBatch];
 };
 template <typename K, int RB>
-__global__ void __launch_bounds__(256) k_rs_hist_b(DevBatch<K> B, uint32_t cap, int passes, int begin_bit) {
+__global__ void __launch_bounds__(256) k_rs_hist_b(DevBatch<K> B, uint32_t cap, int passes, int begin_bit, int end_bit) {
   extern __shared__ uint32_t s_hist[];
-  rs_hist_body<K, RB>(B.keys_a[blockIdx.y], cap, passes, begin_bit, B.ws[blockIdx.y], nullptr, 0u, B.n_dev[blockIdx.y], s_hist);
-}
+  rs_hist_body<K, RB>(B.keys_a[blockIdx.y], cap, passes, begin_bit, end_bit, B.ws[blockIdx.y], nullptr, 0u, B.n_dev[blockIdx.y], s_hist);
+}
+
+template <int RB, int THREADS, int ITEMS>
+struct LookBack {
+  static constexpr int kOwn = ((1 << RB) + THREADS - 1) / THREADS;
+  static constexpr int kWindow = (kOwn == 1 && ITEMS < 32) ? 32 : 16;
+};
 
 template <typename K, bool HAS_VALUES, int THREADS, int ITEMS, int RB, bool REORDER = false>
 __device__ __forceinline__ void rs_pass_body(const K* __restrict__ keys_in, K* __restrict__ keys_out,
                                              const uint32_t* __restrict__ vals_in,
-                                             uint32_t* __restrict__ vals_out, uint32_t n, int shift,
+                                             uint32_t* __restrict__ vals_out, uint32_t n, int shift, uint32_t mask,
                                              const uint32_t* __restrict__ bin_hist,
                                              uint32_t* __restrict__ status, uint32_t* __restrict__ ticket,
                                              const unsigned long long* __restrict__ n_dev) {
@@ -136,7 +146,7 @@
   for (int i = 0; i < ITEMS; ++i) {
     const uint32_t idx = wbase + i * 64 + lane;
     const bool valid = idx < n;
-    const uint32_t d = digit_of<RB>(key[i], shift);
+    const uint32_t d = digit_of(key[i], shift, mask);
     const unsigned long long peers = match_digit<RB>(d, __ballot(valid));
     const uint32_t prev = s_cnt[wave][d];
     rd[i] = (prev + (uint32_t)__popcll(peers & ((1ull << lane) - 1ull))) | (d << 20);
@@ -146,42 +156,71 @@
   }
   __syncthreads();
 
-  for (int d = tid; d < kBins; d += THREADS) {
-    uint32_t total = 0;
-#pragma unroll
-    for (int w = 0; w < kWaves; ++w) {
-      const uint32_t c = s_cnt[w][d];
-      s_cnt[w][d] = total;
-      total += c;
-    }
-    if (REORDER) s_loc[d] = total;
-    uint32_t* st = status + d;
-    uint32_t prefix = 0;
-    __hip_atomic_store(st + (size_t)tile * kBins, total | kFlagLocal, __ATOMIC_RELAXED, __HIP_MEMORY_SCOPE_AGENT);
-    constexpr int kWindow = 8;
-    int t = (int)tile - 1;
-    bool done = false;
-    while (!done) {
-      uint32_t s[kWindow];
-#pragma unroll
-      for (int j = 0; j < kWindow; ++j)
-        s[j] = (t - j >= 0) ? __hip_atomic_load(st + (size_t)(t - j) * kBins, __ATOMIC_RELAXED, __HIP_MEMORY_SCOPE_AGENT)
-                            : kFlagPrefix;
-      int consumed = 0;
-#pragma unroll
-      for (int j = 0; j < kWindow; ++j) {
-        if (done || consumed != j) continue;
-        const uint32_t flag = s[j] >> 30;
-        if (flag == 0u) continue;
-        prefix += s[j] & kCountMask;
-        ++consumed;
-        if (flag == 2u) done = true;
-      }
-      t -= consumed;
-    }
-    __hip_atomic_store(st + (size_t)tile * kBins, (prefix + total) | kFlagPrefix, __ATOMIC_RELAXED,
-                       __HIP_MEMORY_SCOPE_AGENT);
-    s_off[d] = prefix;
+  {
+    using LB = LookBack<RB, THREADS, ITEMS>;
+    constexpr int kOwn = LB::kOwn, kWindow = LB::kWindow;
+    uint32_t total[kOwn], prefix[kOwn];
+    int t[kOwn];
+    bool done[kOwn];
+#pragma unroll
+    for (int q = 0; q < kOwn; ++q) {
+      const int d = (int)tid + q * THREADS;
+      total[q] = 0;
+      prefix[q] = 0;
+      t[q] = (int)tile - 1;
+      done[q] = d >= kBins;
+      if (d < kBins) {
+        uint32_t sum = 0;
+#pragma unroll
+        for (int w = 0; w < kWaves; ++w) {
+          const uint32_t c = s_cnt[w][d];
+          s_cnt[w][d] = sum;
+          sum += c;
+        }
+        total[q] = sum;
+        if (REORDER) s_loc[d] = sum;
+        __hip_atomic_store(status + (size_t)tile * kBins + d, sum | kFlagLocal, __ATOMIC_RELAXED, __HIP_MEMORY_SCOPE_AGENT);
+      }
+    }
+    bool all_done = false;
+    while (!all_done) {
+      uint32_t s[kOwn][kWindow];
+#pragma unroll
+      for (int q = 0; q < kOwn; ++q) {
+        const uint32_t* st = status + (tid + q * THREADS);
+#pragma unroll
+        for (int j = 0; j < kWindow; ++j)
+          s[q][j] = (!done[q] && t[q] - j >= 0) ? __hip_atomic_load(st + (size_t)(t[q] - j) * kBins, __ATOMIC_RELAXED, __HIP_MEMORY_SCOPE_AGENT)
+                                                : kFlagPrefix;
+      }
+      all_done = true;
+#pragma unroll
+      for (int q = 0; q < kOwn; ++q) {
+        bool live = !done[q];
+        int consumed = 0;
+#pragma unroll
+        for (int j = 0; j < kWindow; ++j) {
+          const uint32_t flag = s[q][j] >> 30;
+          live = live && flag != 0u;
+          if (live) {
+            prefix[q] += s[q][j] & kCountMask;
+            ++consumed;
+            if (flag == 2u) { done[q] = true; live = false; }
+          }
+        }
+        t[q] -= consumed;
+        all_done = all_done && done[q];
+      }
+    }
+#pragma unroll
+    for (int q = 0; q < kOwn; ++q) {
+      const int d = (int)tid + q * THREADS;
+      if (d < kBins) {
+        __hip_atomic_store(status + (size_t)tile * kBins + d, (prefix[q] + total[q]) | kFlagPrefix, __ATOMIC_RELAXED,
+                           __HIP_MEMORY_SCOPE_AGENT);
+        s_off[d] = prefix[q];
+      }
+    }
   }
   __syncthreads();
   for (int c = wave; c < kChunks; c += kWaves) {
@@ -236,7 +275,7 @@
     const uint32_t count = (n - t0 < (uint32_t)kTile) ? n - t0 : (uint32_t)kTile;
     for (uint32_t j = tid; j < count; j += THREADS) {
       const K k = s_keys[j];
-      const uint32_t d = digit_of<RB>(k, shift);
+      const uint32_t d = digit_of(k, shift, mask);
       keys_out[s_off[d] + (j - s_loc[d])] = k;
     }
     return;
@@ -256,19 +295,19 @@
 template <typename K, bool HAS_VALUES, int THREADS, int ITEMS, int RB, bool REORDER = false>
 __global__ void __launch_bounds__(THREADS) k_rs_pass(const K* __restrict__ keys_in, K* __restrict__ keys_out,
                                                      const uint32_t* __restrict__ vals_in,
-                                                     uint32_t* __restrict__ vals_out, uint32_t n, int shift,
+                                                     uint32_t* __restrict__ vals_out, uint32_t n, int shift, uint32_t mask,
                                                      const uint32_t* __restrict__ bin_hist,
                                                      uint32_t* __restrict__ status, uint32_t* __restrict__ ticket,
                                                      const unsigned long long* __restrict__ n_dev = nullptr) {
-  rs_pass_body<K, HAS_VALUES, THREADS, ITEMS, RB, REORDER>(keys_in, keys_out, vals_in, vals_out, n, shift, bin_hist, status, ticket, n_dev);
+  rs_pass_body<K, HAS_VALUES, THREADS, ITEMS, RB, REORDER>(keys_in, keys_out, vals_in, vals_out, n, shift, mask, bin_hist, status, ticket, n_dev);
 }
 template <typename K, int THREADS, int ITEMS, int RB>
-__global__ void __launch_bounds__(THREADS) k_rs_pass_b(DevBatch<K> B, uint32_t cap, int begin_bit, int p, uint32_t tiles) {
+__global__ void __launch_bounds__(THREADS) k_rs_pass_b(DevBatch<K> B, uint32_t cap, int begin_bit, int end_bit, int p, uint32_t tiles) {
   const uint32_t y = blockIdx.y;
   uint32_t* ws = B.ws[y];
   const bool odd = (p & 1) != 0;
   rs_pass_body<K, true, THREADS, ITEMS, RB, false>(odd ? B.keys_b[y] : B.keys_a[y], odd ? B.keys_a[y] : B.keys_b[y], odd ? B.vals_b[y] : B.vals_a[y],
-                                                   odd ? B.vals_a[y] : B.vals_b[y], cap, begin_bit + p * RB, ws + (size_t)p * kMaxBins,
+                                                   odd ? B.vals_a[y] : B.vals_b[y], cap, begin_bit + p * RB, digit_mask(RB, begin_bit + p * RB, end_bit), ws + (size_t)p * kMaxBins,
                                                    ws + ((size_t)kMaxPasses * kMaxBins + kMaxPasses) + (size_t)p * tiles * (1 << RB),
                                                    ws + (size_t)kMaxPasses * kMaxBins + p, B.n_dev[y]);
 }
@@ -295,40 +334,59 @@
   return hipSuccess;
 }
 
-template <typename K, bool HAS_VALUES, int THREADS, int ITEMS, int RB, bool REORDER = false>
-inline void launch_passes(Workspace& w, K*& kin, K*& kout, uint32_t*& vin, uint32_t*& vout, size_t n, int passes,
-                          uint32_t tiles, unsigned begin_bit, hipStream_t stream) {
-  constexpr int kBins = 1 << RB;
-  uint32_t* base = w.d_ws + (size_t)w.cur * w.words;
-  uint32_t* hist = base;
-  uint32_t* tickets = base + (size_t)kMaxPasses * kMaxBins;
-  uint32_t* status = base + kHeadWords;
-  for (int p = 0; p < passes; ++p) {
-    hipLaunchKernelGGL((k_rs_pass<K, HAS_VALUES, THREADS, ITEMS, RB, REORDER>), dim3(tiles), dim3(THREADS), 0, stream, kin, kout,
-                       vin, vout, (uint32_t)n, (int)begin_bit + p * RB, hist + (size_t)p * kMaxBins,
-                       status + (size_t)p * tiles * kBins, tickets + p);
-    K* tk = kin; kin = kout; kout = tk;
-    uint32_t* tv = vin; vin = vout; vout = tv;
-  }
-}
-
-template <typename K, bool HAS_VALUES, int RB>
-inline hipError_t sort_rb(Workspace& w, K* keys_a, K* keys_b, uint32_t* vals_a, uint32_t* vals_b, size_t n,
-                          unsigned begin_bit, unsigned end_bit, hipStream_t stream, K** keys_result,
-                          uint32_t** vals_result) {
-  constexpr int kBins = 1 << RB;
-  const int passes = (int)((end_bit - begin_bit + RB - 1) / RB);
-  const bool reorder = !HAS_VALUES && n > (1u << 20);
-  const int tile = (n <= (1u << 20)) ? 2048 : (reorder || n <= (1u << 24)) ? 8192 : 16384;
-  const uint32_t tiles = (uint32_t)((n + tile - 1) / tile);
-  const size_t words = kHeadWords + (size_t)passes * tiles * kBins;
+struct Plan {
+  int rb, passes, tile, threads, items;
+  bool reorder;
+};
+inline Plan plan(size_t n, unsigned bits, bool has_values) {
+  const int cls = n <= (1u << 20) ? 0 : n <= (1u << 24) ? 1 : 2;
+  const unsigned p11 = (bits + 10) / 11, width = p11 ? (bits + p11 - 1) / p11 : 0;
+  const int rb = (cls == 1 && has_values && width > 8 && width <= 10) ? 10 : 8;
+  Plan P{};
+  P.rb = rb;
+  P.passes = (int)((bits + rb - 1) / rb);
+  P.reorder = !has_values && cls == 1;
+  P.threads = cls == 0 ? 256 : 512;
+  P.items = cls == 0 ? 8 : cls == 1 ? 16 : 32;
+  P.tile = P.threads * P.items;
+  return P;
+}
+#define KS_RS_FOR_SHAPE(P, X)                                                   \
+  do {                                                                          \
+    if ((P).rb == 10) { X(512, 16, 10, false); }                                \
+    else if ((P).threads == 256) { X(256, 8, 8, false); }                       \
+    else if ((P).items == 16 && (P).reorder) { X(512, 16, 8, true); }           \
+    else if ((P).items == 16) { X(512, 16, 8, false); }                         \
+    else { X(512, 32, 8, false); }                                              \
+  } while (0)
+inline int window_of(const Plan& P) {
+  int w = 0;
+#define KS_RS_WINDOW(THREADS, ITEMS, RB, REORDER) w = LookBack<RB, THREADS, ITEMS>::kWindow
+  KS_RS_FOR_SHAPE(P, KS_RS_WINDOW);
+#undef KS_RS_WINDOW
+  return w;
+}
+inline size_t status_words(const Plan& P, size_t n) { return (size_t)P.passes * ((n + P.tile - 1) / P.tile) * ((size_t)1 << P.rb); }
+
+template <typename K, bool HAS_VALUES>
+inline hipError_t sort_planned(Workspace& w, const Plan& P, K* keys_a, K* keys_b, uint32_t* vals_a, uint32_t* vals_b, size_t n,
+                               unsigned begin_bit, unsigned end_bit, hipStream_t stream, K** keys_result, uint32_t** vals_result) {
+  const uint32_t tiles = (uint32_t)((n + P.tile - 1) / P.tile);
+  const size_t bins = (size_t)1 << P.rb;
+  const size_t words = kHeadWords + status_words(P, n);
   hipError_t e = ensure(w, words, stream);
   if (e != hipSuccess) return e;
   const int h = w.cur ^ 1;
-  hipLaunchKernelGGL((k_rs_hist<K, RB>), dim3((uint32_t)std::min<size_t>((n + 2047) / 2048, kHistBlocks)), dim3(256),
-                     (size_t)passes * kBins * sizeof(uint32_t), stream, keys_a, (uint32_t)n, passes, (int)begin_bit,
-                     w.d_ws + (size_t)h * w.words, w.d_ws + (size_t)(h ^ 1) * w.words,
-                     (uint32_t)((w.dirty[h ^ 1] + 3) & ~(size_t)3));
+  uint32_t* base = w.d_ws + (size_t)h * w.words;
+  uint32_t* zero_ptr = w.d_ws + (size_t)(h ^ 1) * w.words;
+  const uint32_t zero_words = (uint32_t)((w.dirty[h ^ 1] + 3) & ~(size_t)3);
+  const dim3 hgrid((uint32_t)std::min<size_t>((n + 2047) / 2048, kHistBlocks));
+  const size_t hlds = (size_t)P.passes * bins * sizeof(uint32_t);
+#define KS_RS_HIST(RB) \
+  hipLaunchKernelGGL((k_rs_hist<K, RB>), hgrid, dim3(256), hlds, stream, (const K*)keys_a, (uint32_t)n, P.passes, (int)begin_bit, (int)end_bit, base, zero_ptr, zero_words)
+  if (P.rb == 10) KS_RS_HIST(10);
+  else KS_RS_HIST(8);
+#undef KS_RS_HIST
   w.dirty[h ^ 1] = 0;
   w.dirty[h] = words;
   w.cur = h;
@@ -336,77 +394,67 @@
   K* kout = keys_b;
   uint32_t* vin = vals_a;
   uint32_t* vout = vals_b;
-  if (tile == 2048) launch_passes<K, HAS_VALUES, 256, 8, RB>(w, kin, kout, vin, vout, n, passes, tiles, begin_bit, stream);
-  else if (tile == 8192 && reorder) {
-    if constexpr (!HAS_VALUES) launch_passes<K, false, 512, 16, RB, true>(w, kin, kout, vin, vout, n, passes, tiles, begin_bit, stream);
-  } else if (tile == 8192) launch_passes<K, HAS_VALUES, 512, 16, RB>(w, kin, kout, vin, vout, n, passes, tiles, begin_bit, stream);
-  else launch_passes<K, HAS_VALUES, 512, 32, RB>(w, kin, kout, vin, vout, n, passes, tiles, begin_bit, stream);
+  uint32_t* tickets = base + (size_t)kMaxPasses * kMaxBins;
+  uint32_t* status = base + kHeadWords;
+  for (int p = 0; p < P.passes; ++p) {
+    const int shift = (int)begin_bit + p * P.rb;
+#define KS_RS_PASS(THREADS, ITEMS, RB, REORDER)                                                                                  \
+  if constexpr (!(REORDER && HAS_VALUES))                                                                                        \
+    hipLaunchKernelGGL((k_rs_pass<K, HAS_VALUES, THREADS, ITEMS, RB, REORDER>), dim3(tiles), dim3(THREADS), 0, stream, (const K*)kin, \
+                       kout, (const uint32_t*)vin, vout, (uint32_t)n, shift, digit_mask(RB, shift, (int)end_bit),                 \
+                       (const uint32_t*)(base + (size_t)p * kMaxBins), status + (size_t)p * tiles * bins, tickets + p)
+    KS_RS_FOR_SHAPE(P, KS_RS_PASS);
+#undef KS_RS_PASS
+    K* tk = kin; kin = kout; kout = tk;
+    uint32_t* tv = vin; vin = vout; vout = tv;
+  }
   *keys_result = kin;
   if (vals_result) *vals_result = vin;
   return hipGetLastError();
 }
 
-inline size_t dev_tile(size_t cap) { return cap <= (1u << 20) ? 2048 : cap <= (1u << 24) ? 8192 : 16384; }
-inline size_t ws_words_dev(size_t cap, int passes) { return kHeadWords + (size_t)passes * ((cap + dev_tile(cap) - 1) / dev_tile(cap)) * 256; }
+inline size_t ws_words_dev(size_t cap, unsigned begin_bit, unsigned end_bit) {
+  return kHeadWords + status_words(plan(cap, end_bit - begin_bit, true), cap);
+}
+inline bool dev_result_in_b(size_t cap, unsigned begin_bit, unsigned end_bit) { return (plan(cap, end_bit - begin_bit, true).passes & 1) != 0; }
+template <typename K>
+inline hipError_t sort_dev_batch(const DevBatch<K>& B, int nb, size_t ws_words, size_t cap, unsigned begin_bit, unsigned end_bit, hipStream_t stream) {
+  if (end_bit <= begin_bit || end_bit > sizeof(K) * 8 || nb < 1 || nb > kRsBatch) return hipErrorInvalidValue;
+  const Plan P = plan(cap, end_bit - begin_bit, true);
+  const uint32_t tiles = (uint32_t)((cap + P.tile - 1) / P.tile);
+  const size_t words = kHeadWords + status_words(P, cap);
+  if (words > ws_words) return hipErrorInvalidValue;
+  for (int y = 0; y < nb; ++y) {
+    hipError_t e = hipMemsetAsync(B.ws[y], 0, words * sizeof(uint32_t), stream);
+    if (e != hipSuccess) return e;
+  }
+  const dim3 hgrid((uint32_t)std::min<size_t>((cap + 2047) / 2048, kHistBlocks), (uint32_t)nb);
+  const size_t hlds = ((size_t)P.passes << P.rb) * sizeof(uint32_t);
+#define KS_RS_HIST(RB) hipLaunchKernelGGL((k_rs_hist_b<K, RB>), hgrid, dim3(256), hlds, stream, B, (uint32_t)cap, P.passes, (int)begin_bit, (int)end_bit)
+  if (P.rb == 10) KS_RS_HIST(10);
+  else KS_RS_HIST(8);
+#undef KS_RS_HIST
+  for (int p = 0; p < P.passes; ++p) {
+#define KS_RS_PASS(THREADS, ITEMS, RB, REORDER)                                                                                          \
+  if constexpr (!REORDER)                                                                                                                \
+    hipLaunchKernelGGL((k_rs_pass_b<K, THREADS, ITEMS, RB>), dim3(tiles, (uint32_t)nb), dim3(THREADS), 0, stream, B, (uint32_t)cap,       \
+                       (int)begin_bit, (int)end_bit, p, tiles)
+    KS_RS_FOR_SHAPE(P, KS_RS_PASS);
+#undef KS_RS_PASS
+  }
+  return hipGetLastError();
+}
 template <typename K>
 inline hipError_t sort_dev(uint32_t* ws, size_t ws_words, K* keys_a, K* keys_b, uint32_t* vals_a, uint32_t* vals_b,
                            const unsigned long long* n_dev, size_t cap, unsigned begin_bit, unsigned end_bit, hipStream_t stream,
                            K** keys_result, uint32_t** vals_result) {
-  constexpr int RB = 8;
-  constexpr int kBins = 1 << RB;
-  const int passes = (int)((end_bit - begin_bit + RB - 1) / RB);
-  const size_t tile = dev_tile(cap);
-  const uint32_t tiles = (uint32_t)((cap + tile - 1) / tile);
-  if (kHeadWords + (size_t)passes * tiles * kBins > ws_words) return hipErrorInvalidValue;
-  hipError_t e = hipMemsetAsync(ws, 0, (kHeadWords + (size_t)passes * tiles * kBins) * sizeof(uint32_t), stream);
-  if (e != hipSuccess) return e;
-  uint32_t* hist = ws;
-  uint32_t* tickets = ws + (size_t)kMaxPasses * kMaxBins;
-  uint32_t* status = ws + kHeadWords;
-  hipLaunchKernelGGL((k_rs_hist<K, RB>), dim3((uint32_t)std::min<size_t>((cap + 2047) / 2048, kHistBlocks)), dim3(256),
-                     (size_t)passes * kBins * sizeof(uint32_t), stream, (const K*)keys_a, (uint32_t)cap, passes, (int)begin_bit, hist,
-                     (uint32_t*)nullptr, 0u, n_dev);
-  K* kin = keys_a;
-  K* kout = keys_b;
-  uint32_t* vin = vals_a;
-  uint32_t* vout = vals_b;
-  for (int p = 0; p < passes; ++p) {
-#define KS_RS_DEV_PASS(THREADS, ITEMS)                                                                                                 \
-  hipLaunchKernelGGL((k_rs_pass<K, true, THREADS, ITEMS, RB>), dim3(tiles), dim3(THREADS), 0, stream, (const K*)kin, kout,             \
-                     (const uint32_t*)vin, vout, (uint32_t)cap, (int)begin_bit + p * RB, (const uint32_t*)(hist + (size_t)p * kMaxBins), \
-                     status + (size_t)p * tiles * kBins, tickets + p, n_dev)
-    if (tile == 2048) KS_RS_DEV_PASS(256, 8);
-    else if (tile == 8192) KS_RS_DEV_PASS(512, 16);
-    else KS_RS_DEV_PASS(512, 32);
-#undef KS_RS_DEV_PASS
-    K* tk = kin; kin = kout; kout = tk;
-    uint32_t* tv = vin; vin = vout; vout = tv;
-  }
-  *keys_result = kin;
-  *vals_result = vin;
-  return hipGetLastError();
-}
-
-template <typename K>
-inline hipError_t sort_dev_batch(const DevBatch<K>& B, int nb, size_t ws_words, size_t cap, unsigned begin_bit, unsigned end_bit, hipStream_t stream) {
-  constexpr int RB = 8;
-  constexpr int kBins = 1 << RB;
-  const int passes = (int)((end_bit - begin_bit + RB - 1) / RB);
-  const size_t tile = dev_tile(cap);
-  const uint32_t tiles = (uint32_t)((cap + tile - 1) / tile);
-  if (kHeadWords + (size_t)passes * tiles * kBins > ws_words || nb < 1 || nb > kRsBatch) return hipErrorInvalidValue;
-  for (int y = 0; y < nb; ++y) {
-    hipError_t e = hipMemsetAsync(B.ws[y], 0, (kHeadWords + (size_t)passes * tiles * kBins) * sizeof(uint32_t), stream);
-    if (e != hipSuccess) return e;
-  }
-  hipLaunchKernelGGL((k_rs_hist_b<K, RB>), dim3((uint32_t)std::min<size_t>((cap + 2047) / 2048, kHistBlocks), (uint32_t)nb), dim3(256),
-                     (size_t)passes * kBins * sizeof(uint32_t), stream, B, (uint32_t)cap, passes, (int)begin_bit);
-  for (int p = 0; p < passes; ++p) {
-    if (tile == 2048) hipLaunchKernelGGL((k_rs_pass_b<K, 256, 8, RB>), dim3(tiles, (uint32_t)nb), dim3(256), 0, stream, B, (uint32_t)cap, (int)begin_bit, p, tiles);
-    else if (tile == 8192) hipLaunchKernelGGL((k_rs_pass_b<K, 512, 16, RB>), dim3(tiles, (uint32_t)nb), dim3(512), 0, stream, B, (uint32_t)cap, (int)begin_bit, p, tiles);
-    else hipLaunchKernelGGL((k_rs_pass_b<K, 512, 32, RB>), dim3(tiles, (uint32_t)nb), dim3(512), 0, stream, B, (uint32_t)cap, (int)begin_bit, p, tiles);
-  }
-  return hipGetLastError();
+  DevBatch<K> B{};
+  B.keys_a[0] = keys_a, B.keys_b[0] = keys_b, B.vals_a[0] = vals_a, B.vals_b[0] = vals_b, B.n_dev[0] = n_dev, B.ws[0] = ws;
+  const hipError_t e = sort_dev_batch<K>(B, 1, ws_words, cap, begin_bit, end_bit, stream);
+  const bool in_b = dev_result_in_b(cap, begin_bit, end_bit);
+  *keys_result = in_b ? keys_b : keys_a;
+  *vals_result = in_b ? vals_b : vals_a;
+  return e;
 }
 
 template <typename K, bool HAS_VALUES>
@@ -417,7 +465,8 @@
   if (vals_result) *vals_result = vals_a;
   if (end_bit > sizeof(K) * 8) end_bit = (unsigned)(sizeof(K) * 8);
   if (n == 0 || end_bit <= begin_bit) return hipSuccess;
-  return sort_rb<K, HAS_VALUES, 8>(w, keys_a, keys_b, vals_a, vals_b, n, begin_bit, end_bit, stream, keys_result, vals_result);
-}
-
-}
+  return sort_planned<K, HAS_VALUES>(w, plan(n, end_bit - begin_bit, HAS_VALUES), keys_a, keys_b, vals_a, vals_b, n, begin_bit, end_bit,
+                                     stream, keys_result, vals_result);
+}
+
+}
```

Result: slower. 996.4 Mvoxel-updates/s (-1.6%).
